# snap-research/MMVID

Hardware: AMD Instinct MI355X
Metric: video-tokens/sec training step, 8-frame 128px text-to-video (higher is better)
Workload: dtype bf16

## Files before the change

### include/mmvid_hip.h

```cpp
#ifndef MMVID_HIP_H
#define MMVID_HIP_H
#include <stdint.h>
#ifdef __cplusplus
extern "C" {
#endif

const char* mmvid_last_error(void);
int mmvid_abi_version(void);
int mmvid_device_count(void);

int mmvid_vq_sqnorm(const float* codebook, int n, int dim, float* ee, void* stream);
int mmvid_vq_argmin_l2(const float* z, const float* codebook, const float* ee, int64_t rows, int n, int dim,
                       int64_t* idx, float* dmin, void* stream);
int mmvid_gather_rows(const float* table, int64_t table_rows, const int64_t* idx, int64_t rows, int dim,
                      float* out_f32, void* out_bf16, void* stream);

int mmvid_gemm_bf16(int a_kmajor, int b_kmajor, int M, int N, int K, const void* A, int64_t lda, const void* B,
                    int64_t ldb, int batch, int64_t strideA, int64_t strideB, int64_t strideC, int splitk,
                    float alpha, const float* bias, const float* residual, int64_t ldr, const void* dact_pre,
                    void* save_pre, int64_t ldp, int act, int accumulate, float* out_f32, void* out_bf16,
                    int64_t ldc, float* out_colsum,
                    void* stream);

int mmvid_decode_trace(void* dev_buf);
int mmvid_decode_persistent_trace(void* dev_buf);

int mmvid_gemm_bf16_dw(int64_t M, int N, int K, const void* dY, int64_t ldy, const void* X, int64_t ldx, int splitk,
                       float* workspace, float* dW, int accumulate, void* stream);
int mmvid_gemm_dw_pick_splitk(int64_t M, int N, int K);
typedef struct {
    int N, K;
    const void* dY;
    int64_t ldy, strideY;
    const void* X;
    int64_t ldx, strideX;
    float* const* dW_list;
} mmvid_dw_kind_t;
int mmvid_gemm_bf16_dw_multi(int64_t M, int nkinds, const mmvid_dw_kind_t* kinds, int groups, int accumulate, void* stream);
int mmvid_gemm_bf16_dw_grouped(int64_t M, int N, int K, const void* dY, int64_t ldy, int64_t strideY, const void* X, int64_t ldx,
                               int64_t strideX, int groups, float* const* dW_list, int accumulate, void* stream);
double mmvid_gemm_dw_multi_fill(int nkinds, const mmvid_dw_kind_t* kinds, int groups);

int mmvid_layernorm_fwd(const float* x, int64_t ldx, int64_t rows, int E, const float* w, const float* b, float eps,
                        void* y_bf16, float* y_f32, int64_t ldy, float* mean, float* rstd, void* stream);
int mmvid_layernorm_bwd(const float* dy, int64_t lddy, const float* x, int64_t ldx, const float* mean,
                        const float* rstd, const float* w, int64_t rows, int E, float* dx, int64_t lddx,
                        int add_into_dx, void* dx_bf16, float* dw, float* db, float* dx_colsum, void* stream);
int mmvid_layernorm_bwd_ws(const float* dy, int64_t lddy, const float* x, int64_t ldx, const float* mean,
                           const float* rstd, const float* w, int64_t rows, int E, float* dx, int64_t lddx,
                           int add_into_dx, void* dx_bf16, float* dw, float* db, float* dx_colsum, float* workspace,
                           int64_t workspace_floats, void* stream);
int mmvid_layernorm_bwd_ex(const void* dy, int dy_is_bf16, int64_t lddy, const float* x, int64_t ldx, const float* mean,
                           const float* rstd, const float* w, int64_t rows, int E, float* dx, int64_t lddx, int add_into_dx,
                           void* dx_bf16, float* dw, float* db, float* dx_colsum, float* workspace, int64_t workspace_floats,
                           void* stream);
typedef struct {
    const float* partial;
    float *dw, *db, *dx_colsum;
} mmvid_ln_reduce_t;
int mmvid_layernorm_bwd_partial(const void* dy, int dy_is_bf16, int64_t lddy, const float* x, int64_t ldx, const float* mean,
                                const float* rstd, const float* w, int64_t rows, int E, float* dx, int64_t lddx, int add_into_dx,
                                void* dx_bf16, int want_dw, int want_db, int want_colsum, float* workspace,
                                int64_t workspace_floats, int* blocks_out, void* stream);
int mmvid_layernorm_bwd_reduce_multi(int n, const mmvid_ln_reduce_t* items, int blocks, int E, void* stream);
int mmvid_groupnorm_swish_nhwc(const void* x, int x_is_bf16, int N, int64_t hw, int C, const float* w,
                               const float* b, float eps, int swish, float* stats_scratch, int partial_blocks,
                               void* y_bf16, float* y_f32, void* stream);

int mmvid_attention_fwd(const void* qkv, int64_t ld, int B, int L, int H, int E, float scale, int mask_mode, int r0,
                        int c0, int r1, int c1, void* out, int64_t ldo, float* lse2, void* stream);
int mmvid_attention_bwd(const void* qkv, int64_t ld, const void* O, int64_t ldo, const void* dO, int64_t lddo,
                        const float* lse2, float* delta, int B, int L, int H, int E, float scale, int mask_mode,
                        int r0, int c0, int r1, int c1, void* dqkv, int64_t ldg, void* stream);
int mmvid_attention_bwd_bias(const void* qkv, int64_t ld, const void* O, int64_t ldo, const void* dO, int64_t lddo,
                             const float* lse2, float* delta, int B, int L, int H, int E, float scale, int mask_mode, int r0,
                             int c0, int r1, int c1, void* dqkv, int64_t ldg, float* dbias, void* stream);
int mmvid_assemble_sequence(const float* const* tables, const int64_t* table_rows, int ntables, const int64_t* ids,
                            const int32_t* seg, const float* pos, int64_t B, int L, int E, float* out, void* stream);
int mmvid_assemble_sequence_bwd(float* const* grad_tables, const int64_t* table_rows, int ntables,
                                const int64_t* ids, const int32_t* seg, const float* dx, int64_t B, int L, int E,
                                float* dpos, int accumulate_dpos, void* stream);
int mmvid_cross_entropy_fwd(const float* logits, int64_t ldl, const int64_t* target, const uint8_t* select,
                            int64_t rows, int V, float* lse, float* loss_sum, void* stream);
int mmvid_cross_entropy_bwd(const float* logits, int64_t ldl, const int64_t* target, const uint8_t* select,
                            const float* lse, const float* gscale, int64_t rows, int V, void* dlogits_bf16,
                            int64_t ldd, void* stream);
int mmvid_colsum_bf16(const void* dy, int64_t ld, int64_t M, int N, float* db, void* stream);
typedef struct {
    const float* w[3];
    float* gw[3];
    int32_t dst0, rows, naxes, src0;
    int32_t d[3];
    int32_t pad;
} mmvid_pos_segment_t;
int mmvid_pos_table_fwd(const mmvid_pos_segment_t* segs, int nseg, int L, int E, float* out, void* stream);
int mmvid_pos_table_bwd(const mmvid_pos_segment_t* segs, int nseg, int E, const float* g, void* stream);
int mmvid_lincomb3(const float* a, const float* b, const float* c, float wa, float wb, float wc, float* out, void* stream);
int mmvid_scale3(const float* g, float wa, float wb, float wc, float* ga, float* gb, float* gc, void* stream);
int mmvid_rows_pack(const float* W, int64_t V, int E, const int64_t* ids, int n, int64_t* uid, float* rows, void* stream);
int mmvid_rows_merge(float* W, int64_t V, int E, const int64_t* ids, const float* rows, int n, void* stream);

int mmvid_device_faults(int64_t* counts, int reset);

int mmvid_grad_sqnorm(const float* g, int64_t n, float* out_accum, void* stream);
int mmvid_adam_step(float* p, const float* g, float* m, float* v, void* shadow_bf16, int64_t n, float lr,
                    float beta1, float beta2, float eps, float weight_decay, int step, const float* step_dev,
                    float max_norm, const float* sqnorm, float grad_scale, void* stream);
int mmvid_grad_sqnorm_det(const float* g, int64_t n, float* partials, float* out_accum, void* stream);
int mmvid_adam_step_lr(float* p, const float* g, float* m, float* v, void* shadow_bf16, int64_t n, float lr,
                       const float* lr_dev, float beta1, float beta2, float eps, float weight_decay, int step,
                       const float* step_dev, float max_norm, const float* sqnorm, float grad_scale, void* stream);
int mmvid_grad_sqnorm_rows(const float* g, int64_t n, float* partials, float* out_accum, const uint8_t* row_flags,
                           int64_t table_lo, int64_t table_rows, int rowlen, void* stream);
int mmvid_adam_step_rows(float* p, const float* g, float* m, float* v, void* shadow_bf16, int64_t n, float lr,
                         const float* lr_dev, float beta1, float beta2, float eps, float weight_decay, int step,
                         const float* step_dev, float max_norm, const float* sqnorm, float grad_scale,
                         const uint8_t* row_flags, int64_t table_lo, int64_t table_rows, int rowlen, void* stream);
int mmvid_lr_schedule(const float* step_dev, int kind, float lr_min, float lr_max, int warmup_steps, int every,
                      float* lr_out, void* stream);
int mmvid_counter_add(float* counter, float value, void* stream);
int mmvid_cast_f32_to_bf16(const float* x, void* y, int64_t n, void* stream);

int mmvid_msm_masks(uint64_t seed, const float* step_dev, int B, int T, int f, const float* strategy_prob, float bern_lo,
                    float bern_hi, float pc_prob, uint8_t* mask1, float* not_fully_masked, int32_t* strategy_out,
                    void* stream);
int mmvid_msm_masks_inject(const int32_t* decisions, const uint8_t* bernoulli, int B, int T, int f, uint8_t* mask1,
                           float* not_fully_masked, void* stream);
int mmvid_warp_params_bytes(void);
int mmvid_vid_warp(uint64_t seed, const float* step_dev, const float* x, int B, int T, int C, int H, int W,
                   const float* strategy_prob, void* params_scratch, int draw_params, float* out, void* stream);
int mmvid_vid_warp_new_frames(uint64_t seed, const float* step_dev, const float* x, int B, int T, int C, int H, int W,
                              const float* strategy_prob, void* params_scratch, int draw_params, float* new_frames,
                              void* stream);
int mmvid_vid_warp_tokens(const int64_t* target_tok, const int64_t* new_frame_tok, const void* params, int B, int T, int n,
                          int64_t* out, void* stream);
int mmvid_frames_u8_to_f32(const uint8_t* frames_u8, int N, int H, int W, float* out, void* stream);
int mmvid_frames_to_u8(const float* img, int64_t N, int H, int W, uint8_t* out, void* stream);
int mmvid_vid_warp_new_frames_u8(uint64_t seed, const float* step_dev, const uint8_t* x_u8, int B, int T, int H, int W,
                                 const float* strategy_prob, void* params_scratch, int draw_params, float* new_frames,
                                 void* stream);
int mmvid_vid_warp_draw(uint64_t seed, const float* step_dev, int B, int T, const float* strategy_prob, void* params_scratch,
                        void* stream);
int mmvid_token_rows_gather(const uint16_t* table, int64_t table_rows, const int64_t* frame_index, int64_t rows, int n,
                            int64_t* out, void* stream);
int mmvid_erase_tokens_choice(uint64_t seed, const float* step_dev, int nchoice, const float* cumprob, const int32_t* modes,
                              const int32_t* boxes, int frame0_full, int B, int Tv, int f, int64_t value, int64_t* tok,
                              void* stream);
int mmvid_random_erase_tokens(uint64_t seed, const float* step_dev, int B, int Tv, int f, float p, float scale_lo,
                              float scale_hi, float ratio_lo, float ratio_hi, int erase_half, int64_t value, int64_t* tok,
                              void* stream);

int mmvid_visual_color_jitter(uint64_t seed, const float* step_dev, float* x, int B, int Tv, int C, int H, int W, float p,
                              int first_frame, float* params_out, void* stream);

typedef struct {
    const float *ln1_w, *ln1_b, *ln2_w, *ln2_b;
    const void* in_w;
    const float* in_b;
    const void* out_w;
    const float* out_b;
    const void* fc_w;
    const float* fc_b;
    const void* pj_w;
    const float* pj_b;
    float *g_ln1_w, *g_ln1_b, *g_ln2_w, *g_ln2_b, *g_in_w, *g_in_b, *g_out_w, *g_out_b, *g_fc_w, *g_fc_b, *g_pj_w,
        *g_pj_b;
} mmvid_tower_layer_t;

typedef struct {
    int B, L, E, H, F, layers;
    int mask_mode, r0, c0, r1, c1;
    float ln_eps;
} mmvid_tower_cfg_t;

int mmvid_tower_workspace(const mmvid_tower_cfg_t* cfg, int64_t* saved_bytes, int64_t* scratch_bytes);
int mmvid_tower_forward(const mmvid_tower_cfg_t* cfg, const mmvid_tower_layer_t* layers, const float* x_in,
                        float* x_out, void* saved, void* scratch, void* stream);
int mmvid_tower_backward(const mmvid_tower_cfg_t* cfg, const mmvid_tower_layer_t* layers, float* g,
                         void* saved, void* scratch, void* stream);


int mmvid_tower_prefill(const mmvid_tower_cfg_t* cfg, const mmvid_tower_layer_t* layers, const float* x_in,
                        float* x_out, void* kv_cache, int Lmax, void* scratch, void* stream);
int mmvid_tower_decode(const mmvid_tower_cfg_t* cfg, const mmvid_tower_layer_t* layers, const float* x_in, float* x_out,
                       void* kv_cache, int Lmax, const int32_t* pos_dev, int pos, void* scratch, void* stream);
int mmvid_tower_decode_fused(const mmvid_tower_cfg_t* cfg, const mmvid_tower_layer_t* layers, const float* x_in,
                             float* x_out, void* kv_cache, int Lmax, const int32_t* pos_dev, int pos, void* scratch,
                             void* stream);
int mmvid_tower_decode_fused_slice(const mmvid_tower_cfg_t* cfg, const mmvid_tower_layer_t* layers, const float* x_in,
                                   float* x_out, void* kv_cache, int Lmax, int cache_batch, int32_t* pos_dev, int pos,
                                   int advance_pos, void* scratch, void* stream);
int mmvid_tower_decode_persistent_supported(const mmvid_tower_cfg_t* cfg, int Lmax);
int64_t mmvid_tower_decode_persistent_workspace_bytes(int B);
int mmvid_tower_decode_persistent(const mmvid_tower_cfg_t* cfg, const mmvid_tower_layer_t* layers, const float* x_in, float* x_out,
                                  void* kv_cache, int Lmax, int32_t* pos_dev, int pos, int advance_pos, void* workspace, void* stream);
typedef struct {
    int64_t* tok;
    const float* table;
    int64_t table_rows;
    const float* pos_rows;
    int32_t pos_off;
    int32_t record_pos0;
    int64_t* record;
    int64_t record_ld;
    const float *lnf_w, *lnf_b;
    const void* head_w;
    const float* head_b;
    const float* E;
    int64_t e_step_stride;
    int64_t tok_offset;
    float* logits_out;
    int32_t V, e_pos0;
    float lnf_eps, temperature;
} mmvid_decode_token_t;
int mmvid_artv_token_step_persistent(const mmvid_tower_cfg_t* cfg, const mmvid_tower_layer_t* layers, const mmvid_decode_token_t* t,
                                     float* x_out, void* kv_cache, int Lmax, int32_t* pos_dev, void* workspace, void* stream);
int mmvid_gemv_rows(const float* x, int64_t ldx, int NB, int K, const float* ln_w, const float* ln_b, float eps, const void* W,
                    const float* bias, int N, int act, const float* residual, int64_t ldr, int round_in, int round_out,
                    float* out, int64_t ldo, void* stream);
int mmvid_decode_embed(const int64_t* tok, const float* table, int64_t table_rows, const float* pos_rows,
                       const int32_t* pos_dev, int pos_off, int B, int E, float* x, void* stream);
int mmvid_decode_embed_record(const int64_t* tok, const float* table, int64_t table_rows, const float* pos_rows,
                              const int32_t* pos_dev, int pos_off, int B, int E, float* x, int64_t* record, int64_t record_ld,
                              int record_pos0, void* stream);
int mmvid_kv_store(const void* qkv, int64_t ldq, int B, int L, int E, const int32_t* pos_dev, int pos0, int Lmax,
                   void* cache, void* stream);
int mmvid_attention_decode(const void* qkv, int64_t ldq, const void* cache, int B, int Lmax, int H, int E,
                           const int32_t* pos_dev, int pos0, float scale, void* out, int64_t ldo, void* stream);

int mmvid_conv2d_nhwc(int mode, const void* x, int N, int Hin, int Win, int Cin, const void* w, const float* bias,
                      int Cout, const void* residual_bf16, const float* residual_f32, int clamp01, void* out_bf16,
                      float* out_f32, float* gn_partial, void* stream);
int mmvid_conv2d_nhwc_splitk(int mode, const void* x, int N, int Hin, int Win, int Cin, const void* w, const float* bias,
                             int Cout, const void* residual_bf16, const float* residual_f32, int clamp01, void* out_bf16,
                             float* out_f32, float* gn_partial, int splitk, float* workspace, void* stream);
int mmvid_conv3x3_strip_supported(int H, int W, int Cin, int Cout);
int mmvid_conv3x3_strip_nhwc(const void* x, int N, int H, int W, int Cin, const void* w, const float* bias, int Cout,
                             const void* residual_bf16, const float* residual_f32, void* out_bf16, float* out_f32,
                             float* gn_partial64, void* stream);
int mmvid_image_to_nhwc8(const float* img, int N, int H, int W, void* out_bf16, void* stream);
int mmvid_nhwc_to_nchw_f32(const float* x, int N, int H, int W, int C, int Cuse, float* out, void* stream);
int mmvid_spatial_attention(const void* q, const void* k, const void* v, int N, int HW, int C, float scale,
                            float* scores_scratch, void* out_bf16, void* stream);
int mmvid_spatial_attention_ld(const void* q, const void* k, const void* v, int64_t ld, int N, int HW, int C, float scale,
                               float* scores_scratch, void* out_bf16, void* stream);

int mmvid_sample_race(const float* logits, int64_t ld, const float* E, const float* noise_u, float temperature,
                      float logit_div, int64_t R, int V, int64_t tok_offset, int64_t* tok, float* y, void* stream);
int mmvid_sample_race_at(const float* logits, int64_t ld, const float* E, const int32_t* step_dev, int step0, int64_t e_step_stride,
                         const float* noise_u, float temperature, float logit_div, int64_t R, int V, int64_t tok_offset, int64_t* tok,
                         float* y, void* stream);
int mmvid_mp_select_keep(const float* Y, const float* E, const uint8_t* preserve, int b, int Bm, int TS, int k,
                         uint8_t* mask1, void* stream);
int mmvid_mp_build_input(const float* control_emb, const float* image_emb, int64_t table_rows, const float* tpos,
                         const int64_t* I_tok, const uint8_t* mask1, int b, int Bm, int csl, int TS, int E, int64_t mask_id,
                         float* out, void* stream);
int mmvid_mp_update(const uint8_t* mask1, const float* Ynew, const int64_t* Inew, const float* rel_logit,
                    const float* vid_logit, int b, int Bm, int TS, int t, int dynamic, float* Y, int64_t* I_tok,
                    int64_t* Imax, float* Smax, int32_t* tmax, uint8_t* active, float* S_out, int32_t* jmax_out,
                    void* stream);
int mmvid_head_bce_fwd(const float* x, int64_t ldx, const int64_t* rows, int R, int E, const float* ln_w, const float* ln_b,
                       float eps, const float* w, const float* b, const float* label, const float* row_weight,
// ... 154 lines not shown
```

### mmvid_amd/_lib.py

```python
import ctypes
import os
from ctypes import POINTER, Structure, c_char_p, c_float, c_int, c_int32, c_int64, c_uint8, c_uint64, c_void_p

HERE = os.path.dirname(os.path.abspath(__file__))
LIB_PATH = os.environ.get('MMVID_LIB') or os.path.join(HERE, 'libmmvid_hip.so')

P = c_void_p
I, I64, F, U64 = c_int, c_int64, c_float, c_uint64


class TowerLayer(Structure):
    _fields_ = [(n, P) for n in (
        'ln1_w', 'ln1_b', 'ln2_w', 'ln2_b', 'in_w', 'in_b', 'out_w', 'out_b', 'fc_w', 'fc_b', 'pj_w', 'pj_b',
        'g_ln1_w', 'g_ln1_b', 'g_ln2_w', 'g_ln2_b', 'g_in_w', 'g_in_b', 'g_out_w', 'g_out_b', 'g_fc_w', 'g_fc_b',
        'g_pj_w', 'g_pj_b')]


class TowerCfg(Structure):
    _fields_ = [('B', I), ('L', I), ('E', I), ('H', I), ('F', I), ('layers', I), ('mask_mode', I), ('r0', I),
                ('c0', I), ('r1', I), ('c1', I), ('ln_eps', F)]


class DecodeToken(Structure):
    _fields_ = [('tok', c_void_p), ('table', c_void_p), ('table_rows', c_int64), ('pos_rows', c_void_p), ('pos_off', c_int32),
                ('record_pos0', c_int32), ('record', c_void_p), ('record_ld', c_int64), ('lnf_w', c_void_p), ('lnf_b', c_void_p),
                ('head_w', c_void_p), ('head_b', c_void_p), ('E', c_void_p), ('e_step_stride', c_int64), ('tok_offset', c_int64),
                ('logits_out', c_void_p), ('V', c_int32), ('e_pos0', c_int32), ('lnf_eps', c_float), ('temperature', c_float)]


class PostLnLayer(Structure):
    _fields_ = [(n, P) for n in ('qkv_w', 'qkv_b', 'out_w', 'out_b', 'ln1_w', 'ln1_b', 'fc_w', 'fc_b', 'pj_w', 'pj_b', 'ln2_w', 'ln2_b')]


class PostLnCfg(Structure):
    _fields_ = [('B', I), ('L', I), ('E', I), ('H', I), ('F', I), ('layers', I), ('ln_eps', F)]


class Conv3dCfg(Structure):
    _fields_ = [(n, I) for n in ('N', 'T', 'H', 'W', 'Cin', 'Cout', 'kt', 'kh', 'kw', 'st', 'sh', 'sw', 'pt0', 'pt1', 'ph0', 'ph1',
                                 'pw0', 'pw1', 'relu', 'nseg')] + [('seg_end', I * 3), ('ldo', I * 3), ('c_off', I * 3), ('out', P * 3)]


class VqganOp(Structure):
    _fields_ = [('op', c_int32), ('mode', c_int32), ('N', c_int32), ('H', c_int32), ('W', c_int32), ('C', c_int32),
                ('Cout', c_int32), ('flags', c_int32), ('in0', I64), ('in1', I64), ('in2', I64), ('out_bf16', I64),
                ('out_f32', I64), ('scratch', I64), ('w', P), ('b', P), ('ext_in', P), ('ext_out', P), ('eps', F),
                ('pad', c_int32)]


SIGNATURES = {
    'mmvid_vq_sqnorm': [P, I, I, P, P],
    'mmvid_vq_argmin_l2': [P, P, P, I64, I, I, P, P, P],
    'mmvid_gather_rows': [P, I64, P, I64, I, P, P, P],
    'mmvid_gemm_bf16': [I, I, I, I, I, P, I64, P, I64, I, I64, I64, I64, I, F, P, P, I64, P, P, I64, I, I, P, P, I64, P, P],
    'mmvid_gemm_bf16_dw': [I64, I, I, P, I64, P, I64, I, P, P, I, P],
    'mmvid_gemm_dw_pick_splitk': [I64, I, I],
    'mmvid_gemm_bf16_dw_grouped': [I64, I, I, P, I64, I64, P, I64, I64, I, P, I, P],
    'mmvid_gemm_bf16_dw_multi': [I64, I, P, I, I, P],
    'mmvid_layernorm_fwd': [P, I64, I64, I, P, P, F, P, P, I64, P, P, P],
    'mmvid_layernorm_bwd': [P, I64, P, I64, P, P, P, I64, I, P, I64, I, P, P, P, P, P],
    'mmvid_layernorm_bwd_ws': [P, I64, P, I64, P, P, P, I64, I, P, I64, I, P, P, P, P, P, I64, P],
    'mmvid_layernorm_bwd_partial': [P, I, I64, P, I64, P, P, P, I64, I, P, I64, I, P, I, I, I, P, I64, P, P],
    'mmvid_layernorm_bwd_reduce_multi': [I, P, I, I, P],
    'mmvid_layernorm_bwd_ex': [P, I, I64, P, I64, P, P, P, I64, I, P, I64, I, P, P, P, P, P, I64, P],
    'mmvid_groupnorm_swish_nhwc': [P, I, I, I64, I, P, P, F, I, P, I, P, P, P],
    'mmvid_attention_fwd': [P, I64, I, I, I, I, F, I, I, I, I, I, P, I64, P, P],
    'mmvid_attention_bwd': [P, I64, P, I64, P, I64, P, P, I, I, I, I, F, I, I, I, I, I, P, I64, P],
    'mmvid_attention_bwd_bias': [P, I64, P, I64, P, I64, P, P, I, I, I, I, F, I, I, I, I, I, P, I64, P, P],
    'mmvid_assemble_sequence': [POINTER(P), POINTER(I64), I, P, P, P, I64, I, I, P, P],
    'mmvid_assemble_sequence_bwd': [POINTER(P), POINTER(I64), I, P, P, P, I64, I, I, P, I, P],
    'mmvid_cross_entropy_fwd': [P, I64, P, P, I64, I, P, P, P],
    'mmvid_cross_entropy_bwd': [P, I64, P, P, P, P, I64, I, P, I64, P],
    'mmvid_colsum_bf16': [P, I64, I64, I, P, P],
    'mmvid_grad_sqnorm': [P, I64, P, P],
    'mmvid_adam_step': [P, P, P, P, P, I64, F, F, F, F, F, I, P, F, P, F, P],
    'mmvid_cast_f32_to_bf16': [P, P, I64, P],
    'mmvid_tower_workspace': [POINTER(TowerCfg), POINTER(I64), POINTER(I64)],
    'mmvid_tower_forward': [POINTER(TowerCfg), POINTER(TowerLayer), P, P, P, P, P],
    'mmvid_tower_backward': [POINTER(TowerCfg), POINTER(TowerLayer), P, P, P, P],
    'mmvid_tower_prefill': [POINTER(TowerCfg), POINTER(TowerLayer), P, P, P, I, P, P],
    'mmvid_tower_decode': [POINTER(TowerCfg), POINTER(TowerLayer), P, P, P, I, P, I, P, P],
    'mmvid_tower_decode_fused': [POINTER(TowerCfg), POINTER(TowerLayer), P, P, P, I, P, I, P, P],
    'mmvid_tower_decode_persistent': [POINTER(TowerCfg), POINTER(TowerLayer), P, P, P, I, P, I, I, P, P],
    'mmvid_artv_token_step_persistent': [POINTER(TowerCfg), POINTER(TowerLayer), POINTER(DecodeToken), P, P, I, P, P, P],
    'mmvid_tower_decode_fused_slice': [POINTER(TowerCfg), POINTER(TowerLayer), P, P, P, I, I, P, I, I, P, P],
    'mmvid_gemv_rows': [P, I64, I, I, P, P, F, P, P, I, I, P, I64, I, I, P, I64, P],
    'mmvid_decode_embed': [P, P, I64, P, P, I, I, I, P, P],
    'mmvid_decode_embed_record': [P, P, I64, P, P, I, I, I, P, P, I64, I, P],
    'mmvid_kv_store': [P, I64, I, I, I, P, I, I, P, P],
    'mmvid_attention_decode': [P, I64, P, I, I, I, I, P, I, F, P, I64, P],
    'mmvid_conv2d_nhwc': [I, P, I, I, I, I, P, P, I, P, P, I, P, P, P, P],
    'mmvid_conv2d_nhwc_splitk': [I, P, I, I, I, I, P, P, I, P, P, I, P, P, P, I, P, P],
    'mmvid_conv3x3_strip_supported': [I, I, I, I],
    'mmvid_conv3x3_strip_nhwc': [P, I, I, I, I, P, P, I, P, P, P, P, P, P],
    'mmvid_image_to_nhwc8': [P, I, I, I, P, P],
    'mmvid_nhwc_to_nchw_f32': [P, I, I, I, I, I, P, P],
    'mmvid_spatial_attention': [P, P, P, I, I, I, F, P, P, P],
    'mmvid_spatial_attention_ld': [P, P, P, I64, I, I, I, F, P, P, P],
    'mmvid_conv2d_nhwc_split3': [I, P, I, I, I, I, P, P, I, P, I, P, P, I, P, P],
    'mmvid_conv3x3_strip_nhwc_split3': [P, I, I, I, I, P, P, I, P, P, P, P, P],
    'mmvid_conv3x3_strip_nhwc_f16': [P, I, I, I, I, P, P, I, P, P, P, P, P],
    'mmvid_split_f32_bf16x2': [P, I64, P, P],
    'mmvid_image_to_nhwc8_split': [P, I, I, I, P, P],
    'mmvid_groupnorm_swish_nhwc_split': [P, I, I64, I, P, P, F, I, P, I, P, P],
    'mmvid_groupnorm_swish_nhwc_f16out': [P, I, I64, I, P, P, F, I, P, I, P, P],
    'mmvid_decode_trace': [P],
    'mmvid_decode_persistent_trace': [P],
    'mmvid_vqgan_run': [POINTER(VqganOp), I, P, P],
    'mmvid_sample_race': [P, I64, P, P, F, F, I64, I, I64, P, P, P],
    'mmvid_sample_race_at': [P, I64, P, P, I, I64, P, F, F, I64, I, I64, P, P, P],
    'mmvid_mp_select_keep': [P, P, P, I, I, I, I, P, P],
    'mmvid_mp_build_input': [P, P, I64, P, P, P, I, I, I, I, I, I64, P, P],
    'mmvid_mp_update': [P, P, P, P, P, I, I, I, I, I, P, P, P, P, P, P, P, P, P],
    'mmvid_head_bce_fwd': [P, I64, P, I, I, P, P, F, P, P, P, P, P, I, F, P, P, P, P, P],
    'mmvid_head_bce_bwd': [P, I64, P, I, I, P, P, P, P, P, P, P, P, P, I, F, P, P, I64, P, P, P, P, P],
    'mmvid_bert_build_ids': [P, P, P, P, P, P, I, I, I, I, I64, I64, I, I, P, P, P, P, P],
    'mmvid_grad_sqnorm_det': [P, I64, P, P, P],
    'mmvid_adam_step_lr': [P, P, P, P, P, I64, F, P, F, F, F, F, I, P, F, P, F, P],
    'mmvid_lr_schedule': [P, I, F, F, I, I, P, P],
    'mmvid_grad_sqnorm_rows': [P, I64, P, P, P, I64, I64, I, P],
    'mmvid_adam_step_rows': [P, P, P, P, P, I64, F, P, F, F, F, F, I, P, F, P, F, P, I64, I64, I, P],
    'mmvid_counter_add': [P, F, P],
    'mmvid_msm_masks': [U64, P, I, I, I, P, F, F, F, P, P, P, P],
    'mmvid_msm_masks_inject': [P, P, I, I, I, P, P, P],
    'mmvid_vid_warp': [U64, P, P, I, I, I, I, I, P, P, I, P, P],
    'mmvid_vid_warp_new_frames': [U64, P, P, I, I, I, I, I, P, P, I, P, P],
    'mmvid_vid_warp_tokens': [P, P, P, I, I, I, P, P],
    'mmvid_frames_u8_to_f32': [P, I, I, I, P, P],
    'mmvid_vid_warp_new_frames_u8': [U64, P, P, I, I, I, I, P, P, I, P, P],
    'mmvid_vid_warp_draw': [U64, P, I, I, P, P, P],
    'mmvid_token_rows_gather': [P, I64, P, I64, I, P, P],
    'mmvid_erase_tokens_choice': [U64, P, I, P, P, P, I, I, I, I, I64, P, P],
    'mmvid_random_erase_tokens': [U64, P, I, I, I, F, F, F, F, F, I, I64, P, P],
    'mmvid_visual_color_jitter': [U64, P, P, I, I, I, I, I, F, I, P, P],
    'mmvid_gemm_f32': [I, I, I, I, P, I64, P, I64, I, I64, I64, I64, F, P, P, P, I64, P],
    'mmvid_conv2d_nhwc_f32': [I, P, I, I, I, I, P, P, I, P, I, P, P],
    'mmvid_image_to_nhwc4_f32': [P, I, I, I, P, P],
    'mmvid_groupnorm_swish_nhwc_f32': [P, I, I64, I, P, P, F, I, P, P, P],
    'mmvid_spatial_attention_f32': [P, P, P, I, I, I, F, P, P, P],
    'mmvid_probe': [I, P, P, P],
    'mmvid_prof_begin': [I],
    'mmvid_prof_enable': [I],
    'mmvid_graph_stats': [P],
    'mmvid_set_option': [c_char_p, I],
    'mmvid_get_option': [c_char_p, POINTER(I)],
    'mmvid_colsum_bf16_det': [P, I64, I64, I, P, P, I64, P],
    'mmvid_cross_entropy_fwd_det': [P, I64, P, P, I64, I, P, P, P, I64, P],
    'mmvid_assemble_sequence_bwd_det': [POINTER(P), POINTER(I64), I, P, P, P, I64, I, I, P, I, P, I64, P],
    'mmvid_gemm_bf16_det': [I, I, I, I, I, P, I64, P, I64, I, I64, I64, I64, I, F, P, P, I64, P, P, I64, I, I, P, P, I64, P, P, I64, P],
    'mmvid_attention_bwd_bias_det': [P, I64, P, I64, P, I64, P, P, I, I, I, I, F, I, I, I, I, I, P, I64, P, P, I64, P],
    'mmvid_device_faults': [P, I],
    'mmvid_pos_table_fwd': [P, I, I, I, P, P],
    'mmvid_pos_table_bwd': [P, I, I, P, P],
    'mmvid_lincomb3': [P, P, P, F, F, F, P, P],
    'mmvid_scale3': [P, F, F, F, P, P, P, P],
    'mmvid_prof_end': [P, P, P, P, I],
    'mmvid_rows_pack': [P, I64, I, P, I, P, P, P],
    'mmvid_rows_merge': [P, I64, I, P, P, I, P],
    'mmvid_clip_patchify': [P, I, I, I, I, I, P, P],
    'mmvid_clip_image_assemble': [P, P, P, P, P, F, I, I, I, P, P],
    'mmvid_clip_text_embed': [P, I, I, P, I64, P, I, P, P, P],
    'mmvid_clip_pool_project': [P, I, I, I, P, P, P, F, P, I, I, P, P],
# ... 129 lines not shown
```

### mmvid_amd/clip_tower.py

```python
import ctypes
import os
import math

import torch
from torch import nn

from . import _lib, ops
from .functional import _note_params, _with_param_zeros

TOWER_SHAPES = {
    'openai_clip_visual': (768, 12, 12),
    'openai_clip_text': (512, 12, 8),
}
MATRIX_KEYS = ('attn.in_proj_weight', 'attn.out_proj.weight', 'mlp.c_fc.weight', 'mlp.c_proj.weight')


class _Holder(nn.Module):
    """Parameter container (no forward): gives parameters their reference names."""


def _linear_params(out_f, in_f, std):
    h = _Holder()
    h.weight = nn.Parameter(torch.randn(out_f, in_f) * std)
    h.bias = nn.Parameter(torch.zeros(out_f))
    return h


def _ln_params(e):
    h = _Holder()
    h.weight = nn.Parameter(torch.ones(e))
    h.bias = nn.Parameter(torch.zeros(e))
    return h


class ResidualAttentionBlockParams(_Holder):
    def __init__(self, width, layers):
        super().__init__()
        proj_std = (width**-0.5) * ((2 * layers)**-0.5)
        attn_std = width**-0.5
        fc_std = (2 * width)**-0.5
        self.attn = _Holder()
        self.attn.in_proj_weight = nn.Parameter(torch.randn(3 * width, width) * attn_std)
        self.attn.in_proj_bias = nn.Parameter(torch.zeros(3 * width))
        self.attn.out_proj = _linear_params(width, width, proj_std)
        self.ln_1 = _ln_params(width)
        self.mlp = _Holder()
        self.mlp.c_fc = _linear_params(4 * width, width, fc_std)
        self.mlp.c_proj = _linear_params(width, 4 * width, proj_std)
        self.ln_2 = _ln_params(width)


class _TowerParams(_Holder):
    def __init__(self, width, layers):
        super().__init__()
        self.resblocks = nn.ModuleList([ResidualAttentionBlockParams(width, layers) for _ in range(layers)])


class _TowerFn(torch.autograd.Function):
    @staticmethod
    def forward(ctx, x, tower, keep, *params):
        _note_params(ctx, (x, tower, keep) + params)
        ctx.tower = tower
        y, saved = tower._run_forward(x, keep=keep)
        ctx.saved_arena = saved
        ctx.shape = x.shape
        return y

    @staticmethod
    def backward(ctx, gy):
        g = gy.contiguous().clone()
        ctx.tower._run_backward(g, ctx.saved_arena, ctx.shape)
        ctx.saved_arena = None
        return _with_param_zeros(ctx, (g.view(ctx.shape), None, None) + (None, ) * (len(ctx.needs_input_grad) - 3))


class DecodeSession:

    def __init__(self, tower, kv_cache, first_pos, graph, fused=True):
        self.tower, self.cache, self.fused = tower, kv_cache, fused
        B, dev = kv_cache.shape[1], kv_cache.device
        self.cfg = tower._cfg(B, kv_cache.shape[2])
        self.layers, self._keep = tower._layer_structs(False)
        _, self.scratch = tower._workspace(self.cfg, dev, False)
        self.x = torch.zeros(B, tower.width, device=dev, dtype=torch.float32)
        self.y = torch.zeros_like(self.x)
        self.pos = torch.tensor([first_pos], dtype=torch.int32, device=dev)
        self.host_pos = int(first_pos)
        self.graph, self.want_graph, self.calls = None, graph, 0
        self._slice_cfgs = {}
        lib = _lib.load()
        self.persistent = bool(fused is True and os.environ.get('MMVID_DECODE_PERSISTENT', '1') != '0'
                               and lib.mmvid_tower_decode_persistent_supported(ctypes.byref(self.cfg), kv_cache.shape[2]))
        self.ws = torch.zeros(lib.mmvid_tower_decode_persistent_workspace_bytes(B) // 8, dtype=torch.int64, device=dev) if self.persistent else None

    def _enqueue(self):
        B, E = self.x.shape[0], self.x.shape[-1]
        if self.persistent:
            _lib.call('mmvid_tower_decode_persistent', ctypes.byref(self.cfg), self.layers, ops._p(self.x), ops._p(self.y),
                      ops._p(self.cache), self.cache.shape[2], ops._p(self.pos), 0, 1, ops._p(self.ws), ops._stream())
            return
        Lmax = self.cache.shape[2]
        if self.fused and E <= 768:
            per = 64 if E in (512, 768) else 16
            for b0 in range(0, B, per):
                nb = min(per, B - b0)
                cfg = self.cfg if nb == B else self._slice_cfgs.setdefault(nb, self.tower._cfg(nb, Lmax))
                _lib.call('mmvid_tower_decode_fused_slice', ctypes.byref(cfg), self.layers, self.x[b0:].data_ptr(), self.y[b0:].data_ptr(),
                          self.cache[0, b0].data_ptr(), Lmax, B, ops._p(self.pos), 0, int(b0 + per >= B), ops._p(self.scratch), ops._stream())
            return
        _lib.call('mmvid_tower_decode', ctypes.byref(self.cfg), self.layers, ops._p(self.x), ops._p(self.y),
                  ops._p(self.cache), Lmax, ops._p(self.pos), 0, ops._p(self.scratch), ops._stream())
        self.pos.add_(1)

    def token_step(self, tk):
        assert self.persistent
        _lib.call('mmvid_artv_token_step_persistent', ctypes.byref(self.cfg), self.layers, ctypes.byref(tk), ops._p(self.y), ops._p(self.cache),
                  self.cache.shape[2], ops._p(self.pos), ops._p(self.ws), ops._stream())
        self.host_pos += 1

    def failed(self):
        return bool(self.persistent and int(self.ws[1]) != 0)

    def fall_back(self, pos):
        self.persistent, self.graph = False, None
        self.fell_back = getattr(self, 'fell_back', 0) + 1
        self.pos.fill_(int(pos))
        self.host_pos = int(pos)

    def check(self):
        if self.failed():
            raise _lib.MMVIDError('persistent decode step: a poll timed out (the device was shared while it ran); results are invalid. '
                                  'Set MMVID_DECODE_PERSISTENT=0 to use the five-launch step.')

    @torch.no_grad()
    def step(self, x_new, verify=False):
        self.x.copy_(x_new)
        self.calls += 1
        if self.want_graph and self.graph is None and self.calls == 2:
            g = torch.cuda.CUDAGraph()
            side = torch.cuda.Stream()
            side.wait_stream(torch.cuda.current_stream())
            with torch.cuda.stream(side):
                with torch.cuda.graph(g, stream=side):
                    self._enqueue()
            torch.cuda.current_stream().wait_stream(side)
            self.graph = g
        if self.graph is not None:
            self.graph.replay()
        else:
            self._enqueue()
        if verify and self.persistent and self.failed():
            self.fall_back(self.host_pos)
            self._enqueue()
        self.host_pos += 1
        return self.y


class OpenAICLIPTransformer(nn.Module):
    def __init__(self, seq_len=0, which_model='openai_clip_text', model_path=None, causal=True, mask_type='causal',
                 mask_kwargs=None, layers=None, width=None, heads=None):
        super().__init__()
        if not which_model.startswith('openai_clip'):
            raise NotImplementedError(which_model)
        w, l, h = TOWER_SHAPES[which_model]
        self.width, self.layers, self.heads = width or w, layers or l, heads or h
        self.debug_keep_saved = False
        assert self.width == 64 * self.heads, 'head_dim must be 64 (CLIP towers)'
        self.context_length = seq_len
        self.causal = causal
        self.transformer = _TowerParams(self.width, self.layers)
        self.mask_spec = self.build_attention_mask(seq_len, mask_type, **(mask_kwargs or {})) if causal else None
        if model_path is not None:
            self.load_clip_checkpoint(model_path, which_model)
        self._shadow = None
        self._shadow_key = None
        self._scratch = None
        self._scratch_retired = []
        self.backward_chunk_layers = int(os.environ.get('MMVID_BWD_CHUNK', 0))
        self.on_layers_done = None

    @staticmethod
    def build_attention_mask(context_length, mask_type='causal', **kwargs):
        if mask_type == 'causal':
            return 'causal'
        if mask_type == 'mask_prev':
            idx = list(kwargs['index'])
            assert len(idx) <= 2, 'the kernels carry at most two restricted rows (BERT uses [ST1],[VID])'
            return ('rows', [(int(i), int(i)) for i in idx])
        raise NotImplementedError(mask_type)

    def dense_attention_mask(self, L=None):
        L = L or self.context_length
        if self.mask_spec is None:
            return None
        if self.mask_spec == 'causal':
            return torch.full((L, L), float('-inf')).triu_(1)
        m = torch.zeros(L, L)
        for r, c in self.mask_spec[1]:
            m[r, :c] = float('-inf')
        return m

    def load_clip_checkpoint(self, path, which_model):
        sd = torch.jit.load(path, map_location='cpu').state_dict()
        prefix = 'transformer.' if which_model == 'openai_clip_text' else 'visual.transformer.'
        own = {k[len(prefix):]: v.float() for k, v in sd.items() if k.startswith(prefix + 'resblocks.')}
        self.transformer.load_state_dict(own)

    def forward(self, x, **kwargs):
        assert x.dim() == 3 and x.shape[-1] == self.width
        keep = torch.is_grad_enabled() and (x.requires_grad or self._any_trainable())
        return _TowerFn.apply(x, self, keep, *self.parameters())

    def new_kv_cache(self, B, max_len, device):
        assert self.mask_spec == 'causal', 'incremental decoding needs the causal mask'
        return torch.empty(self.layers, B, max_len, 2 * self.width, device=device, dtype=torch.bfloat16)

    @torch.no_grad()
    def prefill(self, x, kv_cache):
        x = ops._chk(x.contiguous(), torch.float32, 'tower input')
        B, L, _ = x.shape
        cfg = self._cfg(B, L)
        layers, _keep = self._layer_structs(False)
        _, scratch = self._workspace(cfg, x.device, False)
        y = torch.empty_like(x)
        _lib.call('mmvid_tower_prefill', ctypes.byref(cfg), layers, ops._p(x), ops._p(y), ops._p(kv_cache),
                  kv_cache.shape[2], ops._p(scratch), ops._stream())
        return y

    @torch.no_grad()
    def decode_step(self, x_new, kv_cache, pos, pos_dev=None):
        x_new = ops._chk(x_new.contiguous(), torch.float32, 'tower input')
        B = x_new.shape[0]
        cfg = self._cfg(B, kv_cache.shape[2])
        layers, _keep = self._layer_structs(False)
        _, scratch = self._workspace(cfg, x_new.device, False)
        y = torch.empty_like(x_new)
        _lib.call('mmvid_tower_decode', ctypes.byref(cfg), layers, ops._p(x_new), ops._p(y), ops._p(kv_cache),
                  kv_cache.shape[2], ops._p(pos_dev), int(pos), ops._p(scratch), ops._stream())
        return y

    def decode_session(self, kv_cache, first_pos, graph=True, fused=True):
        return DecodeSession(self, kv_cache, first_pos, graph, fused)

    def _any_trainable(self):
        return any(p.requires_grad for p in self.parameters())

    def _matrix_params(self):
        for blk in self.transformer.resblocks:
            yield blk.attn.in_proj_weight
            yield blk.attn.out_proj.weight
            yield blk.mlp.c_fc.weight
            yield blk.mlp.c_proj.weight

    def attach_shadow(self, views):
        self._shadow = list(views)
        self.mark_shadow_fresh()

    def mark_shadow_fresh(self):
        self._shadow_key = tuple((p._version, p.data_ptr()) for p in self._matrix_params())

    def _sync_shadow(self):
        ps = list(self._matrix_params())
        key = tuple((p._version, p.data_ptr()) for p in ps)
        if self._shadow is None or self._shadow[0].device != ps[0].device:
            self._shadow = [torch.empty(p.shape, device=p.device, dtype=torch.bfloat16) for p in ps]
            self._shadow_key = None
        if key != self._shadow_key:
            for p, s in zip(ps, self._shadow):
                ops.cast_bf16(p.detach().contiguous(), s)
            self._shadow_key = key
        return self._shadow

    def _cfg(self, B, L):
        c = _lib.TowerCfg()
        c.B, c.L, c.E, c.H, c.F, c.layers = B, L, self.width, self.heads, 4 * self.width, self.layers
        c.mask_mode, c.r0, c.c0, c.r1, c.c1 = ops._mask_args(self.mask_spec)
        c.ln_eps = 1e-5
        return c

    def _layer_structs(self, with_grads):
        sh = self._sync_shadow()
        arr = (_lib.TowerLayer * self.layers)()
        keep = []

        def ptr(t):
            keep.append(t)
            return t.data_ptr()

        def gptr(p):
            if not with_grads or not p.requires_grad:
                return None
            if p.grad is None:
                p.grad = torch.zeros_like(p)
            return p.grad.data_ptr()

        for i, blk in enumerate(self.transformer.resblocks):
            a = arr[i]
            a.ln1_w, a.ln1_b = ptr(blk.ln_1.weight), ptr(blk.ln_1.bias)
            a.ln2_w, a.ln2_b = ptr(blk.ln_2.weight), ptr(blk.ln_2.bias)
            a.in_w, a.in_b = ptr(sh[4 * i]), ptr(blk.attn.in_proj_bias)
            a.out_w, a.out_b = ptr(sh[4 * i + 1]), ptr(blk.attn.out_proj.bias)
            a.fc_w, a.fc_b = ptr(sh[4 * i + 2]), ptr(blk.mlp.c_fc.bias)
            a.pj_w, a.pj_b = ptr(sh[4 * i + 3]), ptr(blk.mlp.c_proj.bias)
            a.g_ln1_w, a.g_ln1_b = gptr(blk.ln_1.weight), gptr(blk.ln_1.bias)
            a.g_ln2_w, a.g_ln2_b = gptr(blk.ln_2.weight), gptr(blk.ln_2.bias)
            a.g_in_w, a.g_in_b = gptr(blk.attn.in_proj_weight), gptr(blk.attn.in_proj_bias)
            a.g_out_w, a.g_out_b = gptr(blk.attn.out_proj.weight), gptr(blk.attn.out_proj.bias)
            a.g_fc_w, a.g_fc_b = gptr(blk.mlp.c_fc.weight), gptr(blk.mlp.c_fc.bias)
            a.g_pj_w, a.g_pj_b = gptr(blk.mlp.c_proj.weight), gptr(blk.mlp.c_proj.bias)
        return arr, keep

    def _workspace(self, cfg, device, keep):
        sb, cb = ctypes.c_int64(), ctypes.c_int64()
        _lib.call('mmvid_tower_workspace', ctypes.byref(cfg), ctypes.byref(sb), ctypes.byref(cb))
        if self._scratch is None or self._scratch.device != torch.device(device) or self._scratch.numel() < cb.value:
            if self._scratch is not None:
                self._scratch_retired.append(self._scratch)
            self._scratch = torch.empty(cb.value, device=device, dtype=torch.uint8)
        saved = torch.empty(sb.value, device=device, dtype=torch.uint8) if keep else None
        return saved, self._scratch

    def _run_forward(self, x, keep):
        x = ops._chk(x.contiguous(), torch.float32, 'tower input')
        B, L, _ = x.shape
        cfg = self._cfg(B, L)
        layers, _keep = self._layer_structs(False)
        saved, scratch = self._workspace(cfg, x.device, keep)
        y = torch.empty_like(x)
        _lib.call('mmvid_tower_forward', ctypes.byref(cfg), layers, ops._p(x), ops._p(y), ops._p(saved), ops._p(scratch),
                  ops._stream())
        if self.debug_keep_saved:
            self._last_saved = saved
        return y, saved

    def backward_chunks(self):
        if self.on_layers_done is None:
            return [(0, self.layers)]
        if self.backward_chunk_layers <= 0:
            return self._planned_chunks()
        step = self.backward_chunk_layers
        out, hi = [], self.layers
        while hi > 0:
            lo = max(0, hi - step)
            out.append((lo, hi))
            hi = lo
        return out

    def _planned_chunks(self):
        if getattr(self, '_chunk_plan', None) is None or self._chunk_plan[0] != self.layers:
            E = self.width
            F = 4 * E
            t = sum(-(-n // 256) * -(-k // 128) for n, k in ((3 * E, E), (E, E), (F, E), (E, F)))
            waste = lambda n: (-(-n * t // 256)) - n * t / 256.0
            best, plan = None, [(0, self.layers)]
            for a in range(3, self.layers - 2):
                w = waste(a) + waste(self.layers - a) + 0.02 * abs(a - 0.6 * self.layers)
                if best is None or w < best:
                    best, plan = w, [(self.layers - a, self.layers), (0, self.layers - a)]
            self._chunk_plan = (self.layers, plan)
        return self._chunk_plan[1]

    def _run_backward(self, g, saved, shape):
        if saved is None:
            raise _lib.MMVIDError('tower backward without saved activations (forward ran under no_grad)')
        B, L, _ = shape
        cfg = self._cfg(B, L)
        layers, _keep = self._layer_structs(True)
        _, scratch = self._workspace(cfg, g.device, False)
        sb = ctypes.c_int64()
        _lib.call('mmvid_tower_workspace', ctypes.byref(cfg), ctypes.byref(sb), None)
        if sb.value != saved.numel():
            raise _lib.MMVIDError(f'tower backward: the saved arena holds {saved.numel()} bytes, the current layout needs {sb.value} '
                                  '(the library changed between forward and backward)')
        per_layer = saved.numel() // self.layers
        for lo, hi in self.backward_chunks():
            sub = self._cfg(B, L)
            sub.layers = hi - lo
            lp = ctypes.cast(ctypes.byref(layers, lo * ctypes.sizeof(_lib.TowerLayer)), ctypes.POINTER(_lib.TowerLayer))
            _lib.call('mmvid_tower_backward', ctypes.byref(sub), lp, ops._p(g),
                      ctypes.c_void_p(saved.data_ptr() + lo * per_layer), ops._p(scratch), ops._stream())
            if self.on_layers_done is not None:
                self.on_layers_done(lo)
```

### mmvid_amd/csrc/attn.hip

```cpp
#include <type_traits>

#include "../../include/mmvid_hip.h"
#include "gemm_core.h"
#include "prof.h"

namespace {
using mmvid_core::blds16;
using mmvid_core::dma_publish_barrier;
using mmvid_core::make_rsrc;
using mmvid_core::rsrc_t;
using mmvid_core::bf16x4_t;
using mmvid_core::ds_read_tr16;
using mmvid_core::lds_addr;
using mmvid_core::lgkm_wait_tied;
using mmvid_core::xcd_remap;

struct MaskSpec {
    int mode;
    int r0, c0, r1, c1;
};

__device__ __forceinline__ bool is_masked(const MaskSpec& m, int q, int key, int L) {
    const bool pad = key >= L;
    const bool causal = (m.mode == 1) & (key > q);
// ... 441 lines not shown
            f32x16 dp = mfma32z(row_frag<SS, 0>(Vt, rl), dof[0]);
            s = mfma32(row_frag<SS, 1>(Kt, rl), qf[1], s), dp = mfma32(row_frag<SS, 1>(Vt, rl), dof[1], dp);
            s = mfma32(row_frag<SS, 2>(Kt, rl), qf[2], s), dp = mfma32(row_frag<SS, 2>(Vt, rl), dof[2], dp);
            s = mfma32(row_frag<SS, 3>(Kt, rl), qf[3], s), dp = mfma32(row_frag<SS, 3>(Vt, rl), dof[3], dp);
            if (SS == 0 && more) {
                __builtin_amdgcn_sched_barrier(0);
                sk.issue((t + 1) * 64, nxt, wave), sv.issue((t + 1) * 64, nxt + TILE, wave);
            }
            mfma_settle(s), mfma_settle(dp);
            bf16x8_t kt4[4];
            tr_frags4<SS, KOFF>(trk, kt4);
            if constexpr (!PLAIN) {
                if ((mask.mode == 1 && key0 + 31 > q_wave0) || key0 < row_kmax) {
#pragma unroll
                    for (int r = 0; r < 16; ++r) s[r] = is_masked(mask, q, key0 + acc_row(r, h), L) ? -INFINITY : s[r];
                }
                if (key0 + 32 > L) {
#pragma unroll
                    for (int r = 0; r < 16; ++r) s[r] = (key0 + acc_row(r, h) >= L) ? -INFINITY : s[r];
                }
            }
            (void)exp2_affine_sum(s, scale_log2, neg_lse);
#pragma unroll
            for (int r = 0; r < 16; ++r) s[r] *= dp[r] - my_delta;
            bf16x8_t dsf[2] = {pack_half(s, 0), pack_half(s, 1)};
            lgkm_wait_tied<0>(kt4[0], kt4[1], kt4[2], kt4[3], dsf[0], dsf[1]);
            dq[0] = mfma32(kt4[0], dsf[0], dq[0]);
            dq[1] = mfma32(kt4[1], dsf[0], dq[1]);
            dq[0] = mfma32(kt4[2], dsf[1], dq[0]);
            dq[1] = mfma32(kt4[3], dsf[1], dq[1]);
        };
        sub(ic<0>{});
        if (PLAIN || t * 64 + 32 < L) sub(ic<1>{});
    };
    if (!wave_active) {
        for (int t = t_begin; t < t_end; ++t) {
            dma_publish_barrier();
            char* nxt = smem[(t + 1 - t_begin) & 1];
            if (t + 1 < t_end) sk.issue((t + 1) * 64, nxt, wave), sv.issue((t + 1) * 64, nxt + TILE, wave);
        }
        return;
    }
#pragma unroll 1
    for (int ph = 0; ph < 2; ++ph) {
        const int a = ph == 0 ? t_begin : hi, z = ph == 0 ? lo : t_end;
#pragma unroll 1
        for (int t = a; t < z; ++t) {
            dma_publish_barrier();
            if ((t - t_begin) & 1)
                tile(ic<1>{}, ic<0>{}, t);
            else
                tile(ic<0>{}, ic<0>{}, t);
        }
        if (ph == 0) {
#pragma unroll 1
            for (int t = lo; t < hi; t += 2) {
                dma_publish_barrier();
                tile(ic<0>{}, ic<1>{}, t);
                dma_publish_barrier();
                tile(ic<1>{}, ic<1>{}, t + 1);
            }
        }
    }
    mfma_settle(dq[0]), mfma_settle(dq[1]);
    if (q < L) store_row64(dqkv + ((long)b * L + q) * ldg + hd * 64, dq, scale, h);
    if (dbias) colsum_rows64<DET>(dq, scale, q < L, (DET ? dbias_slab_row(dbias, b, qt, wave, L, E) : dbias) + hd * 64, lane);
}

constexpr int DKV_BUF = 2 * TILE + 512;

template <int SS>
__device__ __forceinline__ f32x16 row_consts(const float* st, int h) {
    f32x16 a;
#pragma unroll
    for (int g4 = 0; g4 < 4; ++g4) {
        const float4 v = *reinterpret_cast<const float4*>(st + 32 * SS + 8 * g4 + 4 * h);
        a[4 * g4] = v.x, a[4 * g4 + 1] = v.y, a[4 * g4 + 2] = v.z, a[4 * g4 + 3] = v.w;
    }
    return a;
}

template <bool DET>
__global__ __launch_bounds__(256, 3) void attn_bwd_dkv_kernel(const bf16_t* __restrict__ qkv, long ld, const bf16_t* __restrict__ dO, long lddo,
                                                               const float* __restrict__ lse2, const float* __restrict__ delta, int L, int H,
                                                               int E, FastDiv nrt_d, FastDiv h_d, float scale, float scale_log2,
                                                               float inv_scale_log2, MaskSpec mask, bf16_t* __restrict__ dqkv, long ldg,
                                                               float* __restrict__ dbias) {
    __shared__ __attribute__((aligned(16))) char dsm[2][DKV_BUF];
    const int tid = threadIdx.x, lane = tid & 63, wave = __builtin_amdgcn_readfirstlane(tid >> 6), l32 = lane & 31, h = lane >> 5;
    const BlockCoords bc = block_coords(nrt_d, h_d);
    const int kt = bc.rt, hd = bc.hd, b = bc.b;
    const bf16_t* Qbase = qkv + (long)b * L * ld + hd * 64;
    const bf16_t* dObase = dO + (long)b * L * lddo + hd * 64;
    const float* lse_b = lse2 + ((long)b * H + hd) * L;
    const float* del_b = delta + ((long)b * H + hd) * L;
    const int nq_tiles = (L + 63) >> 6;
    const RowLane rl = row_lane_offs(lane);
    const TrLane trq = tr_lane_at(tr_lane_offs(lane), lds_addr(dsm[0]));
    const int key_wave0 = kt * ROWS_PER_BLOCK + wave * 32;
    const int key = key_wave0 + l32;
    const bool wave_active = key_wave0 < L;
    bf16x8_t kf[4], vf[4];
    {
        const int keyc = key < L ? key : L - 1;
        const bf16_t* Kp = qkv + ((long)b * L + keyc) * ld + E + hd * 64;
        const bf16_t* Vp = Kp + E;
#pragma unroll
        for (int s = 0; s < 4; ++s) {
            kf[s] = *reinterpret_cast<const bf16x8_t*>(Kp + 16 * s + 8 * h);
            vf[s] = *reinterpret_cast<const bf16x8_t*>(Vp + 16 * s + 8 * h);
        }
    }
    auto load_stat = [&](int t) -> float {
        if (tid >= 128) return 0.f;
        const int qq = t * 64 + (tid & 63);
        if (tid < 64) return qq < L ? -lse_b[qq] * inv_scale_log2 : -INFINITY;
        return qq < L ? -del_b[qq] : 0.f;
    };
    const int t_begin = (mask.mode == 1) ? (kt * ROWS_PER_BLOCK) >> 6 : 0, t_end = nq_tiles;

    TileStage sq, sdo;
    sq.init(Qbase, ld, L, wave, lane), sdo.init(dObase, lddo, L, wave, lane);
    sq.issue(t_begin * 64, dsm[0], wave), sdo.issue(t_begin * 64, dsm[0] + TILE, wave);
    float stat = load_stat(t_begin);
    if (tid < 128) reinterpret_cast<float*>(dsm[0] + 2 * TILE)[tid] = stat;

    f32x16 dk[2] = {zero16(), zero16()}, dv[2] = {zero16(), zero16()};
    const bool rows_hit0 = mask.mode == 2 && key_wave0 < mask.c0, rows_hit1 = mask.mode == 2 && key_wave0 < mask.c1;

    auto tile = [&](auto st_c, int t) {
        constexpr int ST = decltype(st_c)::value;
        constexpr int OFF = ST * DKV_BUF;
        const char* Qt = dsm[ST];
        const char* dOt = Qt + TILE;
        const float* st_nlse = reinterpret_cast<const float*>(Qt + 2 * TILE);
        const float* st_ndel = st_nlse + 64;
        char* nx = dsm[ST ^ 1];
        const bool more = t + 1 < t_end;
        dma_publish_barrier();
        if (!wave_active) {
            if (more) {
                sq.issue((t + 1) * 64, nx, wave), sdo.issue((t + 1) * 64, nx + TILE, wave);
                stat = load_stat(t + 1);
                if (tid < 128) reinterpret_cast<float*>(nx + 2 * TILE)[tid] = stat;
            }
            return;
        }
        auto sub = [&](auto ss_c) {
            constexpr int SS = decltype(ss_c)::value;
            const int q0 = t * 64 + 32 * SS;
            f32x16 s = row_consts<SS>(st_nlse, h), dp = row_consts<SS>(st_ndel, h);
            s = mfma32(row_frag<SS, 0>(Qt, rl), kf[0], s), dp = mfma32(row_frag<SS, 0>(dOt, rl), vf[0], dp);
            s = mfma32(row_frag<SS, 1>(Qt, rl), kf[1], s), dp = mfma32(row_frag<SS, 1>(dOt, rl), vf[1], dp);
            s = mfma32(row_frag<SS, 2>(Qt, rl), kf[2], s), dp = mfma32(row_frag<SS, 2>(dOt, rl), vf[2], dp);
            s = mfma32(row_frag<SS, 3>(Qt, rl), kf[3], s), dp = mfma32(row_frag<SS, 3>(dOt, rl), vf[3], dp);
            if (SS == 0 && more) {
                __builtin_amdgcn_sched_barrier(0);
                sq.issue((t + 1) * 64, nx, wave), sdo.issue((t + 1) * 64, nx + TILE, wave);
                stat = load_stat(t + 1);
            }
            mfma_settle(s), mfma_settle(dp);
            bf16x8_t dot4[4];
            tr_frags4<SS, OFF + TILE>(trq, dot4);
            bool nm = mask.mode == 1 && key_wave0 + 31 > q0;
            nm = nm || (rows_hit0 && mask.r0 >= q0 && mask.r0 < q0 + 32) || (rows_hit1 && mask.r1 >= q0 && mask.r1 < q0 + 32);
            if (nm) {
#pragma unroll
                for (int r = 0; r < 16; ++r) s[r] = is_masked(mask, q0 + acc_row(r, h), key, L) ? -INFINITY : s[r];
            }
#pragma unroll
            for (int r = 0; r < 16; ++r) {
                float p, ds;
                asm("v_mul_f32 %0, %2, %3\n\tv_exp_f32 %0, %0\n\ts_nop 0\n\tv_mul_f32 %1, %0, %4"
                    : "=&v"(p), "=&v"(ds)
                    : "v"(s[r]), "v"(scale_log2), "v"(dp[r]));
                s[r] = p, dp[r] = ds;
            }
            bf16x8_t pf[2] = {pack_half(s, 0), pack_half(s, 1)};
            bf16x8_t dsf[2] = {pack_half(dp, 0), pack_half(dp, 1)};
            bf16x8_t qt4[4];
            tr_frags4<SS, OFF>(trq, qt4);
            lgkm_wait_tied<8>(dot4[0], dot4[1], dot4[2], dot4[3], pf[0], pf[1]);
            dv[0] = mfma32(dot4[0], pf[0], dv[0]);
            dv[1] = mfma32(dot4[1], pf[0], dv[1]);
            dv[0] = mfma32(dot4[2], pf[1], dv[0]);
            dv[1] = mfma32(dot4[3], pf[1], dv[1]);
            lgkm_wait_tied<0>(qt4[0], qt4[1], qt4[2], qt4[3], dsf[0], dsf[1]);
            dk[0] = mfma32(qt4[0], dsf[0], dk[0]);
            dk[1] = mfma32(qt4[1], dsf[0], dk[1]);
            dk[0] = mfma32(qt4[2], dsf[1], dk[0]);
            dk[1] = mfma32(qt4[3], dsf[1], dk[1]);
        };
        sub(ic<0>{});
        if (t * 64 + 32 < L) sub(ic<1>{});
        if (more && tid < 128) reinterpret_cast<float*>(nx + 2 * TILE)[tid] = stat;
    };
    for (int t = t_begin; t < t_end; t += 2) {
        tile(ic<0>{}, t);
        if (t + 1 >= t_end) break;
        tile(ic<1>{}, t + 1);
    }
    if (!wave_active) return;
    mfma_settle(dk[0]), mfma_settle(dk[1]), mfma_settle(dv[0]), mfma_settle(dv[1]);
    const int lane_e = (int)__lane_id(), key_e = key_wave0 + (lane_e & 31), h_e = lane_e >> 5;
    if (key_e < L) {
        bf16_t* kp = dqkv + ((long)b * L + key_e) * ldg + E + hd * 64;
        store_row64(kp, dk, scale, h_e);
        store_row64(kp + E, dv, 1.0f, h_e);
    }
    if (dbias) {
        float* db = DET ? dbias_slab_row(dbias, b, kt, wave, L, E) : dbias;
        colsum_rows64<DET>(dk, scale, key_e < L, db + E + hd * 64, lane_e);
        colsum_rows64<DET>(dv, 1.0f, key_e < L, db + 2 * E + hd * 64, lane_e);
    }
}

static MaskSpec make_mask(int mode, int r0, int c0, int r1, int c1) {
    MaskSpec m;
    m.mode = mode, m.r0 = r0, m.c0 = c0, m.r1 = r1, m.c1 = c1;
    return m;
}

}

#define ATTN_COMMON_CHECKS(name)                                                                            \
    MMVID_REQUIRE(B > 0 && L > 0 && H > 0 && E == H * 64, name ": need E == H*64 (head_dim 64), got E=%d H=%d", E, H); \
    MMVID_REQUIRE(mask_mode >= 0 && mask_mode <= 2, name ": mask_mode %d", mask_mode);                             \
    MMVID_REQUIRE((int64_t)cdiv(L, ROWS_PER_BLOCK) * H * B * (H > 64 ? H : 64) < (1ll << 31), name ": too many (batch, head, row block) units")

extern "C" int mmvid_attention_fwd(const void* qkv, int64_t ld, int B, int L, int H, int E, float scale, int mask_mode,
                                   int r0, int c0, int r1, int c1, void* out, int64_t ldo, float* lse2, void* stream) {
    MMVID_REQUIRE(qkv && out && lse2, "attention_fwd: null pointer");
    ATTN_COMMON_CHECKS("attention_fwd");
    MMVID_REQUIRE(ld % 8 == 0 && ldo % 8 == 0 && ((uintptr_t)out & 15) == 0, "attention_fwd: leading dims must be multiples of 8, out 16-byte aligned");
    MMVID_REQUIRE((int64_t)L * ld * 2 < (1ll << 31), "attention_fwd: one batch entry of qkv must be smaller than 2 GiB");
    hipStream_t s = (hipStream_t)stream;
    MmvidProfScope prof(PROF_ATTN_FWD, 4.0 * B * H * (double)L * L * 64, s);
    const int nrt = cdiv(L, ROWS_PER_BLOCK), nblocks = nrt * H * B;
    const FastDiv nrt_d = make_fastdiv(nrt), h_d = make_fastdiv(H);
    const MaskSpec m = make_mask(mask_mode, r0, c0, r1, c1);
    hipLaunchKernelGGL(attn_fwd_kernel<false>, dim3(nblocks), dim3(256), 0, s, (const bf16_t*)qkv, (long)ld, L, H, E, nrt_d, h_d,
                       scale * 1.4426950408889634f, m, (bf16_t*)out, (long)ldo, lse2, (const int32_t*)nullptr);
    MMVID_LAUNCH_CHECK("attention_fwd");
    return MMVID_OK;
}

extern "C" int mmvid_attention_fwd_keylen(const void* qkv, int64_t ld, int B, int L, int H, int E, float scale, const int32_t* key_len,
                                          void* out, int64_t ldo, float* lse2, void* stream) {
    MMVID_REQUIRE(qkv && out && key_len, "attention_fwd_keylen: null pointer");
    const int mask_mode = 0;
    ATTN_COMMON_CHECKS("attention_fwd_keylen");
    MMVID_REQUIRE(ld % 8 == 0 && ldo % 8 == 0 && ((uintptr_t)out & 15) == 0,
                  "attention_fwd_keylen: leading dims must be multiples of 8, out 16-byte aligned");
    MMVID_REQUIRE((int64_t)L * ld * 2 < (1ll << 31), "attention_fwd_keylen: one batch entry of qkv must be smaller than 2 GiB");
    hipStream_t s = (hipStream_t)stream;
    MmvidProfScope prof(PROF_ATTN_FWD, 4.0 * B * H * (double)L * L * 64, s);
    const int nrt = cdiv(L, ROWS_PER_BLOCK), nblocks = nrt * H * B;
    const FastDiv nrt_d = make_fastdiv(nrt), h_d = make_fastdiv(H);
    hipLaunchKernelGGL(attn_fwd_kernel<true>, dim3(nblocks), dim3(256), 0, s, (const bf16_t*)qkv, (long)ld, L, H, E, nrt_d, h_d,
                       scale * 1.4426950408889634f, make_mask(0, -1, 0, -1, 0), (bf16_t*)out, (long)ldo, lse2, key_len);
    MMVID_LAUNCH_CHECK("attention_fwd_keylen");
    return MMVID_OK;
}

extern "C" int mmvid_attention_bwd(const void* qkv, int64_t ld, const void* O, int64_t ldo, const void* dO, int64_t lddo,
                                   const float* lse2, float* delta, int B, int L, int H, int E, float scale,
                                   int mask_mode, int r0, int c0, int r1, int c1, void* dqkv, int64_t ldg,
                                   void* stream) {
    return mmvid_attention_bwd_bias(qkv, ld, O, ldo, dO, lddo, lse2, delta, B, L, H, E, scale, mask_mode, r0, c0, r1, c1, dqkv, ldg,
                                    nullptr, stream);
}

static int attention_bwd_impl(const void* qkv, int64_t ld, const void* O, int64_t ldo, const void* dO, int64_t lddo,
                                        const float* lse2, float* delta, int B, int L, int H, int E, float scale,
                                        int mask_mode, int r0, int c0, int r1, int c1, void* dqkv, int64_t ldg,
                                        float* dbias, float* det_slab, void* stream) {
    MMVID_REQUIRE(qkv && O && dO && lse2 && delta && dqkv, "attention_bwd: null pointer");
    ATTN_COMMON_CHECKS("attention_bwd");
    MMVID_REQUIRE(ld % 8 == 0 && ldo % 8 == 0 && lddo % 8 == 0 && ldg % 8 == 0 && ((uintptr_t)dqkv & 15) == 0,
                  "attention_bwd: leading dims must be multiples of 8, dqkv 16-byte aligned");
    MMVID_REQUIRE((int64_t)L * ld * 2 < (1ll << 31) && (int64_t)L * lddo * 2 < (1ll << 31),
                  "attention_bwd: one batch entry of qkv / dO must be smaller than 2 GiB");
    hipStream_t s = (hipStream_t)stream;
    const MaskSpec m = make_mask(mask_mode, r0, c0, r1, c1);
    const float sl2 = scale * 1.4426950408889634f;
    MmvidProfScope prof(PROF_ATTN_BWD, 10.0 * B * H * (double)L * L * 64, s);
    const int nrt = cdiv(L, ROWS_PER_BLOCK), nblocks = nrt * H * B;
    const FastDiv nrt_d = make_fastdiv(nrt), h_d = make_fastdiv(H);
    if (dbias && det_slab) {
        const int nslab = B * nrt * 4;
        if (hipMemsetAsync(det_slab, 0, (size_t)nslab * 3 * E * 4, s) != hipSuccess) {
            mmvid_set_error("attention_bwd_bias_det: memset failed");
            return MMVID_ERR_HIP;
        }
        hipLaunchKernelGGL(attn_bwd_dq_kernel<true>, dim3(nblocks), dim3(256), 0, s, (const bf16_t*)qkv, (long)ld, (const bf16_t*)O, (long)ldo,
                           (const bf16_t*)dO, (long)lddo, lse2, delta, L, H, E, nrt_d, h_d, scale, sl2, m, (bf16_t*)dqkv, (long)ldg, det_slab);
        hipLaunchKernelGGL(attn_bwd_dkv_kernel<true>, dim3(nblocks), dim3(256), 0, s, (const bf16_t*)qkv, (long)ld, (const bf16_t*)dO, (long)lddo,
                           lse2, delta, L, H, E, nrt_d, h_d, scale, sl2, 1.0f / sl2, m, (bf16_t*)dqkv, (long)ldg, det_slab);
        mmvid_slab_reduce(det_slab, nslab, 3 * E, dbias, s);
        MMVID_LAUNCH_CHECK("attention_bwd_bias_det");
        return MMVID_OK;
    }
    hipLaunchKernelGGL(attn_bwd_dq_kernel<false>, dim3(nblocks), dim3(256), 0, s, (const bf16_t*)qkv, (long)ld, (const bf16_t*)O, (long)ldo,
                       (const bf16_t*)dO, (long)lddo, lse2, delta, L, H, E, nrt_d, h_d, scale, sl2, m, (bf16_t*)dqkv, (long)ldg, dbias);
    hipLaunchKernelGGL(attn_bwd_dkv_kernel<false>, dim3(nblocks), dim3(256), 0, s, (const bf16_t*)qkv, (long)ld, (const bf16_t*)dO, (long)lddo, lse2,
                       delta, L, H, E, nrt_d, h_d, scale, sl2, 1.0f / sl2, m, (bf16_t*)dqkv, (long)ldg, dbias);
    MMVID_LAUNCH_CHECK("attention_bwd");
    return MMVID_OK;
}

extern "C" int mmvid_attention_bwd_bias(const void* qkv, int64_t ld, const void* O, int64_t ldo, const void* dO, int64_t lddo,
                                        const float* lse2, float* delta, int B, int L, int H, int E, float scale,
                                        int mask_mode, int r0, int c0, int r1, int c1, void* dqkv, int64_t ldg,
                                        float* dbias, void* stream) {
    return attention_bwd_impl(qkv, ld, O, ldo, dO, lddo, lse2, delta, B, L, H, E, scale, mask_mode, r0, c0, r1, c1, dqkv, ldg, dbias,
                              nullptr, stream);
}

extern "C" int64_t mmvid_attention_bwd_bias_det_workspace_bytes(int B, int L, int E) {
    return (int64_t)B * cdiv(L > 0 ? L : 1, ROWS_PER_BLOCK) * 4 * 3 * E * 4;
}

extern "C" int mmvid_attention_bwd_bias_det(const void* qkv, int64_t ld, const void* O, int64_t ldo, const void* dO, int64_t lddo,
                                            const float* lse2, float* delta, int B, int L, int H, int E, float scale,
                                            int mask_mode, int r0, int c0, int r1, int c1, void* dqkv, int64_t ldg,
                                            float* dbias, void* workspace, int64_t workspace_bytes, void* stream) {
    if (dbias)
        MMVID_REQUIRE(workspace && B > 0 && L > 0 && workspace_bytes >= mmvid_attention_bwd_bias_det_workspace_bytes(B, L, E),
                      "attention_bwd_bias_det: workspace of %lld bytes needed (mmvid_attention_bwd_bias_det_workspace_bytes)",
                      (long long)mmvid_attention_bwd_bias_det_workspace_bytes(B, L, E));
    return attention_bwd_impl(qkv, ld, O, ldo, dO, lddo, lse2, delta, B, L, H, E, scale, mask_mode, r0, c0, r1, c1, dqkv, ldg, dbias,
                              (float*)workspace, stream);
}
```

### mmvid_amd/csrc/gemm.hip

```cpp
#include "../../include/mmvid_hip.h"
#include "gemm_core.h"
#include "prof.h"

namespace {
using namespace mmvid_core;


constexpr int GROUP_MAX = 48;
constexpr int KIND_MAX = 4;
struct GroupKind {
    const unsigned short* A;
    const unsigned short* B;
    long strideA, strideB, lda, ldb;
    int M, N, tiles_n, tiles_m;
    int first;
    int out0;
    int colmajor;
};

struct GemmParams {
    const bf16_t* A;
    const bf16_t* B;
    int M, N, K;
    long lda, ldb;
    long strideA, strideB, strideC;
    int splitk;
    const float* bias;
    const float* residual;
    long ldr;
    const bf16_t* dact_pre;
    bf16_t* save_pre;
    long ldp;
    int act;
    int accumulate;
    float alpha;
    float* out_f32;
    bf16_t* out_bf16;
    long ldc;
    float* partial;
    float* colsum;
    int colsum_det;
    int tiles_n, tiles_m;
    int group_n;
};
struct GroupTable {
    int n_kinds;
    GroupKind kinds[KIND_MAX];
    float* out_list[GROUP_MAX];
};
__device__ __forceinline__ float sigmoid1702(float x) {
    return __builtin_amdgcn_rcpf(1.0f + __builtin_amdgcn_exp2f(-1.702f * 1.4426950408889634f * x));
}
__device__ __forceinline__ float quick_gelu(float x) { return x * sigmoid1702(x); }
__device__ __forceinline__ float gelu_erf(float x) { return 0.5f * x * (1.0f + erff(x * 0.70710678118654752f)); }
__device__ __forceinline__ float quick_gelu_grad(float x) {
    float s = sigmoid1702(x);
    return s * (1.0f + 1.702f * x * (1.0f - s));
}

__device__ __forceinline__ void slab_write_row(const f32x16 (&acc_i)[2], float* slab, int wm, int wn, int lane) {
    const int frow = lane & 31, fh = lane >> 5;
#pragma unroll
    for (int j = 0; j < 2; ++j)
#pragma unroll
        for (int q = 0; q < 4; ++q)
            *reinterpret_cast<float4*>(slab + (wm * 32 + frow) * SLAB_PITCH + wn * 64 + j * 32 + 8 * q + 4 * fh) =
                make_float4(acc_i[j][4 * q], acc_i[j][4 * q + 1], acc_i[j][4 * q + 2], acc_i[j][4 * q + 3]);
}
template <int NT, int WAVE_ROWS>
__device__ __forceinline__ void slab_piece_wr(int tid, int k, int i, int& r, int& m_local, int& c) {
    const int idx = tid + NT * k;
    r = idx >> 5;
    c = (idx & 31) * 4;
    m_local = (r >> 5) * WAVE_ROWS + i * 32 + (r & 31);
}
template <int THREADS, int WAVE_ROWS, int NI>
__device__ __forceinline__ void gemm_epilogue(const GemmParams& p, char* smem, f32x16 (&acc)[NI][2], int bm0, int bn0, int batch,
                                              int ks, int tid, int wm, int wn, int lane) {
#pragma unroll
    for (int i = 0; i < NI; ++i) mfma_settle(acc[i][0]), mfma_settle(acc[i][1]);
    float* slab = reinterpret_cast<float*>(smem);
    const long cb = (long)batch * p.strideC;
    const int n = bn0 + 4 * (tid & 31);
    const bool n_ok = n < p.N;
    const bool use_bias = p.bias && (p.splitk == 1 || ks == 0);
    const float4 bias4 = (use_bias && n_ok) ? *reinterpret_cast<const float4*>(p.bias + n) : make_float4(0.f, 0.f, 0.f, 0.f);
    const float* addbase = p.residual ? p.residual + cb
                                      : ((p.accumulate && !p.partial && p.splitk == 1) ? p.out_f32 + cb : nullptr);
    const long ldadd = p.residual ? p.ldr : p.ldc;
    float cs[4] = {0.f, 0.f, 0.f, 0.f};
#pragma unroll
    for (int i = 0; i < NI; ++i) {
        __syncthreads();
        slab_write_row(acc[i], slab, wm, wn, lane);
        __syncthreads();
        float4 v4[8], add4[8];
        uint2 pre2[8];
        int mrow[8];
#pragma unroll
        for (int k = 0; k < 8; ++k) {
            int r, ml, c;
            slab_piece_wr<THREADS, WAVE_ROWS>(tid, k, i, r, ml, c);
            mrow[k] = bm0 + ml;
            const bool ok = n_ok && mrow[k] < p.M;
            v4[k] = *reinterpret_cast<const float4*>(slab + r * SLAB_PITCH + c);
            add4[k] = (addbase && ok) ? *reinterpret_cast<const float4*>(addbase + (long)mrow[k] * ldadd + n)
                                      : make_float4(0.f, 0.f, 0.f, 0.f);
            pre2[k] = (p.dact_pre && ok) ? *reinterpret_cast<const uint2*>(p.dact_pre + cb + (long)mrow[k] * p.ldp + n)
                                         : make_uint2(0u, 0u);
        }
#pragma unroll
        for (int k = 0; k < 8; ++k) {
            const int m = mrow[k];
            if (!n_ok || m >= p.M) continue;
            float v[4] = {v4[k].x * p.alpha + bias4.x, v4[k].y * p.alpha + bias4.y, v4[k].z * p.alpha + bias4.z,
                          v4[k].w * p.alpha + bias4.w};
            if (p.partial) {
                *reinterpret_cast<float4*>(p.partial + ((long)ks * p.M + m) * p.N + n) = make_float4(v[0], v[1], v[2], v[3]);
                continue;
            }
            if (p.splitk > 1) {
                float* o = p.out_f32 + cb + (long)m * p.ldc + n;
#pragma unroll
                for (int e = 0; e < 4; ++e) unsafeAtomicAdd(o + e, v[e]);
                continue;
            }
            if (p.save_pre)
                *reinterpret_cast<uint2*>(p.save_pre + cb + (long)m * p.ldp + n) = make_uint2(pack_bf2(v[0], v[1]), pack_bf2(v[2], v[3]));
            if (p.act == 1) {
#pragma unroll
                for (int e = 0; e < 4; ++e) v[e] = quick_gelu(v[e]);
// ... 295 lines not shown
    extern __shared__ __attribute__((aligned(16))) char smem[];
    const int tid = threadIdx.x;
    const int lane = tid & 63, wave = __builtin_amdgcn_readfirstlane(tid >> 6);
    const int wm = wave >> 1, wn = wave & 1;
    const int ntiles = p.tiles_n > 0 ? p.tiles_n * p.tiles_m : 1;
    const int tile_step = p.tiles_n > 0 ? (int)gridDim.x : 1;
    const int batch = blockIdx.z / p.splitk, ks = blockIdx.z % p.splitk;
  for (int tile = p.tiles_n > 0 ? (int)blockIdx.x : 0; tile < ntiles; tile += tile_step) {
    const int gx = p.tiles_n > 0 ? p.tiles_n : (int)gridDim.x;
    const int wg = p.tiles_n > 0 ? xcd_remap(tile, ntiles) : xcd_remap(blockIdx.x + gridDim.x * blockIdx.y, gridDim.x * gridDim.y);
    const int bn0 = (wg % gx) * BN, bm0 = (wg / gx) * S::ROWS;
    const bf16_t* A = p.A + (long)batch * p.strideA;
    const bf16_t* B = p.B + (long)batch * p.strideB;

    const int ktiles_total = (p.K + BK - 1) / BK;
    const int per = (ktiles_total + p.splitk - 1) / p.splitk;
    const int kt0 = ks * per;
    int kt1 = kt0 + per;
    if (kt1 > ktiles_total) kt1 = ktiles_total;
    const int nt = kt1 - kt0;

    f32x16 acc[2][2];
#pragma unroll
    for (int i = 0; i < 2; ++i)
#pragma unroll
        for (int j = 0; j < 2; ++j)
#pragma unroll
            for (int r = 0; r < 16; ++r) acc[i][j][r] = 0.0f;

    OperandStage<AKM, S::NSUB, S::PPW> sa;
    OperandStage<BKM, 1, S::PPW> sb;
    sa.init(A, p.lda, p.M, p.K, bm0, wave, lane);
    sb.init(B, p.ldb, p.N, p.K, bn0, wave, lane);
    if constexpr (S::NSTAGE == 2) {
        auto stage_tile = [&](int t, char* buf) {
            const int k0 = (kt0 + t) * BK;
            sa.issue(k0, p.K, buf, wave, lane);
            sb.issue(k0, p.K, buf + S::NSUB * TILE_BYTES, wave, lane);
        };
        if (nt > 0) stage_tile(0, smem);
        for (int t = 0; t < nt; ++t) {
            char* cur = smem + (t & 1) * S::STAGE_BYTES;
            char* nxt = smem + ((t + 1) & 1) * S::STAGE_BYTES;
            dma_publish_barrier();
            if (t + 1 < nt) stage_tile(t + 1, nxt);
            mma_tile<AKM, BKM>(cur + (wm >> 1) * TILE_BYTES, cur + S::NSUB * TILE_BYTES, acc, wm & 1, wn, lane);
        }
    } else {
        k_loop_pingpong<AKM, BKM>(
            smem, nt, wave, lane, wm, wn, acc, [&](int t, char* buf) { sa.issue((kt0 + t) * BK, p.K, buf, wave, lane); },
            [&](int t, char* buf) { sb.issue((kt0 + t) * BK, p.K, buf + S::NSUB * TILE_BYTES, wave, lane); });
    }

    gemm_epilogue<S::THREADS, 64, 2>(p, smem, acc, bm0, bn0, batch, ks, tid, wm, wn, lane);
    if (tile + tile_step < ntiles) __syncthreads();
  }
}

template <bool AKM, bool BKM, int EPI, bool GROUPED>
__device__ __forceinline__ void gemm_lw_body(GemmParams p, const GroupTable* gt) {
    using S = BlockShape<4>;
    constexpr int NMW = 8, NL = NLOAD;
    int multi_bm0 = 0, multi_bn0 = 0;
    if constexpr (GROUPED) {
        const int wg = xcd_remap(blockIdx.x, gridDim.x);
        GroupKind kd = gt->kinds[0];
#pragma unroll
        for (int i = 1; i < KIND_MAX; ++i)
            if (wg >= gt->kinds[i].first) kd = gt->kinds[i];
        const int rem = wg - kd.first, per = kd.tiles_n * kd.tiles_m;
        const int g = rem / per, t = rem - g * per;
        float* const out = gt->out_list[kd.out0 + g];
        if (out == nullptr) return;
        int tm, tn;
        if (kd.colmajor)
            tn = t / kd.tiles_m, tm = t - tn * kd.tiles_m;
        else
            tm = t / kd.tiles_n, tn = t - tm * kd.tiles_n;
        multi_bm0 = tm * S::ROWS, multi_bn0 = tn * BN;
        p.A = kd.A + (long)g * kd.strideA, p.B = kd.B + (long)g * kd.strideB;
        p.strideA = p.strideB = p.strideC = 0;
        p.M = kd.M, p.N = kd.N, p.lda = kd.lda, p.ldb = kd.ldb, p.ldc = kd.N;
        p.out_f32 = out;
    }
    extern __shared__ __attribute__((aligned(16))) char smem[];
    const int tid = threadIdx.x;
    const int lane = tid & 63, wave = __builtin_amdgcn_readfirstlane(tid >> 6);
    const int wm = (wave & 7) >> 1, wn = wave & 1;
    const int ntiles = p.tiles_n > 0 ? p.tiles_n * p.tiles_m : 1;
    const int tile_step = p.tiles_n > 0 ? (int)gridDim.x : 1;
    const int ks = p.splitk > 1 ? (int)blockIdx.z : 0;
    const int batch = blockIdx.z;
    const int gx = p.tiles_n > 0 ? p.tiles_n : (int)gridDim.x;
    const bf16_t* A = p.A + (long)batch * p.strideA;
    const bf16_t* B = p.B + (long)batch * p.strideB;
    const int ktiles_total = (p.K + BK - 1) / BK;
    const int per = (ktiles_total + p.splitk - 1) / p.splitk;
    const int kt0 = ks * per;
    const int nt = kt0 + per > ktiles_total ? (ktiles_total - kt0 > 0 ? ktiles_total - kt0 : 0) : per;
    float* bias_lds = nullptr;
    if (p.bias) {
        bias_lds = reinterpret_cast<float*>(smem + S::LDS_BYTES);
        for (int e = tid; e < p.N; e += 64 * NMW + 64 * NL) bias_lds[e] = p.bias[e];
        __syncthreads();
    }
    auto tile_origin = [&](int tile, int& bm0, int& bn0) {
        if constexpr (GROUPED) {
            bm0 = multi_bm0, bn0 = multi_bn0;
            return;
        }
        const int wg = p.tiles_n > 0 ? xcd_remap(tile, ntiles) : xcd_remap(blockIdx.x + gridDim.x * blockIdx.y, gridDim.x * gridDim.y);
        int tn = wg % gx, tm = wg / gx;
        if (p.tiles_n > 0 && p.group_n > 0) {
            const int per_group = p.tiles_m * p.group_n;
            const int g = wg / per_group, rem = wg - g * per_group;
            const int c0 = g * p.group_n;
            const int width = p.tiles_n - c0 < p.group_n ? p.tiles_n - c0 : p.group_n;
            tm = rem / width, tn = c0 + rem - tm * width;
        }
        bn0 = tn * BN, bm0 = tm * S::ROWS;
    };
    const int first = p.tiles_n > 0 ? (int)blockIdx.x : 0;
    if (wave >= NMW) {
        const int w = wave - NMW;
        LoaderStage<AKM, NL> sa;
        LoaderStage<BKM, NL> sb;
        bool have = false;
        for (int tile = first; tile < ntiles; tile += tile_step) {
            int bm0, bn0;
            if (!have) {
                tile_origin(tile, bm0, bn0);
                sa.init(A, p.lda, p.M, p.K, bm0), sb.init(B, p.ldb, p.N, p.K, bn0), sa.init_offsets(2, w, lane), sb.init_offsets(1, w, lane);
                loader_prologue<AKM, BKM, NL>(sa, sb, smem, kt0, nt, p.K, w, lane);
            }
            k_loop_loader<AKM, BKM, NL>(sa, sb, smem, kt0, nt, p.K, w, lane);
            have = false;
            if (tile + tile_step < ntiles) {
                tile_origin(tile + tile_step, bm0, bn0);
                sa.init(A, p.lda, p.M, p.K, bm0), sb.init(B, p.ldb, p.N, p.K, bn0), sa.init_offsets(2, w, lane), sb.init_offsets(1, w, lane);
                loader_prologue<AKM, BKM, NL>(sa, sb, smem, kt0, nt, p.K, w, lane);
                have = true;
            }
        }
        return;
    }
    DirectEpi de;
    de.init(p, batch);
    constexpr int NOUT = EPI == 3 ? 2 : 1;
    [[maybe_unused]] Pending<NOUT> pend;
    for (int tile = first; tile < ntiles; tile += tile_step) {
        int bm0, bn0;
        tile_origin(tile, bm0, bn0);
        f32x16 acc[2][2];
#pragma unroll
        for (int i = 0; i < 2; ++i)
#pragma unroll
            for (int j = 0; j < 2; ++j)
#pragma unroll
                for (int r = 0; r < 16; ++r) acc[i][j][r] = 0.0f;
        [[maybe_unused]] PreRegs pre_in;
        if constexpr (EPI == 4) pre_load(p, de, bm0, bn0, wm, wn, lane, pre_in);
        k_loop_consumer<AKM, BKM>(smem, nt, wave, lane, wm, wn, acc);
        if constexpr (EPI == 4) {
            pending_fill_dact(p, pre_in, acc, pend, bm0, bn0, wm, wn, lane);
            pending_flush<1>(de, pend);
        } else if constexpr (EPI >= 2) {
// ... 169 lines not shown
    else if (!a_kmajor && b_kmajor)
        launch<false, true>(p, batch, s);
    else
        launch<true, true>(p, batch, s);
    if (det_ws && out_colsum) mmvid_slab_reduce(det_ws, nslab, N, out_colsum, s);
    if (det_ws && splitk > 1) {
        const long mn = (long)M * N;
        hipLaunchKernelGGL(splitk_reduce_kernel, dim3(cdiv(mn / 4, 256)), dim3(256), 0, s, det_ws, splitk, mn, out_f32, 1);
    }
    MMVID_LAUNCH_CHECK("gemm_bf16");
    return MMVID_OK;
}

extern "C" int mmvid_gemm_bf16(int a_kmajor, int b_kmajor, int M, int N, int K, const void* A, int64_t lda,
                               const void* B, int64_t ldb, int batch, int64_t strideA, int64_t strideB,
                               int64_t strideC, int splitk, float alpha, const float* bias, const float* residual,
                               int64_t ldr, const void* dact_pre, void* save_pre, int64_t ldp, int act,
                               int accumulate, float* out_f32, void* out_bf16, int64_t ldc, float* out_colsum,
                               void* stream) {
    return gemm_bf16_impl(a_kmajor, b_kmajor, M, N, K, A, lda, B, ldb, batch, strideA, strideB, strideC, splitk, alpha, bias, residual,
                          ldr, dact_pre, save_pre, ldp, act, accumulate, out_f32, out_bf16, ldc, out_colsum, nullptr, stream);
}

extern "C" int64_t mmvid_gemm_bf16_det_workspace_bytes(int M, int N, int splitk, int with_colsum) {
    if (splitk > 1) return (int64_t)splitk * M * N * 4;
    return with_colsum ? (int64_t)cdiv(M, 64) * N * 4 : 0;
}

extern "C" int mmvid_gemm_bf16_det(int a_kmajor, int b_kmajor, int M, int N, int K, const void* A, int64_t lda,
                                   const void* B, int64_t ldb, int batch, int64_t strideA, int64_t strideB,
                                   int64_t strideC, int splitk, float alpha, const float* bias, const float* residual,
                                   int64_t ldr, const void* dact_pre, void* save_pre, int64_t ldp, int act,
                                   int accumulate, float* out_f32, void* out_bf16, int64_t ldc, float* out_colsum,
                                   void* workspace, int64_t workspace_bytes, void* stream) {
    float* ws = nullptr;
    if (M > 0 && N > 0 && (splitk > 1 || out_colsum)) {
        const int64_t need = mmvid_gemm_bf16_det_workspace_bytes(M, N, splitk, out_colsum != nullptr);
        MMVID_REQUIRE(workspace && workspace_bytes >= need && ((uintptr_t)workspace & 15) == 0,
                      "gemm_bf16_det: a 16-byte aligned workspace of %lld bytes is needed (mmvid_gemm_bf16_det_workspace_bytes)",
                      (long long)need);
        ws = (float*)workspace;
    }
    return gemm_bf16_impl(a_kmajor, b_kmajor, M, N, K, A, lda, B, ldb, batch, strideA, strideB, strideC, splitk, alpha, bias, residual,
                          ldr, dact_pre, save_pre, ldp, act, accumulate, out_f32, out_bf16, ldc, out_colsum, ws, stream);
}

extern "C" int mmvid_gemm_dw_pick_splitk(int64_t M, int N, int K) {
    const long tiles = (long)cdiv(N, 256) * cdiv(K, BN);
    const long ktiles = cdiv(M, BK);
    long sk = tiles > 0 ? 256 / tiles : 1;
    if (sk > ktiles / 6) sk = ktiles / 6;
    if (sk > 16) sk = 16;
    if (sk < 1) sk = 1;
    return (int)sk;
}

extern "C" int mmvid_gemm_bf16_dw(int64_t M, int N, int K, const void* dY, int64_t ldy, const void* X, int64_t ldx,
                                  int splitk, float* workspace, float* dW, int accumulate, void* stream) {
    MMVID_REQUIRE(dY && X && dW && M > 0 && N > 0 && K > 0, "gemm_bf16_dw: bad arguments");
    MMVID_REQUIRE(N % 8 == 0 && K % 8 == 0 && ldy % 8 == 0 && ldx % 8 == 0, "gemm_bf16_dw: N, K, ldy, ldx must be multiples of 8");
    MMVID_REQUIRE(splitk >= 1 && (splitk == 1 || workspace), "gemm_bf16_dw: split-K needs a workspace");
    MMVID_REQUIRE(M * ldy * 2 < (1ll << 31) && M * ldx * 2 < (1ll << 31), "gemm_bf16_dw: an operand of 2 GiB or more");
    GemmParams p;
    p.A = (const bf16_t*)dY, p.B = (const bf16_t*)X;
    p.M = N, p.N = K, p.K = (int)M, p.lda = ldy, p.ldb = ldx;
    p.strideA = p.strideB = p.strideC = 0, p.splitk = splitk;
    p.bias = nullptr, p.residual = nullptr, p.ldr = 0, p.dact_pre = nullptr, p.save_pre = nullptr, p.ldp = 0;
    p.act = 0, p.accumulate = accumulate, p.alpha = 1.0f;
    p.out_f32 = dW, p.out_bf16 = nullptr, p.ldc = K;
    p.partial = splitk > 1 ? workspace : nullptr;
    p.colsum = nullptr, p.colsum_det = 0;
    p.tiles_n = p.tiles_m = 0, p.group_n = 0;
    hipStream_t s = (hipStream_t)stream;
    launch<true, true>(p, 1, s);
    if (splitk > 1) {
        const long mn = (long)N * K;
        hipLaunchKernelGGL(splitk_reduce_kernel, dim3(cdiv(mn / 4, 256)), dim3(256), 0, s, workspace, splitk, mn, dW, accumulate);
    }
    MMVID_LAUNCH_CHECK("gemm_bf16_dw");
    return MMVID_OK;
}

extern "C" int mmvid_gemm_bf16_dw_multi(int64_t M, int nkinds, const mmvid_dw_kind_t* kinds, int groups, int accumulate, void* stream) {
    MMVID_REQUIRE(kinds && M > 0 && nkinds > 0 && nkinds <= KIND_MAX && groups > 0, "gemm_bf16_dw_multi: bad arguments");
    using S = BlockShape<4>;
    static bool attr = false;
    if (!attr) {
        (void)hipFuncSetAttribute((const void*)gemm_bf16_lw_grouped_kernel, hipFuncAttributeMaxDynamicSharedMemorySize,
                                  (int)(S::LDS_BYTES + BIAS_LDS_BYTES));
        attr = true;
    }
    for (int k = 0; k < nkinds; ++k) {
        const mmvid_dw_kind_t& kd = kinds[k];
        MMVID_REQUIRE(kd.dY && kd.X && kd.dW_list && kd.N > 0 && kd.K > 0, "gemm_bf16_dw_multi: kind %d: null pointer / bad size", k);
        MMVID_REQUIRE(kd.N % 8 == 0 && kd.K % 8 == 0 && kd.ldy % 8 == 0 && kd.ldx % 8 == 0 && kd.strideY % 8 == 0 && kd.strideX % 8 == 0,
                      "gemm_bf16_dw_multi: kind %d: N, K, ldy, ldx and the group strides must be multiples of 8", k);
        MMVID_REQUIRE(M * kd.ldy * 2 < (1ll << 31) && M * kd.ldx * 2 < (1ll << 31), "gemm_bf16_dw_multi: an operand of 2 GiB or more per group");
        MMVID_REQUIRE((int64_t)kd.N * kd.K < (1ll << 29), "gemm_bf16_dw_multi: an output of 2 GiB or more");
    }
    const int per_launch = GROUP_MAX / nkinds;
    for (int g0 = 0; g0 < groups; g0 += per_launch) {
        const int n = groups - g0 < per_launch ? groups - g0 : per_launch;
        GroupTable gt;
        gt.n_kinds = nkinds;
        int tiles = 0;
        bool any = false;
        double flops = 0;
        for (int g = 0; g < GROUP_MAX; ++g) gt.out_list[g] = nullptr;
        for (int k = 0; k < KIND_MAX; ++k) {
            GroupKind& o = gt.kinds[k];
            if (k >= nkinds) {
                o = gt.kinds[0];
                o.first = 0x7fffffff;
                continue;
            }
            const mmvid_dw_kind_t& kd = kinds[k];
            o.A = (const unsigned short*)kd.dY + (int64_t)g0 * kd.strideY, o.B = (const unsigned short*)kd.X + (int64_t)g0 * kd.strideX;
            o.strideA = kd.strideY, o.strideB = kd.strideX, o.lda = kd.ldy, o.ldb = kd.ldx;
            o.M = kd.N, o.N = kd.K, o.tiles_n = cdiv(kd.K, BN), o.tiles_m = cdiv(kd.N, S::ROWS);
            o.first = tiles, o.out0 = k * n;
            o.colmajor = kd.K > kd.N ? 1 : 0;
            tiles += o.tiles_n * o.tiles_m * n;
            for (int g = 0; g < n; ++g) {
                gt.out_list[o.out0 + g] = kd.dW_list[g0 + g];
                if (kd.dW_list[g0 + g]) any = true, flops += 2.0 * M * kd.N * (double)kd.K;
            }
        }
        if (!any) continue;
        GemmParams p;
        p.A = gt.kinds[0].A, p.B = gt.kinds[0].B;
        p.M = gt.kinds[0].M, p.N = gt.kinds[0].N, p.K = (int)M, p.lda = gt.kinds[0].lda, p.ldb = gt.kinds[0].ldb;
        p.strideA = p.strideB = p.strideC = 0, p.splitk = 1;
        p.bias = nullptr, p.residual = nullptr, p.ldr = 0, p.dact_pre = nullptr, p.save_pre = nullptr, p.ldp = 0;
        p.act = 0, p.accumulate = accumulate, p.alpha = 1.0f;
        p.out_f32 = nullptr, p.out_bf16 = nullptr, p.ldc = gt.kinds[0].N;
        p.partial = nullptr, p.colsum = nullptr, p.colsum_det = 0;
        p.tiles_n = p.tiles_m = 0, p.group_n = 0;
        MmvidProfScope prof(PROF_GEMM_TN, flops, (hipStream_t)stream);
        hipLaunchKernelGGL(gemm_bf16_lw_grouped_kernel, dim3(tiles), dim3(512 + 64 * NLOAD), S::LDS_BYTES + BIAS_LDS_BYTES, (hipStream_t)stream, p, gt);
    }
    MMVID_LAUNCH_CHECK("gemm_bf16_dw_multi");
    return MMVID_OK;
}

extern "C" int mmvid_gemm_bf16_dw_grouped(int64_t M, int N, int K, const void* dY, int64_t ldy, int64_t strideY, const void* X,
                                          int64_t ldx, int64_t strideX, int groups, float* const* dW_list, int accumulate,
                                          void* stream) {
    mmvid_dw_kind_t kd;
    kd.N = N, kd.K = K, kd.dY = dY, kd.ldy = ldy, kd.strideY = strideY, kd.X = X, kd.ldx = ldx, kd.strideX = strideX, kd.dW_list = dW_list;
    return mmvid_gemm_bf16_dw_multi(M, 1, &kd, groups, accumulate, stream);
}

extern "C" double mmvid_gemm_dw_multi_fill(int nkinds, const mmvid_dw_kind_t* kinds, int groups) {
    long tiles = 0;
    for (int k = 0; k < nkinds; ++k) {
        long live = 0;
        for (int g = 0; g < groups; ++g) live += kinds[k].dW_list == nullptr || kinds[k].dW_list[g] != nullptr;
        tiles += (long)cdiv(kinds[k].N, 256) * cdiv(kinds[k].K, BN) * live;
    }
    const long rounds = cdiv(tiles, 256);
    return tiles > 0 ? (double)tiles / (double)(rounds * 256) : 0.0;
}
```

### mmvid_amd/csrc/tower.hip

```cpp
#include "../../include/mmvid_hip.h"
#include "common.h"
#include <vector>

#include "graphs.h"

namespace {

inline int64_t align256(int64_t x) { return (x + 255) & ~(int64_t)255; }
constexpr int kMaxSplitK = 16;
constexpr int kLnBwdBlocks = 512;

struct Dims {
    int B, L, E, H, F, layers;
    int64_t M;
};
Dims dims_of(const mmvid_tower_cfg_t& c) {
    Dims d;
    d.B = c.B, d.L = c.L, d.E = c.E, d.H = c.H, d.F = c.F, d.layers = c.layers;
    d.M = (int64_t)c.B * c.L;
    return d;
}

struct SavedLayer {
    int64_t x_in, x_mid, mean1, rstd1, mean2, rstd2, h1, qkv, o, lse2, h2, pre, act, k_gpj, k_dpre, k_gout, k_dqkv, k_ln1, k_ln2, total;
// ... 7 lines not shown
        return o;
    };
    s.x_in = take(d.M * d.E * 4);
    s.x_mid = take(d.M * d.E * 4);
    s.mean1 = take(d.M * 4), s.rstd1 = take(d.M * 4), s.mean2 = take(d.M * 4), s.rstd2 = take(d.M * 4);
    s.h1 = take(d.M * d.E * 2);
    s.qkv = take(d.M * 3 * d.E * 2);
    s.o = take(d.M * d.E * 2);
    s.lse2 = take((int64_t)d.B * d.H * d.L * 4);
    s.h2 = take(d.M * d.E * 2);
    s.pre = take(d.M * d.F * 2);
    s.act = take(d.M * d.F * 2);
    const int64_t keep = 1;
    s.k_gpj = take(keep * d.M * d.E * 2), s.k_dpre = take(keep * d.M * d.F * 2);
    s.k_gout = take(keep * d.M * d.E * 2), s.k_dqkv = take(keep * d.M * 3 * d.E * 2);
    s.k_ln1 = take(keep * (int64_t)kLnBwdBlocks * 3 * d.E * 4), s.k_ln2 = take(keep * (int64_t)kLnBwdBlocks * 3 * d.E * 4);
    s.total = off;
    return s;
}

struct Scratch {
    int64_t delta, d_h, d_o, splitk_ws, infer, total;
};
Scratch scratch_layout(const Dims& d) {
    Scratch s;
    int64_t off = 0;
    auto take = [&](int64_t bytes) {
        int64_t o = off;
        off += align256(bytes);
        return o;
    };
    s.delta = take((int64_t)d.B * d.H * d.L * 4);
    s.d_h = take(d.M * d.E * 2);
    s.d_o = take(d.M * d.E * 2);
    s.splitk_ws = take((int64_t)kMaxSplitK * d.F * d.E * 4);
    s.infer = take(saved_layout(d).total);
    s.total = off;
    return s;
}

int64_t det_slab_bytes(const Dims& d) {
    const int64_t a = mmvid_gemm_bf16_det_workspace_bytes((int)d.M, d.F, 1, 1);
    const int64_t b = mmvid_attention_bwd_bias_det_workspace_bytes(d.B, d.L, d.E);
    const int64_t c = mmvid_colsum_bf16_det_workspace_bytes(d.M, d.E);
    return a > b ? (a > c ? a : c) : (b > c ? b : c);
}

#define TRY(call)                   \
    do {                            \
        int rc__ = (call);          \
        if (rc__ != 0) return rc__; \
    } while (0)

int check_cfg(const mmvid_tower_cfg_t* c) {
    MMVID_REQUIRE(c, "tower: null config");
    MMVID_REQUIRE(c->B > 0 && c->L > 0 && c->layers > 0, "tower: bad B/L/layers");
    MMVID_REQUIRE(c->E == c->H * 64 && c->E % 8 == 0 && c->F % 8 == 0 && c->E <= 1024,
                  "tower: need E == 64*H <= 1024 and F %% 8 == 0 (E=%d H=%d F=%d)", c->E, c->H, c->F);
    return 0;
}

int linear_fwd(int64_t M, int N, int K, const void* X, const void* W, const float* bias, const float* residual,
               void* save_pre, int act, float* out_f32, void* out_bf16, void* st) {
    return mmvid_gemm_bf16(0, 0, (int)M, N, K, X, K, W, K, 1, 0, 0, 0, 1, 1.0f, bias, residual, N, nullptr, save_pre, N,
                           act, 0, out_f32, out_bf16, N, nullptr, st);
}
int linear_dx(int64_t M, int N, int K, const void* dY, const void* W, const void* dact_pre, float* out_f32,
              void* out_bf16, void* st, float* out_colsum = nullptr, void* det_ws = nullptr, int64_t det_bytes = 0) {
    if (out_colsum && det_ws)
        return mmvid_gemm_bf16_det(0, 1, (int)M, K, N, dY, N, W, K, 1, 0, 0, 0, 1, 1.0f, nullptr, nullptr, 0, dact_pre, nullptr, K,
                                   0, 0, out_f32, out_bf16, K, out_colsum, det_ws, det_bytes, st);
    return mmvid_gemm_bf16(0, 1, (int)M, K, N, dY, N, W, K, 1, 0, 0, 0, 1, 1.0f, nullptr, nullptr, 0, dact_pre, nullptr, K,
                           0, 0, out_f32, out_bf16, K, out_colsum, st);
}
int linear_dw(int64_t M, int N, int K, const void* dY, const void* X, float* dW, float* db, float* ws, void* st) {
    if (dW) {
        const int sk = mmvid_gemm_dw_pick_splitk(M, N, K);
        TRY(mmvid_gemm_bf16_dw(M, N, K, dY, N, X, K, sk, ws, dW, 1, st));
    }
    if (db) TRY(mmvid_colsum_bf16(dY, N, M, N, db, st));
    return 0;
}

}

extern "C" int mmvid_tower_workspace(const mmvid_tower_cfg_t* cfg, int64_t* saved_bytes, int64_t* scratch_bytes) {
    TRY(check_cfg(cfg));
    const Dims d = dims_of(*cfg);
    if (saved_bytes) *saved_bytes = saved_layout(d).total * d.layers;
    if (scratch_bytes) *scratch_bytes = scratch_layout(d).total;
    return MMVID_OK;
}

static int tower_forward_enqueue(const mmvid_tower_cfg_t* cfg, const mmvid_tower_layer_t* layers, const float* x_in,
                                 float* x_out, void* saved, void* scratch, void* stream, void* kv_cache = nullptr,
                                 int kv_lmax = 0);
static int tower_backward_enqueue(const mmvid_tower_cfg_t* cfg, const mmvid_tower_layer_t* layers, float* g,
                                  void* saved, void* scratch, void* stream);

static uint64_t tower_key(uint64_t seed, const mmvid_tower_cfg_t* cfg, const mmvid_tower_layer_t* layers, const void* a,
                          const void* b, const void* c, const void* d, const void* stream) {
    uint64_t k = mmvid_hash_bytes(cfg, sizeof(*cfg), 0xcbf29ce484222325ull ^ seed);
    k = mmvid_hash_bytes(layers, sizeof(mmvid_tower_layer_t) * (size_t)cfg->layers, k);
    return mmvid_hash_ptr(stream, mmvid_hash_ptr(d, mmvid_hash_ptr(c, mmvid_hash_ptr(b, mmvid_hash_ptr(a, k)))));
}

extern "C" int mmvid_tower_forward(const mmvid_tower_cfg_t* cfg, const mmvid_tower_layer_t* layers,
                                   const float* x_in, float* x_out, void* saved, void* scratch, void* stream) {
    TRY(check_cfg(cfg));
    MMVID_REQUIRE(layers && x_in && x_out && scratch, "tower_forward: null pointer");
    const uint64_t key = tower_key(2, cfg, layers, x_in, x_out, saved, scratch, stream);
    return mmvid_run_cached(key, (hipStream_t)stream, [=](hipStream_t s) {
        return tower_forward_enqueue(cfg, layers, x_in, x_out, saved, scratch, (void*)s);
    });
}

static int tower_forward_enqueue(const mmvid_tower_cfg_t* cfg, const mmvid_tower_layer_t* layers, const float* x_in,
                                 float* x_out, void* saved, void* scratch, void* stream, void* kv_cache, int kv_lmax) {
    const Dims d = dims_of(*cfg);
    const SavedLayer sl = saved_layout(d);
    const Scratch sc = scratch_layout(d);
    char* scr = (char*)scratch;
    const float scale = 0.125f;
    const float* x = x_in;
    for (int i = 0; i < d.layers; ++i) {
        const mmvid_tower_layer_t& ly = layers[i];
        char* sv = saved ? (char*)saved + (int64_t)i * sl.total : scr + sc.infer;
        float* xin_s = (float*)(sv + sl.x_in);
        float* xmid = (float*)(sv + sl.x_mid);
        if (saved && i == 0) {
            if (hipMemcpyAsync(xin_s, x_in, d.M * d.E * 4, hipMemcpyDeviceToDevice, (hipStream_t)stream) != hipSuccess) {
                mmvid_set_error("tower_forward: memcpy failed");
                return MMVID_ERR_HIP;
            }
            x = xin_s;
        }
        float* xnext;
        if (i == d.layers - 1)
            xnext = x_out;
        else if (saved)
            xnext = (float*)((char*)saved + (int64_t)(i + 1) * sl.total + sl.x_in);
        else
            xnext = x_out;
        TRY(mmvid_layernorm_fwd(x, d.E, d.M, d.E, ly.ln1_w, ly.ln1_b, cfg->ln_eps, sv + sl.h1, nullptr, d.E,
                                (float*)(sv + sl.mean1), (float*)(sv + sl.rstd1), stream));
        TRY(linear_fwd(d.M, 3 * d.E, d.E, sv + sl.h1, ly.in_w, ly.in_b, nullptr, nullptr, 0, nullptr, sv + sl.qkv, stream));
        if (kv_cache)
            TRY(mmvid_kv_store(sv + sl.qkv, 3 * d.E, d.B, d.L, d.E, nullptr, 0, kv_lmax,
                               (char*)kv_cache + (int64_t)i * d.B * kv_lmax * 2 * d.E * 2, stream));
        TRY(mmvid_attention_fwd(sv + sl.qkv, 3 * d.E, d.B, d.L, d.H, d.E, scale, cfg->mask_mode, cfg->r0, cfg->c0, cfg->r1,
                                cfg->c1, sv + sl.o, d.E, (float*)(sv + sl.lse2), stream));
        TRY(linear_fwd(d.M, d.E, d.E, sv + sl.o, ly.out_w, ly.out_b, x, nullptr, 0, xmid, nullptr, stream));
        TRY(mmvid_layernorm_fwd(xmid, d.E, d.M, d.E, ly.ln2_w, ly.ln2_b, cfg->ln_eps, sv + sl.h2, nullptr, d.E,
                                (float*)(sv + sl.mean2), (float*)(sv + sl.rstd2), stream));
        TRY(linear_fwd(d.M, d.F, d.E, sv + sl.h2, ly.fc_w, ly.fc_b, nullptr, saved ? sv + sl.pre : nullptr, 1, nullptr,
                       sv + sl.act, stream));
        TRY(linear_fwd(d.M, d.E, d.F, sv + sl.act, ly.pj_w, ly.pj_b, xmid, nullptr, 0, xnext, nullptr, stream));
        x = xnext;
    }
    return MMVID_OK;
}

extern "C" int mmvid_tower_backward(const mmvid_tower_cfg_t* cfg, const mmvid_tower_layer_t* layers, float* g,
                                    void* saved, void* scratch, void* stream) {
    TRY(check_cfg(cfg));
    MMVID_REQUIRE(layers && g && saved && scratch, "tower_backward: null pointer");
    const uint64_t key = tower_key(mmvid_option(MMVID_OPT_DETERMINISTIC) ? 5 : 3, cfg, layers, g, saved, scratch, nullptr, stream);
    return mmvid_run_cached(key, (hipStream_t)stream, [=](hipStream_t s) {
        return tower_backward_enqueue(cfg, layers, g, saved, scratch, (void*)s);
    });
}

static int tower_backward_enqueue(const mmvid_tower_cfg_t* cfg, const mmvid_tower_layer_t* layers, float* g, void* saved,
                                  void* scratch, void* stream) {
    const Dims d = dims_of(*cfg);
    const SavedLayer sl = saved_layout(d);
    const Scratch sc = scratch_layout(d);
    char* scr = (char*)scratch;
    char* keep = (char*)saved;
    struct { int64_t g_pj, d_pre, g_out, dqkv, total; } kl = {sl.k_gpj, sl.k_dpre, sl.k_gout, sl.k_dqkv, sl.total};
    const float scale = 0.125f;
    void* d_h = scr + sc.d_h;
    float* ws = (float*)(scr + sc.splitk_ws);
    void* det_ws = nullptr;
    const int64_t det_bytes = det_slab_bytes(d);
    if (mmvid_option(MMVID_OPT_DETERMINISTIC)) {
        MMVID_REQUIRE(det_bytes <= sc.total - sc.infer, "tower_backward: the deterministic slabs do not fit the scratch arena");
        det_ws = scr + sc.infer;
    }
    const int64_t ln_ws_floats = (int64_t)kLnBwdBlocks * 3 * d.E;
    std::vector<mmvid_ln_reduce_t> ln_items;
    int ln_blocks = 0;
    for (int i = d.layers - 1; i >= 0; --i) {
        const mmvid_tower_layer_t& ly = layers[i];
        const char* sv = (const char*)saved + (int64_t)i * sl.total;
        char* kp = keep + (int64_t)i * kl.total;
        void* g_pj = kp + kl.g_pj;
        if (i == d.layers - 1) {
            TRY(mmvid_cast_f32_to_bf16(g, g_pj, d.M * d.E, stream));
            if (ly.g_pj_b && det_ws) TRY(mmvid_colsum_bf16_det(g_pj, d.E, d.M, d.E, ly.g_pj_b, det_ws, det_bytes, stream));
            if (ly.g_pj_b && !det_ws) TRY(mmvid_colsum_bf16(g_pj, d.E, d.M, d.E, ly.g_pj_b, stream));
        }
        TRY(linear_dx(d.M, d.E, d.F, g_pj, ly.pj_w, sv + sl.pre, nullptr, kp + kl.d_pre, stream, ly.g_fc_b, det_ws, det_bytes));
        TRY(linear_dx(d.M, d.F, d.E, kp + kl.d_pre, ly.fc_w, nullptr, nullptr, d_h, stream));
        {
            mmvid_ln_reduce_t r = {(const float*)(kp + sl.k_ln2), ly.g_ln2_w, ly.g_ln2_b, ly.g_out_b};
            int nb = 0;
            TRY(mmvid_layernorm_bwd_partial(d_h, 1, d.E, (const float*)(sv + sl.x_mid), d.E, (const float*)(sv + sl.mean2),
                                            (const float*)(sv + sl.rstd2), ly.ln2_w, d.M, d.E, g, d.E, 1, kp + kl.g_out, r.dw != nullptr,
                                            r.db != nullptr, r.dx_colsum != nullptr, (float*)(kp + sl.k_ln2), ln_ws_floats, &nb, stream));
            if (r.dw || r.db || r.dx_colsum) ln_items.push_back(r), ln_blocks = nb;
        }
        TRY(linear_dx(d.M, d.E, d.E, kp + kl.g_out, ly.out_w, nullptr, nullptr, scr + sc.d_o, stream));
        if (det_ws)
            TRY(mmvid_attention_bwd_bias_det(sv + sl.qkv, 3 * d.E, sv + sl.o, d.E, scr + sc.d_o, d.E, (const float*)(sv + sl.lse2),
                                             (float*)(scr + sc.delta), d.B, d.L, d.H, d.E, scale, cfg->mask_mode, cfg->r0, cfg->c0,
                                             cfg->r1, cfg->c1, kp + kl.dqkv, 3 * d.E, ly.g_in_b, det_ws, det_bytes, stream));
        else
            TRY(mmvid_attention_bwd_bias(sv + sl.qkv, 3 * d.E, sv + sl.o, d.E, scr + sc.d_o, d.E, (const float*)(sv + sl.lse2),
                                         (float*)(scr + sc.delta), d.B, d.L, d.H, d.E, scale, cfg->mask_mode, cfg->r0, cfg->c0,
                                         cfg->r1, cfg->c1, kp + kl.dqkv, 3 * d.E, ly.g_in_b, stream));
        TRY(linear_dx(d.M, 3 * d.E, d.E, kp + kl.dqkv, ly.in_w, nullptr, nullptr, d_h, stream));
        {
            mmvid_ln_reduce_t r = {(const float*)(kp + sl.k_ln1), ly.g_ln1_w, ly.g_ln1_b, i > 0 ? layers[i - 1].g_pj_b : nullptr};
            int nb = 0;
            TRY(mmvid_layernorm_bwd_partial(d_h, 1, d.E, (const float*)(sv + sl.x_in), d.E, (const float*)(sv + sl.mean1),
                                            (const float*)(sv + sl.rstd1), ly.ln1_w, d.M, d.E, g, d.E, 1,
                                            i > 0 ? (void*)(keep + (int64_t)(i - 1) * kl.total + kl.g_pj) : nullptr, r.dw != nullptr,
                                            r.db != nullptr, r.dx_colsum != nullptr, (float*)(kp + sl.k_ln1), ln_ws_floats, &nb, stream));
            if (r.dw || r.db || r.dx_colsum) ln_items.push_back(r), ln_blocks = nb;
        }
    }
    if (!ln_items.empty()) TRY(mmvid_layernorm_bwd_reduce_multi((int)ln_items.size(), ln_items.data(), ln_blocks, d.E, stream));
    struct Kind {
        int N, K;
        int64_t dy_off, x_off;
        float* mmvid_tower_layer_t::*gw;
    };
    const Kind kinds[4] = {{d.E, d.F, kl.g_pj, sl.act, &mmvid_tower_layer_t::g_pj_w},
                           {d.F, d.E, kl.d_pre, sl.h2, &mmvid_tower_layer_t::g_fc_w},
                           {d.E, d.E, kl.g_out, sl.o, &mmvid_tower_layer_t::g_out_w},
                           {3 * d.E, d.E, kl.dqkv, sl.h1, &mmvid_tower_layer_t::g_in_w}};
    std::vector<float*> outs((size_t)d.layers * 4);
    mmvid_dw_kind_t kd[4];
    int nk = 0;
    for (const Kind& k : kinds) {
        float** o = outs.data() + (size_t)nk * d.layers;
        bool any = false;
        for (int i = 0; i < d.layers; ++i) o[i] = layers[i].*(k.gw), any = any || o[i];
        if (!any) continue;
        kd[nk].N = k.N, kd[nk].K = k.K;
        kd[nk].dY = keep + k.dy_off, kd[nk].ldy = k.N, kd[nk].strideY = kl.total / 2;
        kd[nk].X = (const char*)saved + k.x_off, kd[nk].ldx = k.K, kd[nk].strideX = sl.total / 2;
        kd[nk].dW_list = o;
        ++nk;
    }
    if (nk == 0) return MMVID_OK;
    if (mmvid_gemm_dw_multi_fill(nk, kd, d.layers) >= 0.7) return mmvid_gemm_bf16_dw_multi(d.M, nk, kd, d.layers, 1, stream);
    for (int k = 0; k < nk; ++k)
        for (int i = d.layers - 1; i >= 0; --i)
            TRY(linear_dw(d.M, kd[k].N, kd[k].K, (const char*)kd[k].dY + (int64_t)i * kl.total, (const char*)kd[k].X + (int64_t)i * sl.total,
                          kd[k].dW_list[i], nullptr, ws, stream));
    return MMVID_OK;
}

extern "C" int mmvid_tower_prefill(const mmvid_tower_cfg_t* cfg, const mmvid_tower_layer_t* layers, const float* x_in,
                                   float* x_out, void* kv_cache, int Lmax, void* scratch, void* stream) {
    TRY(check_cfg(cfg));
    MMVID_REQUIRE(layers && x_in && x_out && kv_cache && scratch, "tower_prefill: null pointer");
    MMVID_REQUIRE(cfg->mask_mode == 1 && cfg->L <= Lmax, "tower_prefill: needs the causal mask and L (%d) <= Lmax (%d)", cfg->L,
                  Lmax);
    return tower_forward_enqueue(cfg, layers, x_in, x_out, nullptr, scratch, stream, kv_cache, Lmax);
}

extern "C" int mmvid_tower_decode(const mmvid_tower_cfg_t* cfg, const mmvid_tower_layer_t* layers, const float* x_in,
                                  float* x_out, void* kv_cache, int Lmax, const int32_t* pos_dev, int pos, void* scratch,
                                  void* stream) {
    TRY(check_cfg(cfg));
    MMVID_REQUIRE(layers && x_in && x_out && kv_cache && scratch, "tower_decode: null pointer");
    MMVID_REQUIRE(cfg->mask_mode == 1, "tower_decode: incremental decoding needs the causal mask");
    const int B = cfg->B, E = cfg->E, F = cfg->F, H = cfg->H;
    char* p = (char*)scratch;
    auto take = [&](int64_t bytes) {
        char* o = p;
        p += align256(bytes);
        return o;
    };
    void* h = take((int64_t)B * E * 2);
    void* qkv = take((int64_t)B * 3 * E * 2);
    void* o = take((int64_t)B * E * 2);
    float* xmid = (float*)take((int64_t)B * E * 4);
    void* act = take((int64_t)B * F * 2);
    float* xa = (float*)take((int64_t)B * E * 4);
    float* xb = (float*)take((int64_t)B * E * 4);
    const float* x = x_in;
    for (int i = 0; i < cfg->layers; ++i) {
        const mmvid_tower_layer_t& ly = layers[i];
        void* cache = (char*)kv_cache + (int64_t)i * B * Lmax * 2 * E * 2;
        float* xnext = (i == cfg->layers - 1) ? x_out : ((i & 1) ? xb : xa);
        TRY(mmvid_layernorm_fwd(x, E, B, E, ly.ln1_w, ly.ln1_b, cfg->ln_eps, h, nullptr, E, nullptr, nullptr, stream));
        TRY(linear_fwd(B, 3 * E, E, h, ly.in_w, ly.in_b, nullptr, nullptr, 0, nullptr, qkv, stream));
        TRY(mmvid_kv_store(qkv, 3 * E, B, 1, E, pos_dev, pos, Lmax, cache, stream));
        TRY(mmvid_attention_decode(qkv, 3 * E, cache, B, Lmax, H, E, pos_dev, pos, 0.125f, o, E, stream));
        TRY(linear_fwd(B, E, E, o, ly.out_w, ly.out_b, x, nullptr, 0, xmid, nullptr, stream));
        TRY(mmvid_layernorm_fwd(xmid, E, B, E, ly.ln2_w, ly.ln2_b, cfg->ln_eps, h, nullptr, E, nullptr, nullptr, stream));
        TRY(linear_fwd(B, F, E, h, ly.fc_w, ly.fc_b, nullptr, nullptr, 1, nullptr, act, stream));
        TRY(linear_fwd(B, E, F, act, ly.pj_w, ly.pj_b, xmid, nullptr, 0, xnext, nullptr, stream));
        x = xnext;
    }
    return MMVID_OK;
}
```

### mmvid_amd/dalle_bert.py

```python
import torch
import torch.nn.functional as F
from torch import nn

from . import ops, sampling
from .clip_tower import OpenAICLIPTransformer
from .frontend import Frontend, face_choices
from .functional import PosTable, AssembleSequence, BertHeads, LNLinear, Linear, LayerNormRows
from .modules import AxialPositionalEmbedding, AxialPositionalEmbeddingList


def exists(val):
    return val is not None


def set_requires_grad(model, value):
    if model is not None:
        for p in model.parameters():
            p.requires_grad = value


def eval_decorator(fn):
    def inner(model, *args, **kwargs):
        was_training = model.training
        model.eval()
        out = fn(model, *args, **kwargs)
        model.train(was_training)
        return out

    return inner


class DivideMax(nn.Module):
    def __init__(self, dim):
        super().__init__()
        self.dim = dim

    def forward(self, x):
        return x / x.amax(dim=self.dim, keepdim=True)


class BERT(nn.Module):
    TEXT_ID_LOG_MAX = 16

    def __init__(self, *, dim, vae, cvae=None, num_text_tokens=10000, text_seq_len=256, stable=False,
                 text_feature_dim=0, fixed_language_model=None, which_transformer='none', num_visuals=1,
                 num_targets=1, use_separate_visual_emb=False, insert_sep=False, text_emb_bottleneck=False,
                 **kwargs):
        super().__init__()
        image_size = vae.image_size
        num_image_tokens = vae.num_tokens
        image_fmap_size = vae.image_size // (2**vae.num_layers)
        image_seq_len = image_fmap_size**2
        self.dim, self.num_visuals, self.num_targets = dim, num_visuals, num_targets
        self.random_erasing = dict(p=1.0, scale=(0.2, 0.8), ratio=(0.5, 2.0))
        self.visual_eraser = dict(p=0.95, scale=(0.55, 0.85), ratio=(0.5, 2.0))

        if fixed_language_model is None:
            num_text_tokens = num_text_tokens + text_seq_len
            self.text_emb = nn.Embedding(num_text_tokens, dim)
            self.text_pos_emb = nn.Embedding(text_seq_len, dim)
            self.text_feature_mapping = None
        else:
            assert text_feature_dim > 0
            text_seq_len, num_text_tokens = 1, 1
            self.text_emb = self.text_pos_emb = None
            if text_emb_bottleneck is not None:
                nf = int(text_emb_bottleneck)
                if nf <= 0 or nf % 8 or text_feature_dim % 8 or max(nf, text_feature_dim, dim) > 1024:
                    raise ValueError(f'text_emb_bottleneck={text_emb_bottleneck!r}, text_feature_dim={text_feature_dim}: the mapping '
                                     'kernels take widths that are multiples of 8, at most 1024 (pass text_emb_bottleneck=None '
                                     'for the single Linear)')
                self.text_feature_mapping = nn.Sequential(nn.LayerNorm(text_feature_dim), nn.Linear(text_feature_dim, nf),
                                                          nn.LayerNorm(nf), nn.Linear(nf, dim), nn.LayerNorm(dim))
            else:
                if text_feature_dim % 8:
                    raise ValueError(f'text_feature_dim={text_feature_dim} must be a multiple of 8')
                self.text_feature_mapping = nn.Linear(text_feature_dim, dim)
            self.register_buffer('_no_text_row', torch.zeros(1, dim), persistent=False)
        self.text_feature_dim = text_feature_dim
        self.image_emb = nn.Embedding(num_image_tokens + 2, dim)
        self.target_pos_emb = AxialPositionalEmbedding(dim, axial_shape=(num_targets, image_fmap_size, image_fmap_size))
        if cvae is not None:
# ... 59 lines not shown
    def _w16(self, lin):
        w = lin.weight
        c = self._w16_cache.get(id(lin))
        if c is not None and c[0] == 'attached':
            if c[2] == w.data_ptr():
                if c[3] != w._version:
                    ops.cast_bf16(w.detach().contiguous(), c[1])
                    self._w16_cache[id(lin)] = ('attached', c[1], c[2], w._version)
                return c[1]
            c = None
        key = (w._version, w.data_ptr())
        if c is None or c[0] != key:
            c = (key, ops.cast_bf16(w.detach().contiguous()))
            self._w16_cache[id(lin)] = c
        return c[1]

    def attach_head_shadow(self, lin, view):
        self._w16_cache[id(lin)] = ('attached', view, lin.weight.data_ptr(), lin.weight._version)

    def head_shadow_targets(self):
        m = self.text_feature_mapping
        extra = [] if m is None else ([m] if isinstance(m, nn.Linear) else [m[1], m[3]])
        return [self.to_logits[1]] + extra

    def _tables(self):
        vis = self.visual_emb.weight if (self.num_visuals > 0 and self.visual_emb is not None) else self.image_emb.weight
        text = self.text_emb.weight if self.text_emb is not None else self._no_text_row
        return (self.special_emb.weight, text, vis, self.image_emb.weight)

    def sparse_grad_rows(self):
        if self.text_emb is None:
            return {}
        log = self._text_id_log
        if not log or self._text_id_overflow:
            return {'text_emb.weight': None}
        return {'text_emb.weight': log[0] if len(log) == 1 else torch.cat(log)}

    def _note_table_backward(self, _g):
        self.table_grad_pending = True

    table_grad_pending = False

    def reset_sparse_grad_rows(self):
        self._text_id_log, self._text_id_overflow = [], False

    def _log_text_ids(self, ids):
        if not torch.is_grad_enabled() or self.text_emb is None:
            return
        if len(self._text_id_log) >= self.TEXT_ID_LOG_MAX:
            self._text_id_overflow = True
            return
        self._text_id_log.append(ids[:, 1:1 + self.text_seq_len].reshape(-1))

    def _pos_layout(self):
        sp, f = self.special_pos_emb.weight, self.image_fmap_size
        text_pos = self.text_pos_emb.weight if self.text_pos_emb is not None else self._no_text_row
        lay = [(0, 1, 0, (sp, ), ()), (1, self.text_seq_len, 0, (text_pos, ), ())]
        at = 1 + self.text_seq_len
        if self.num_visuals > 0:
            for m in self.visual_pos_emb.module_list:
                lay.append((at, f * f, 0, (m.weights_0, m.weights_1), (f, f)))
                at += f * f + (1 if self.insert_sep else 0)
        lay.append((at, 2, 1, (sp, ), ()))
        at += 2
        tp, T = self.target_pos_emb, self.num_targets
        lay.append((at, T * f * f, 0, (tp.weights_0, tp.weights_1, tp.weights_2), (T, f, f)))
        return lay, at + T * f * f

    def _pos_table(self):
        sp = self.special_pos_emb.weight
        if sp.is_cuda:
            lay, L = self._pos_layout()
            params = [w for seg in lay for w in seg[3]]
            return PosTable.apply(lay, L, *params)
        parts = [sp[0:1], (self.text_pos_emb.weight if self.text_pos_emb is not None else self._no_text_row)[:self.text_seq_len]]
        if self.num_visuals > 0:
            parts.append(self.visual_pos_emb.table(insert_sep=bool(self.insert_sep)))
        parts += [sp[1:3], self.target_pos_emb.table()]
        return torch.cat(parts, 0)

    def get_special_token(self, tok_list, batch_size=1, device='cuda'):
        return torch.tensor(tok_list, dtype=torch.long, device=device).repeat(batch_size, 1)

    def transformer_forward(self, tokens):
        out = self.transformer(tokens)
        if self.stable:
            out = self.norm_by_max(out)
        return out

    def to_logits_rows(self, x):
        shp = x.shape
        lin = self.to_logits[1]
        y = LNLinear.apply(x.reshape(-1, shp[-1]), self.to_logits[0].weight, self.to_logits[0].bias, lin.weight,
                           lin.bias, self._w16(lin))
        return y.view(*shp[:-1], -1)

    def get_image_tokens(self, image, reshape=True, insert_sep=False, which_vae='vae'):
        vae = self.cvae if (which_vae == 'cvae' and self.cvae is not None) else self.vae
        if isinstance(image, list):
            assert len(image[0].shape) == 4, 'image should be list of 4d image tensors'
            image = torch.stack(image, dim=1)
        if len(image.shape) == 4:
            image = image.unsqueeze(1)
        if len(image.shape) == 5:
            b, t, c, h, w = image.shape
            s = vae.image_size
            assert (c, h, w) == (3, s, s), f'invalid image of dimensions {image.shape} passed in during training'
            image = vae.get_codebook_indices(image.reshape(b * t, c, h, w))
            if reshape:
                if insert_sep:
                    image = image.view(b, t, -1)
                    sep = torch.full((b, t, 1), self.image_token_lut['[SEP]'], device=image.device, dtype=torch.long)
                    image = torch.cat((image, sep), dim=2).reshape(b, -1)
                else:
                    image = image.view(b, -1)
        return image

    @torch.no_grad()
    def recon_images(self, images, which_vae='vae'):
        vae = self.cvae if (which_vae == 'cvae' and self.cvae is not None) else self.vae
        return vae.decode(self.get_image_tokens(images, reshape=False, which_vae=which_vae))

    @torch.no_grad()
    def get_codebook_emb(self, images, which_vae='vae'):
        b, t = images.shape[:2]
        img_seq = self.get_image_tokens(images, reshape=False, which_vae=which_vae)
        img_code = img_seq.view(b, t, -1)
        return img_code, ops.gather_rows(self.image_emb.weight.detach(), img_code.contiguous())

    def swap_one_frame_along_batch(self, tokens, t=1):
        b, n, c = tokens.shape
        out = tokens.detach().clone().reshape(b, t, n // t, c)
        rows = torch.arange(b, device=tokens.device)
        idx = torch.randint(0, t, (b, ), device=tokens.device)
        picked = out[rows, idx]
        h = (b + 1) // 2
        out[rows, idx] = torch.cat((picked[h:], picked[:h]), 0)
        return out.reshape(b, n, c)

    def decode_images(self, img_seq):
        return self.vae.decode(img_seq.reshape(-1, self.image_seq_len))

    def decode_masks(self, mask):
        f = self.image_fmap_size
        patch = self.image_size // f
        up = mask.reshape(-1, 1, f, f).repeat_interleave(patch, 2).repeat_interleave(patch, 3)
        return F.pad(up, (0, 0, 0, 0, 0, 2))

    def random_erase_codebook(self, image, eraser, erase_half=False):
        f = self.image_fmap_size
        image = image.contiguous()
        tv = image.shape[1] // (f * f)
        return self.frontend.random_erase(image, tv, f, self.image_token_lut['[MASK]'], eraser['p'], eraser['scale'],
                                          eraser['ratio'], erase_half)

    def erase_codebook_face(self, image, vc_mode, face_mode=None):
        f = self.image_fmap_size
        image = image.contiguous()
        tv = image.shape[1] // (f * f)
        choices, frame0 = face_choices(vc_mode, face_mode)
        return self.frontend.erase_choice(image, tv, f, self.image_token_lut['[MASK]'], choices, frame0)

    def _visual_tokens(self, visual, erase_visual, erase_visual_half, vc_mode, face_mode, visual_aug_mode):
        if self.num_visuals == 0 or not (exists(visual) and len(visual)):
            return None
        if visual_aug_mode == 'motion_color' and torch.is_tensor(visual) and visual.dim() == 5:
            visual = self.frontend.visual_color_jitter(visual, 0.9, 1)
        tok = self.get_image_tokens(visual, insert_sep=self.insert_sep, which_vae='cvae')
# ... 65 lines not shown
        B = text.shape[0]
        text_rows = None
        if self.fixed_language_model is None:
            assert text.shape[-1] == self.text_seq_len, \
                f'the length {text.shape[-1]} of the text tokens you passed in does not have the correct length ({self.text_seq_len})'
            text = ops._chk(text.contiguous(), torch.int64, 'text')
        else:
            if negvc:
                raise NotImplementedError('negvc with a fixed language model: the reference indexes a text table it does not '
                                          'have in this mode (dalle_bert.py:930-932)')
            assert text.dim() == 2 and text.shape[-1] == self.text_feature_dim, \
                f'expected text features of shape [B, {self.text_feature_dim}], got {tuple(text.shape)}'
            text_rows = self._map_text_feature(ops._chk(text.contiguous().float(), torch.float32, 'text'))
            text = torch.zeros(B, 1, dtype=torch.int64, device=device)
        MASK = self.image_token_lut['[MASK]']
        pad_base = self.num_text_tokens - self.text_seq_len
        vis_tok = self._visual_tokens(visual, erase_visual, erase_visual_half, vc_mode, face_mode, visual_aug_mode)
        if not return_loss:
            empty = torch.empty(B, 0, dtype=torch.long, device=device)
            ids = ops.bert_build_ids(text, vis_tok, self.visual_seq_len, empty, None, torch.empty(B, 0, dtype=torch.uint8, device=device),
                                     pad_base, MASK, False, False)[0]
            self.frontend.advance(device)
            self._log_text_ids(ids)
            return self._assemble(ids, self.control_seq_len, text_rows)

        T, f = self.num_targets, self.image_fmap_size
        do_vid = vid and T > 1
        if _mask1 is None:
            mask1, not_fully_masked = self.frontend.msm_masks(B, T, f, device, msm_strategy_prob, msm_bernoulli_prob, pc_prob)
        else:
            mask1 = _mask1.to(device=device, dtype=torch.uint8).contiguous()
            not_fully_masked = kwargs.get('_not_fully_masked', torch.ones(B, device=device))
        target_warp = None
        if do_vid and torch.is_tensor(target) and target.dim() == 5 and _target_warp is None:
            frames = ops._chk(target.contiguous().float(), torch.float32, 'target')
            _, _, C, H, W = frames.shape
            both = torch.empty(B * T + B, C, H, W, device=device, dtype=torch.float32)
            both[:B * T].copy_(frames.view(B * T, C, H, W))
            self.frontend.vid_warp_new_frames(frames, vid_strategy_prob, both[B * T:])
            toks = self.vae.get_codebook_indices(both)
            target = toks[:B * T].reshape(B, -1).contiguous()
            target_warp = self.frontend.vid_warp_tokens(target, toks[B * T:], T)
        elif do_vid and torch.is_tensor(target) and target.dim() == 5:
            both = torch.empty((2 * B, ) + tuple(target.shape[1:]), device=device, dtype=torch.float32)
            both[:B].copy_(target)
            both[B:].copy_(_target_warp)
            toks = self.get_image_tokens(both)
            target, target_warp = toks[:B].contiguous(), toks[B:].contiguous()
        else:
            token_target = torch.is_tensor(target) and target.dim() == 2 and not target.is_floating_point()
            target = self.get_image_tokens(target).contiguous()
            if do_vid and _target_warp is None and token_target:
                target_warp = self._token_target_negative(target, target_frames, vid_strategy_prob)
            elif do_vid:
                tw = _target_warp if _target_warp is not None else target
                target_warp = self.get_image_tokens(tw.to(device)).contiguous()
        self.frontend.advance(device)

        if rel:
            assert B >= 2 and B % 2 == 0
        text_neg_ids = None
        if rel and negvc:
            text_neg_ids = ops._chk(text_neg.contiguous(), torch.int64, 'text_neg')
        ids, sel, tfull, cnt = ops.bert_build_ids(text, vis_tok, self.visual_seq_len, target, target_warp, mask1, pad_base, MASK,
                                                  bool(rel), bool(do_vid), text_neg=text_neg_ids)
        self._log_text_ids(ids)
        if text_rows is not None and (rel or do_vid):
            half = B // 2
            per_pass = [text_rows] + ([torch.cat((text_rows[half:], text_rows[:half]))] if rel else []) + \
                ([text_rows] if do_vid else [])
            text_rows = torch.cat(per_pass)
        x_seq = self._assemble(ids, self.total_seq_len, text_rows)
        if text_neg_ids is not None and self.num_visuals > 0 and self.visual_seq_len > 0:
            L = self.total_seq_len
            v0 = 1 + self.text_seq_len
            keep = torch.cat((torch.arange(0, v0, device=device), torch.arange(v0 + self.visual_seq_len, L, device=device)))
            x_neg = x_seq[B:2 * B].index_select(1, keep).contiguous()
            x_main = torch.cat((x_seq[:B], x_seq[2 * B:])) if do_vid else x_seq[:B]
            y_main = self.transformer_forward(x_main.contiguous())
            y_neg = self.transformer_forward(x_neg)
            y_rel = torch.zeros(B, L, y_neg.shape[-1], device=device, dtype=y_neg.dtype).index_copy(1, keep, y_neg)
            y = torch.cat((y_main[:B], y_rel, y_main[B:])) if do_vid else torch.cat((y_main, y_rel))
        else:
            y = self.transformer_forward(x_seq)
        if self._debug_keep is not None:
            self._debug_keep.update(mask1=mask1, nfm=not_fully_masked, target=target, target_warp=target_warp, ids=ids, sel=sel,
                                    tfull=tfull, cnt=cnt, x_seq=x_seq, y=y)
        nseq = 1 + int(bool(rel)) + int(bool(do_vid))
        rows, labels = self._head_rows(B, nseq, device)
        lin = self.to_logits[1]
        loss_msm, loss_rel, loss_vid, logits = BertHeads.apply(
            y, tfull, sel, cnt, not_fully_masked, labels, rows['rel'][1] if rel else None,
            rows['vid'][nseq - 1] if do_vid else None, bool(rel_no_fully_masked), B, self._w16(lin),
            self.to_logits[0].weight, self.to_logits[0].bias, lin.weight, lin.bias,
            self.to_logits_rel[0].weight, self.to_logits_rel[0].bias, self.to_logits_rel[1].weight, self.to_logits_rel[1].bias,
            self.to_logits_vid[0].weight, self.to_logits_vid[0].bias, self.to_logits_vid[1].weight, self.to_logits_vid[1].bias)
        self._last_logits_msm = logits.view(B, self.total_seq_len, -1)[:, self.control_seq_len:]
        return loss_msm, loss_rel, loss_vid

    @torch.no_grad()
    @eval_decorator
    def generate_images(self, text, *, visual=None, mask=None, img=None, argmax=False, dynamic=True, debug=False,
                        erase_visual=False, mask_predict_steps=10, preserve=None, t_overlap=1, pc_mode=None,
                        vc_mode=None, face_mode=None, mp_config=None, long_mode='long', **kwargs):
        control_emb = self(text, visual=visual, erase_visual=erase_visual, erase_visual_half=True, vc_mode=vc_mode,
                           face_mode=face_mode, return_loss=False)
        img_seq, pnag_samples = self.mask_predict(control_emb, argmax=argmax, dynamic=dynamic, debug=debug,
                                                  steps=mask_predict_steps, preserve=preserve, t_overlap=t_overlap,
                                                  pc_mode=pc_mode, mp_config=mp_config, long_mode=long_mode, **kwargs)
        img_seq = img_seq.reshape(-1, self.image_seq_len)
        images = self.vae.decode(img_seq)
        return images.view(-1, self.num_targets, *images.shape[1:]), pnag_samples, img_seq

    @torch.no_grad()
    def mask_predict(self, control_emb, dynamic=True, debug=False, steps=10, preserve=None, t_overlap=1,
                     mp_config=None, long_mode='long', _race=None, _trace=None, **kwargs):
        return sampling.mask_predict(self, control_emb, dynamic=dynamic, debug=debug, steps=steps, preserve=preserve,
                                     t_overlap=t_overlap, mp_config=mp_config, long_mode=long_mode, race=_race, trace=_trace)
```

### mmvid_amd/ops.py

```python
import ctypes

import torch

from . import _lib
from ._lib import call

bf16, f32, i64 = torch.bfloat16, torch.float32, torch.int64


def _stream():
    return ctypes.c_void_p(torch.cuda.current_stream().cuda_stream)


def _p(t):
    if t is None:
        return None
    return ctypes.c_void_p(t.data_ptr())


_DET_WS = {}


def _det_ws(op, device, nbytes):
    key = (op, str(device), int(nbytes))
# ... 73 lines not shown
    _chk(table, torch.uint16, 'table'), _chk(frame_index, i64, 'frame_index')
    n = table.shape[1]
    out = torch.empty(*frame_index.shape[:-1], frame_index.shape[-1] * n, device=table.device, dtype=i64)
    call('mmvid_token_rows_gather', _p(table), table.shape[0], _p(frame_index), frame_index.numel(), n, _p(out), _stream())
    return out


def gemm(A, B, *, a_kmajor=False, b_kmajor=False, bias=None, residual=None, dact_pre=None, save_pre=None, act=0,
         out_dtype=bf16, out=None, accumulate=False, splitk=1, alpha=1.0, colsum=None):
    _chk(A, bf16, 'A'), _chk(B, bf16, 'B')
    batch = 1
    sA = sB = 0
    if A.dim() == 3:
        batch = A.shape[0]
        sA, sB = A.stride(0), B.stride(0)
        A2, B2 = A[0], B[0]
    else:
        A2, B2 = A, B
    K, M = (A2.shape if a_kmajor else A2.shape[::-1])
    Kb, N = (B2.shape if b_kmajor else B2.shape[::-1])
    assert K == Kb, (A.shape, B.shape)
    if out is None:
        shape = (batch, M, N) if A.dim() == 3 else (M, N)
        out = torch.empty(shape, device=A.device, dtype=out_dtype)
    sC = M * N if batch > 1 else 0
    is32 = out.dtype == f32
    for t, n in ((bias, 'bias'), (residual, 'residual')):
        if t is not None:
            _chk(t, f32, n)
    if _lib.is_deterministic() and (colsum is not None or splitk > 1):
        nb = _lib.load().mmvid_gemm_bf16_det_workspace_bytes(M, N, splitk, int(colsum is not None))
        ws = _det_ws('gemm_bf16', A.device, nb)
        call('mmvid_gemm_bf16_det', int(a_kmajor), int(b_kmajor), M, N, K, _p(A), A2.stride(0), _p(B), B2.stride(0), batch,
             sA, sB, sC, splitk, float(alpha), _p(bias), _p(residual), N, _p(dact_pre), _p(save_pre), N, act,
             int(accumulate), _p(out) if is32 else None, None if is32 else _p(out), N, _p(colsum), _p(ws), ws.numel(), _stream())
        return out
    call('mmvid_gemm_bf16', int(a_kmajor), int(b_kmajor), M, N, K, _p(A), A2.stride(0), _p(B), B2.stride(0), batch,
         sA, sB, sC, splitk, float(alpha), _p(bias), _p(residual), N, _p(dact_pre), _p(save_pre), N, act,
         int(accumulate), _p(out) if is32 else None, None if is32 else _p(out), N, _p(colsum), _stream())
    return out


def gemm_dw(dY, X, dW, accumulate=True, splitk=None):
    _chk(dY, bf16, 'dY'), _chk(X, bf16, 'X'), _chk(dW, f32, 'dW')
    M, N = dY.shape
    K = X.shape[1]
    if splitk is None:
        splitk = _lib.load().mmvid_gemm_dw_pick_splitk(M, N, K)
    ws = torch.empty(splitk * N * K, device=dY.device, dtype=f32) if splitk > 1 else None
    call('mmvid_gemm_bf16_dw', M, N, K, _p(dY), N, _p(X), K, splitk, _p(ws), _p(dW), int(accumulate), _stream())
    return dW


def gemm_dw_grouped(dY, X, dWs, accumulate=True):
    _chk(dY, bf16, 'dY'), _chk(X, bf16, 'X')
    G, M, N = dY.shape
    K = X.shape[2]
    assert X.shape[:2] == (G, M) and len(dWs) == G
    ptrs = (ctypes.c_void_p * G)(*[(_chk(w, f32, 'dW').data_ptr() if w is not None else None) for w in dWs])
    call('mmvid_gemm_bf16_dw_grouped', M, N, K, _p(dY), dY.stride(1), dY.stride(0), _p(X), X.stride(1), X.stride(0), G, ptrs,
         int(accumulate), _stream())
    return dWs


def _dw_kinds(kinds):
    arr = (_lib.DwKind * len(kinds))()
    keep = []
    G, M = kinds[0][0].shape[:2]
    for a, (dY, X, dWs) in zip(arr, kinds):
        _chk(dY, bf16, 'dY'), _chk(X, bf16, 'X')
        assert dY.shape[:2] == (G, M) and X.shape[:2] == (G, M) and len(dWs) == G
        ptrs = (ctypes.c_void_p * G)(*[(_chk(w, f32, 'dW').data_ptr() if w is not None else None) for w in dWs])
        keep.append(ptrs)
        a.N, a.K, a.dY, a.ldy, a.strideY = dY.shape[2], X.shape[2], dY.data_ptr(), dY.stride(1), dY.stride(0)
        a.X, a.ldx, a.strideX, a.dW_list = X.data_ptr(), X.stride(1), X.stride(0), ctypes.cast(ptrs, ctypes.c_void_p)
    return arr, keep, M, G


def gemm_dw_multi(kinds, accumulate=True):
    arr, keep, M, G = _dw_kinds(kinds)
    call('mmvid_gemm_bf16_dw_multi', M, len(kinds), arr, G, int(accumulate), _stream())


def gemm_dw_multi_fill(shapes, groups):
    arr = (_lib.DwKind * len(shapes))()
    for a, (N, K) in zip(arr, shapes):
        a.N, a.K, a.dW_list = N, K, None
    return _lib.load().mmvid_gemm_dw_multi_fill(len(shapes), arr, groups)


def gemm_f32(A, B, *, b_kmajor=False, bias=None, residual=None, alpha=1.0):
    _chk(A, f32, 'A'), _chk(B, f32, 'B')
    M, K = A.shape
    N = B.shape[1] if b_kmajor else B.shape[0]
    out = torch.empty(M, N, device=A.device, dtype=f32)
    call('mmvid_gemm_f32', int(b_kmajor), M, N, K, _p(A), K, _p(B), B.shape[1], 1, 0, 0, 0, float(alpha), _p(bias),
         _p(residual), _p(out), N, _stream())
    return out


def layernorm_fwd(x, w, b, eps=1e-5, out_dtype=bf16, save_stats=True):
    _chk(x, f32, 'x')
    rows, E = x.numel() // x.shape[-1], x.shape[-1]
    y = torch.empty(x.shape, device=x.device, dtype=out_dtype)
    mean = torch.empty(rows, device=x.device, dtype=f32) if save_stats else None
    rstd = torch.empty(rows, device=x.device, dtype=f32) if save_stats else None
    call('mmvid_layernorm_fwd', _p(x), E, rows, E, _p(w), _p(b), float(eps), _p(y) if out_dtype == bf16 else None,
         _p(y) if out_dtype == f32 else None, E, _p(mean), _p(rstd), _stream())
    return y, mean, rstd


def layernorm_bwd(dy, x, mean, rstd, w, dx=None, add=False, dw=None, db=None, dx_colsum=None, workspace=None):
    _chk(dy, f32, 'dy'), _chk(x, f32, 'x')
    rows, E = x.numel() // x.shape[-1], x.shape[-1]
    if dx is None:
        dx = torch.empty_like(x)
        add = False
    if workspace is None and _lib.is_deterministic() and (dw is not None or db is not None or dx_colsum is not None):
        workspace = _det_ws('layernorm_bwd', x.device, 512 * 3 * E * 4).view(f32)
    call('mmvid_layernorm_bwd_ws', _p(dy), E, _p(x), E, _p(mean), _p(rstd), _p(w), rows, E, _p(dx), E, int(add), None,
         _p(dw), _p(db), _p(dx_colsum), _p(workspace), workspace.numel() if workspace is not None else 0, _stream())
    return dx


def layernorm_bwd_partial(dy, x, mean, rstd, w, workspace, dx=None, add=False, dx_bf16=None, want=(True, True, True)):
    _chk(x, f32, 'x'), _chk(workspace, f32, 'workspace')
    rows, E = x.numel() // x.shape[-1], x.shape[-1]
    if dx is None:
        dx, add = torch.empty_like(x), False
    nb = ctypes.c_int()
    call('mmvid_layernorm_bwd_partial', _p(dy), int(dy.dtype == bf16), E, _p(x), E, _p(mean), _p(rstd), _p(w), rows, E, _p(dx), E, int(add),
         _p(dx_bf16), int(want[0]), int(want[1]), int(want[2]), _p(workspace), workspace.numel(), ctypes.byref(nb), _stream())
    return dx, nb.value


def layernorm_bwd_reduce_multi(items, blocks, E):
    arr = (_lib.LnReduce * len(items))()
    for a, (ws, dw, db, cs) in zip(arr, items):
        a.partial, a.dw, a.db, a.dx_colsum = ws.data_ptr(), _p(dw), _p(db), _p(cs)
    call('mmvid_layernorm_bwd_reduce_multi', len(items), arr, blocks, E, _stream())


def gn_stats_buffer(N, hw, C, device):
    return torch.empty(N * (2 * C + 64 * ((hw + 63) // 64)), device=device, dtype=f32)


def conv3x3_strip(x, w, bias, residual=None, out_dtype=bf16, also_bf16=False, gn_stats=None):
    _chk(x, bf16, 'x'), _chk(w, bf16, 'w')
    N, H, W, Cin = x.shape
    Cout = w.shape[0]
    out = torch.empty(N, H, W, Cout, device=x.device, dtype=out_dtype)
    o16 = torch.empty(N, H, W, Cout, device=x.device, dtype=bf16) if (also_bf16 and out_dtype == f32) else None
    rb = residual if (residual is not None and residual.dtype == bf16) else None
    rf = residual if (residual is not None and residual.dtype == f32) else None
    gp = ctypes.c_void_p(gn_stats.data_ptr() + N * Cout * 2 * 4) if gn_stats is not None else None
    call('mmvid_conv3x3_strip_nhwc', _p(x), N, H, W, Cin, _p(w), _p(bias), Cout, _p(rb), _p(rf),
         _p(out) if out_dtype == bf16 else _p(o16), _p(out) if out_dtype == f32 else None, gp, _stream())
    return (out, o16) if o16 is not None else out


def groupnorm_swish(x, w, b, eps=1e-6, swish=True, out_dtype=bf16, stats=None, stats_block=128):
    N, H, W, C = x.shape
    assert x.is_contiguous() and x.dtype in (bf16, f32)
    blocks = 0
    if stats is None:
        stats = gn_stats_buffer(N, H * W, C, x.device)
# ... 367 lines not shown
```

Baseline: 213,200.

## Prune last tower layer to prefix rows for auxiliary rel/vid sequences

For the auxiliary relevance and video-discriminator sequences only a prefix of token rows feeds the heads, so the final transformer layer now computes attention queries, MLP and weight gradients only for those prefix rows, while full sequences keep the whole work. New row-limited attention forward and backward entry points, a row-masked dW multi-GEMM, and top-layer forward/backward paths with row copies are added. This adds complexity, extra copies and memsets, and is enabled by default through an environment variable when the model is not in stable mode.

```diff
diff --git a/include/mmvid_hip.h b/include/mmvid_hip.h
--- a/include/mmvid_hip.h
+++ b/include/mmvid_hip.h
@@ -40,6 +40,8 @@
 int mmvid_gemm_bf16_dw_grouped(int64_t M, int N, int K, const void* dY, int64_t ldy, int64_t strideY, const void* X, int64_t ldx,
                                int64_t strideX, int groups, float* const* dW_list, int accumulate, void* stream);
 double mmvid_gemm_dw_multi_fill(int nkinds, const mmvid_dw_kind_t* kinds, int groups);
+int mmvid_gemm_bf16_dw_multi_rows(int64_t M, int nkinds, const mmvid_dw_kind_t* kinds, int groups, const int32_t* rows, int accumulate,
+                                  void* stream);
 
 int mmvid_layernorm_fwd(const float* x, int64_t ldx, int64_t rows, int E, const float* w, const float* b, float eps,
                         void* y_bf16, float* y_f32, int64_t ldy, float* mean, float* rstd, void* stream);
@@ -75,6 +77,11 @@
 int mmvid_attention_bwd_bias(const void* qkv, int64_t ld, const void* O, int64_t ldo, const void* dO, int64_t lddo,
                              const float* lse2, float* delta, int B, int L, int H, int E, float scale, int mask_mode, int r0,
                              int c0, int r1, int c1, void* dqkv, int64_t ldg, float* dbias, void* stream);
+int mmvid_attention_fwd_rows(const void* qkv, int64_t ld, int B, int L, int H, int E, float scale, int mask_mode, int r0, int c0,
+                             int r1, int c1, int q_rows, void* out, int64_t ldo, float* lse2, void* stream);
+int mmvid_attention_bwd_bias_rows(const void* qkv, int64_t ld, const void* O, int64_t ldo, const void* dO, int64_t lddo,
+                                  const float* lse2, float* delta, int B, int L, int H, int E, float scale, int mask_mode, int r0,
+                                  int c0, int r1, int c1, int q_rows, void* dqkv, int64_t ldg, float* dbias, void* stream);
 int mmvid_assemble_sequence(const float* const* tables, const int64_t* table_rows, int ntables, const int64_t* ids,
                             const int32_t* seg, const float* pos, int64_t B, int L, int E, float* out, void* stream);
 int mmvid_assemble_sequence_bwd(float* const* grad_tables, const int64_t* table_rows, int ntables,
@@ -178,6 +185,10 @@
                         float* x_out, void* saved, void* scratch, void* stream);
 int mmvid_tower_backward(const mmvid_tower_cfg_t* cfg, const mmvid_tower_layer_t* layers, float* g,
                          void* saved, void* scratch, void* stream);
+int mmvid_tower_forward_top(const mmvid_tower_cfg_t* cfg, const mmvid_tower_layer_t* layers, const float* x_in, float* x_out,
+                            void* saved, void* scratch, int full_seqs, int prefix_rows, void* stream);
+int mmvid_tower_backward_top(const mmvid_tower_cfg_t* cfg, const mmvid_tower_layer_t* layers, float* g, void* saved, void* scratch,
+                             int full_seqs, int prefix_rows, void* stream);
 
 
 int mmvid_tower_prefill(const mmvid_tower_cfg_t* cfg, const mmvid_tower_layer_t* layers, const float* x_in,
diff --git a/mmvid_amd/_lib.py b/mmvid_amd/_lib.py
--- a/mmvid_amd/_lib.py
+++ b/mmvid_amd/_lib.py
@@ -57,6 +57,7 @@
     'mmvid_gemm_dw_pick_splitk': [I64, I, I],
     'mmvid_gemm_bf16_dw_grouped': [I64, I, I, P, I64, I64, P, I64, I64, I, P, I, P],
     'mmvid_gemm_bf16_dw_multi': [I64, I, P, I, I, P],
+    'mmvid_gemm_bf16_dw_multi_rows': [I64, I, P, I, P, I, P],
     'mmvid_layernorm_fwd': [P, I64, I64, I, P, P, F, P, P, I64, P, P, P],
     'mmvid_layernorm_bwd': [P, I64, P, I64, P, P, P, I64, I, P, I64, I, P, P, P, P, P],
     'mmvid_layernorm_bwd_ws': [P, I64, P, I64, P, P, P, I64, I, P, I64, I, P, P, P, P, P, I64, P],
@@ -67,6 +68,8 @@
     'mmvid_attention_fwd': [P, I64, I, I, I, I, F, I, I, I, I, I, P, I64, P, P],
     'mmvid_attention_bwd': [P, I64, P, I64, P, I64, P, P, I, I, I, I, F, I, I, I, I, I, P, I64, P],
     'mmvid_attention_bwd_bias': [P, I64, P, I64, P, I64, P, P, I, I, I, I, F, I, I, I, I, I, P, I64, P, P],
+    'mmvid_attention_bwd_bias_rows': [P, I64, P, I64, P, I64, P, P, I, I, I, I, F, I, I, I, I, I, I, P, I64, P, P],
+    'mmvid_attention_fwd_rows': [P, I64, I, I, I, I, F, I, I, I, I, I, I, P, I64, P, P],
     'mmvid_assemble_sequence': [POINTER(P), POINTER(I64), I, P, P, P, I64, I, I, P, P],
     'mmvid_assemble_sequence_bwd': [POINTER(P), POINTER(I64), I, P, P, P, I64, I, I, P, I, P],
     'mmvid_cross_entropy_fwd': [P, I64, P, P, I64, I, P, P, P],
@@ -78,6 +81,8 @@
     'mmvid_tower_workspace': [POINTER(TowerCfg), POINTER(I64), POINTER(I64)],
     'mmvid_tower_forward': [POINTER(TowerCfg), POINTER(TowerLayer), P, P, P, P, P],
     'mmvid_tower_backward': [POINTER(TowerCfg), POINTER(TowerLayer), P, P, P, P],
+    'mmvid_tower_forward_top': [POINTER(TowerCfg), POINTER(TowerLayer), P, P, P, P, I, I, P],
+    'mmvid_tower_backward_top': [POINTER(TowerCfg), POINTER(TowerLayer), P, P, P, I, I, P],
     'mmvid_tower_prefill': [POINTER(TowerCfg), POINTER(TowerLayer), P, P, P, I, P, P],
     'mmvid_tower_decode': [POINTER(TowerCfg), POINTER(TowerLayer), P, P, P, I, P, I, P, P],
     'mmvid_tower_decode_fused': [POINTER(TowerCfg), POINTER(TowerLayer), P, P, P, I, P, I, P, P],
diff --git a/mmvid_amd/clip_tower.py b/mmvid_amd/clip_tower.py
--- a/mmvid_amd/clip_tower.py
+++ b/mmvid_amd/clip_tower.py
@@ -58,10 +58,11 @@
 
 class _TowerFn(torch.autograd.Function):
     @staticmethod
-    def forward(ctx, x, tower, keep, *params):
-        _note_params(ctx, (x, tower, keep) + params)
+    def forward(ctx, x, tower, keep, top_rows, *params):
+        _note_params(ctx, (x, tower, keep, top_rows) + params)
         ctx.tower = tower
-        y, saved = tower._run_forward(x, keep=keep)
+        ctx.top_rows = top_rows
+        y, saved = tower._run_forward(x, keep=keep, top_rows=top_rows)
         ctx.saved_arena = saved
         ctx.shape = x.shape
         return y
@@ -69,9 +70,9 @@
     @staticmethod
     def backward(ctx, gy):
         g = gy.contiguous().clone()
-        ctx.tower._run_backward(g, ctx.saved_arena, ctx.shape)
+        ctx.tower._run_backward(g, ctx.saved_arena, ctx.shape, top_rows=ctx.top_rows)
         ctx.saved_arena = None
-        return _with_param_zeros(ctx, (g.view(ctx.shape), None, None) + (None, ) * (len(ctx.needs_input_grad) - 3))
+        return _with_param_zeros(ctx, (g.view(ctx.shape), None, None, None) + (None, ) * (len(ctx.needs_input_grad) - 4))
 
 
 class DecodeSession:
@@ -206,10 +207,12 @@
         own = {k[len(prefix):]: v.float() for k, v in sd.items() if k.startswith(prefix + 'resblocks.')}
         self.transformer.load_state_dict(own)
 
-    def forward(self, x, **kwargs):
+    def forward(self, x, top_rows=None, **kwargs):
         assert x.dim() == 3 and x.shape[-1] == self.width
         keep = torch.is_grad_enabled() and (x.requires_grad or self._any_trainable())
-        return _TowerFn.apply(x, self, keep, *self.parameters())
+        if top_rows is not None:
+            top_rows = (int(top_rows[0]), int(top_rows[1]))
+        return _TowerFn.apply(x, self, keep, top_rows, *self.parameters())
 
     def new_kv_cache(self, B, max_len, device):
         assert self.mask_spec == 'causal', 'incremental decoding needs the causal mask'
@@ -320,15 +323,19 @@
         saved = torch.empty(sb.value, device=device, dtype=torch.uint8) if keep else None
         return saved, self._scratch
 
-    def _run_forward(self, x, keep):
+    def _run_forward(self, x, keep, top_rows=None):
         x = ops._chk(x.contiguous(), torch.float32, 'tower input')
         B, L, _ = x.shape
         cfg = self._cfg(B, L)
         layers, _keep = self._layer_structs(False)
         saved, scratch = self._workspace(cfg, x.device, keep)
         y = torch.empty_like(x)
-        _lib.call('mmvid_tower_forward', ctypes.byref(cfg), layers, ops._p(x), ops._p(y), ops._p(saved), ops._p(scratch),
-                  ops._stream())
+        if top_rows is None:
+            _lib.call('mmvid_tower_forward', ctypes.byref(cfg), layers, ops._p(x), ops._p(y), ops._p(saved), ops._p(scratch),
+                      ops._stream())
+        else:
+            _lib.call('mmvid_tower_forward_top', ctypes.byref(cfg), layers, ops._p(x), ops._p(y), ops._p(saved), ops._p(scratch),
+                      top_rows[0], top_rows[1], ops._stream())
         if self.debug_keep_saved:
             self._last_saved = saved
         return y, saved
@@ -360,7 +367,7 @@
             self._chunk_plan = (self.layers, plan)
         return self._chunk_plan[1]
 
-    def _run_backward(self, g, saved, shape):
+    def _run_backward(self, g, saved, shape, top_rows=None):
         if saved is None:
             raise _lib.MMVIDError('tower backward without saved activations (forward ran under no_grad)')
         B, L, _ = shape
@@ -377,7 +384,11 @@
             sub = self._cfg(B, L)
             sub.layers = hi - lo
             lp = ctypes.cast(ctypes.byref(layers, lo * ctypes.sizeof(_lib.TowerLayer)), ctypes.POINTER(_lib.TowerLayer))
-            _lib.call('mmvid_tower_backward', ctypes.byref(sub), lp, ops._p(g),
-                      ctypes.c_void_p(saved.data_ptr() + lo * per_layer), ops._p(scratch), ops._stream())
+            if top_rows is not None and hi == self.layers:
+                _lib.call('mmvid_tower_backward_top', ctypes.byref(sub), lp, ops._p(g),
+                          ctypes.c_void_p(saved.data_ptr() + lo * per_layer), ops._p(scratch), top_rows[0], top_rows[1], ops._stream())
+            else:
+                _lib.call('mmvid_tower_backward', ctypes.byref(sub), lp, ops._p(g),
+                          ctypes.c_void_p(saved.data_ptr() + lo * per_layer), ops._p(scratch), ops._stream())
             if self.on_layers_done is not None:
                 self.on_layers_done(lo)
diff --git a/mmvid_amd/csrc/attn.hip b/mmvid_amd/csrc/attn.hip
--- a/mmvid_amd/csrc/attn.hip
+++ b/mmvid_amd/csrc/attn.hip
@@ -547,8 +547,8 @@
 
 template <bool DET>
 __global__ __launch_bounds__(256, 3) void attn_bwd_dkv_kernel(const bf16_t* __restrict__ qkv, long ld, const bf16_t* __restrict__ dO, long lddo,
-                                                               const float* __restrict__ lse2, const float* __restrict__ delta, int L, int H,
-                                                               int E, FastDiv nrt_d, FastDiv h_d, float scale, float scale_log2,
+                                                               const float* __restrict__ lse2, const float* __restrict__ delta, int L, int q_rows,
+                                                               int H, int E, FastDiv nrt_d, FastDiv h_d, float scale, float scale_log2,
                                                                float inv_scale_log2, MaskSpec mask, bf16_t* __restrict__ dqkv, long ldg,
                                                                float* __restrict__ dbias) {
     __shared__ __attribute__((aligned(16))) char dsm[2][DKV_BUF];
@@ -559,7 +559,7 @@
     const bf16_t* dObase = dO + (long)b * L * lddo + hd * 64;
     const float* lse_b = lse2 + ((long)b * H + hd) * L;
     const float* del_b = delta + ((long)b * H + hd) * L;
-    const int nq_tiles = (L + 63) >> 6;
+    const int nq_tiles = (q_rows + 63) >> 6;
     const RowLane rl = row_lane_offs(lane);
     const TrLane trq = tr_lane_at(tr_lane_offs(lane), lds_addr(dsm[0]));
     const int key_wave0 = kt * ROWS_PER_BLOCK + wave * 32;
@@ -695,13 +695,19 @@
 
 extern "C" int mmvid_attention_fwd(const void* qkv, int64_t ld, int B, int L, int H, int E, float scale, int mask_mode,
                                    int r0, int c0, int r1, int c1, void* out, int64_t ldo, float* lse2, void* stream) {
+    return mmvid_attention_fwd_rows(qkv, ld, B, L, H, E, scale, mask_mode, r0, c0, r1, c1, L, out, ldo, lse2, stream);
+}
+
+extern "C" int mmvid_attention_fwd_rows(const void* qkv, int64_t ld, int B, int L, int H, int E, float scale, int mask_mode, int r0,
+                                        int c0, int r1, int c1, int q_rows, void* out, int64_t ldo, float* lse2, void* stream) {
     MMVID_REQUIRE(qkv && out && lse2, "attention_fwd: null pointer");
+    MMVID_REQUIRE(q_rows >= 1 && q_rows <= L, "attention_fwd_rows: q_rows %d outside [1, L]", q_rows);
     ATTN_COMMON_CHECKS("attention_fwd");
     MMVID_REQUIRE(ld % 8 == 0 && ldo % 8 == 0 && ((uintptr_t)out & 15) == 0, "attention_fwd: leading dims must be multiples of 8, out 16-byte aligned");
     MMVID_REQUIRE((int64_t)L * ld * 2 < (1ll << 31), "attention_fwd: one batch entry of qkv must be smaller than 2 GiB");
     hipStream_t s = (hipStream_t)stream;
-    MmvidProfScope prof(PROF_ATTN_FWD, 4.0 * B * H * (double)L * L * 64, s);
-    const int nrt = cdiv(L, ROWS_PER_BLOCK), nblocks = nrt * H * B;
+    MmvidProfScope prof(PROF_ATTN_FWD, 4.0 * B * H * (double)q_rows * L * 64, s);
+    const int nrt = cdiv(q_rows, ROWS_PER_BLOCK), nblocks = nrt * H * B;
     const FastDiv nrt_d = make_fastdiv(nrt), h_d = make_fastdiv(H);
     const MaskSpec m = make_mask(mask_mode, r0, c0, r1, c1);
     hipLaunchKernelGGL(attn_fwd_kernel<false>, dim3(nblocks), dim3(256), 0, s, (const bf16_t*)qkv, (long)ld, L, H, E, nrt_d, h_d,
@@ -738,9 +744,11 @@
 
 static int attention_bwd_impl(const void* qkv, int64_t ld, const void* O, int64_t ldo, const void* dO, int64_t lddo,
                                         const float* lse2, float* delta, int B, int L, int H, int E, float scale,
-                                        int mask_mode, int r0, int c0, int r1, int c1, void* dqkv, int64_t ldg,
+                                        int mask_mode, int r0, int c0, int r1, int c1, int q_rows, void* dqkv, int64_t ldg,
                                         float* dbias, float* det_slab, void* stream) {
     MMVID_REQUIRE(qkv && O && dO && lse2 && delta && dqkv, "attention_bwd: null pointer");
+    MMVID_REQUIRE(q_rows >= 1 && q_rows <= L && (q_rows == L || mask_mode != 1),
+                  "attention_bwd_bias_rows: q_rows %d outside [1, L], or below L with the causal mask", q_rows);
     ATTN_COMMON_CHECKS("attention_bwd");
     MMVID_REQUIRE(ld % 8 == 0 && ldo % 8 == 0 && lddo % 8 == 0 && ldg % 8 == 0 && ((uintptr_t)dqkv & 15) == 0,
                   "attention_bwd: leading dims must be multiples of 8, dqkv 16-byte aligned");
@@ -749,27 +757,29 @@
     hipStream_t s = (hipStream_t)stream;
     const MaskSpec m = make_mask(mask_mode, r0, c0, r1, c1);
     const float sl2 = scale * 1.4426950408889634f;
-    MmvidProfScope prof(PROF_ATTN_BWD, 10.0 * B * H * (double)L * L * 64, s);
+    MmvidProfScope prof(PROF_ATTN_BWD, 10.0 * B * H * (double)q_rows * L * 64, s);
     const int nrt = cdiv(L, ROWS_PER_BLOCK), nblocks = nrt * H * B;
     const FastDiv nrt_d = make_fastdiv(nrt), h_d = make_fastdiv(H);
+    const int nrt_q = cdiv(q_rows, ROWS_PER_BLOCK), nblocks_q = nrt_q * H * B;
+    const FastDiv nrt_q_d = make_fastdiv(nrt_q);
     if (dbias && det_slab) {
         const int nslab = B * nrt * 4;
         if (hipMemsetAsync(det_slab, 0, (size_t)nslab * 3 * E * 4, s) != hipSuccess) {
             mmvid_set_error("attention_bwd_bias_det: memset failed");
             return MMVID_ERR_HIP;
         }
-        hipLaunchKernelGGL(attn_bwd_dq_kernel<true>, dim3(nblocks), dim3(256), 0, s, (const bf16_t*)qkv, (long)ld, (const bf16_t*)O, (long)ldo,
-                           (const bf16_t*)dO, (long)lddo, lse2, delta, L, H, E, nrt_d, h_d, scale, sl2, m, (bf16_t*)dqkv, (long)ldg, det_slab);
+        hipLaunchKernelGGL(attn_bwd_dq_kernel<true>, dim3(nblocks_q), dim3(256), 0, s, (const bf16_t*)qkv, (long)ld, (const bf16_t*)O, (long)ldo,
+                           (const bf16_t*)dO, (long)lddo, lse2, delta, L, H, E, nrt_q_d, h_d, scale, sl2, m, (bf16_t*)dqkv, (long)ldg, det_slab);
         hipLaunchKernelGGL(attn_bwd_dkv_kernel<true>, dim3(nblocks), dim3(256), 0, s, (const bf16_t*)qkv, (long)ld, (const bf16_t*)dO, (long)lddo,
-                           lse2, delta, L, H, E, nrt_d, h_d, scale, sl2, 1.0f / sl2, m, (bf16_t*)dqkv, (long)ldg, det_slab);
+                           lse2, delta, L, q_rows, H, E, nrt_d, h_d, scale, sl2, 1.0f / sl2, m, (bf16_t*)dqkv, (long)ldg, det_slab);
         mmvid_slab_reduce(det_slab, nslab, 3 * E, dbias, s);
         MMVID_LAUNCH_CHECK("attention_bwd_bias_det");
         return MMVID_OK;
     }
-    hipLaunchKernelGGL(attn_bwd_dq_kernel<false>, dim3(nblocks), dim3(256), 0, s, (const bf16_t*)qkv, (long)ld, (const bf16_t*)O, (long)ldo,
-                       (const bf16_t*)dO, (long)lddo, lse2, delta, L, H, E, nrt_d, h_d, scale, sl2, m, (bf16_t*)dqkv, (long)ldg, dbias);
+    hipLaunchKernelGGL(attn_bwd_dq_kernel<false>, dim3(nblocks_q), dim3(256), 0, s, (const bf16_t*)qkv, (long)ld, (const bf16_t*)O, (long)ldo,
+                       (const bf16_t*)dO, (long)lddo, lse2, delta, L, H, E, nrt_q_d, h_d, scale, sl2, m, (bf16_t*)dqkv, (long)ldg, dbias);
     hipLaunchKernelGGL(attn_bwd_dkv_kernel<false>, dim3(nblocks), dim3(256), 0, s, (const bf16_t*)qkv, (long)ld, (const bf16_t*)dO, (long)lddo, lse2,
-                       delta, L, H, E, nrt_d, h_d, scale, sl2, 1.0f / sl2, m, (bf16_t*)dqkv, (long)ldg, dbias);
+                       delta, L, q_rows, H, E, nrt_d, h_d, scale, sl2, 1.0f / sl2, m, (bf16_t*)dqkv, (long)ldg, dbias);
     MMVID_LAUNCH_CHECK("attention_bwd");
     return MMVID_OK;
 }
@@ -778,8 +788,16 @@
                                         const float* lse2, float* delta, int B, int L, int H, int E, float scale,
                                         int mask_mode, int r0, int c0, int r1, int c1, void* dqkv, int64_t ldg,
                                         float* dbias, void* stream) {
-    return attention_bwd_impl(qkv, ld, O, ldo, dO, lddo, lse2, delta, B, L, H, E, scale, mask_mode, r0, c0, r1, c1, dqkv, ldg, dbias,
+    return attention_bwd_impl(qkv, ld, O, ldo, dO, lddo, lse2, delta, B, L, H, E, scale, mask_mode, r0, c0, r1, c1, L, dqkv, ldg, dbias,
                               nullptr, stream);
+}
+
+extern "C" int mmvid_attention_bwd_bias_rows(const void* qkv, int64_t ld, const void* O, int64_t ldo, const void* dO, int64_t lddo,
+                                             const float* lse2, float* delta, int B, int L, int H, int E, float scale, int mask_mode,
+                                             int r0, int c0, int r1, int c1, int q_rows, void* dqkv, int64_t ldg, float* dbias,
+                                             void* stream) {
+    return attention_bwd_impl(qkv, ld, O, ldo, dO, lddo, lse2, delta, B, L, H, E, scale, mask_mode, r0, c0, r1, c1, q_rows, dqkv, ldg,
+                              dbias, nullptr, stream);
 }
 
 extern "C" int64_t mmvid_attention_bwd_bias_det_workspace_bytes(int B, int L, int E) {
@@ -794,6 +812,6 @@
         MMVID_REQUIRE(workspace && B > 0 && L > 0 && workspace_bytes >= mmvid_attention_bwd_bias_det_workspace_bytes(B, L, E),
                       "attention_bwd_bias_det: workspace of %lld bytes needed (mmvid_attention_bwd_bias_det_workspace_bytes)",
                       (long long)mmvid_attention_bwd_bias_det_workspace_bytes(B, L, E));
-    return attention_bwd_impl(qkv, ld, O, ldo, dO, lddo, lse2, delta, B, L, H, E, scale, mask_mode, r0, c0, r1, c1, dqkv, ldg, dbias,
+    return attention_bwd_impl(qkv, ld, O, ldo, dO, lddo, lse2, delta, B, L, H, E, scale, mask_mode, r0, c0, r1, c1, L, dqkv, ldg, dbias,
                               (float*)workspace, stream);
 }
diff --git a/mmvid_amd/csrc/gemm.hip b/mmvid_amd/csrc/gemm.hip
--- a/mmvid_amd/csrc/gemm.hip
+++ b/mmvid_amd/csrc/gemm.hip
@@ -47,6 +47,7 @@
     int n_kinds;
     GroupKind kinds[KIND_MAX];
     float* out_list[GROUP_MAX];
+    int rows[GROUP_MAX];
 };
 __device__ __forceinline__ float sigmoid1702(float x) {
     return __builtin_amdgcn_rcpf(1.0f + __builtin_amdgcn_exp2f(-1.702f * 1.4426950408889634f * x));
@@ -508,6 +509,8 @@
         p.strideA = p.strideB = p.strideC = 0;
         p.M = kd.M, p.N = kd.N, p.lda = kd.lda, p.ldb = kd.ldb, p.ldc = kd.N;
         p.out_f32 = out;
+        const int rows = gt->rows[kd.out0 + g];
+        if (rows > 0) p.K = rows;
     }
     extern __shared__ __attribute__((aligned(16))) char smem[];
     const int tid = threadIdx.x;
@@ -843,7 +846,15 @@
 }
 
 extern "C" int mmvid_gemm_bf16_dw_multi(int64_t M, int nkinds, const mmvid_dw_kind_t* kinds, int groups, int accumulate, void* stream) {
+    return mmvid_gemm_bf16_dw_multi_rows(M, nkinds, kinds, groups, nullptr, accumulate, stream);
+}
+
+extern "C" int mmvid_gemm_bf16_dw_multi_rows(int64_t M, int nkinds, const mmvid_dw_kind_t* kinds, int groups, const int32_t* rows,
+                                             int accumulate, void* stream) {
     MMVID_REQUIRE(kinds && M > 0 && nkinds > 0 && nkinds <= KIND_MAX && groups > 0, "gemm_bf16_dw_multi: bad arguments");
+    if (rows)
+        for (int i = 0; i < nkinds * groups; ++i)
+            MMVID_REQUIRE(rows[i] >= 0 && rows[i] <= M, "gemm_bf16_dw_multi_rows: rows[%d] = %d outside [0, M]", i, (int)rows[i]);
     using S = BlockShape<4>;
     static bool attr = false;
     if (!attr) {
@@ -867,7 +878,7 @@
         int tiles = 0;
         bool any = false;
         double flops = 0;
-        for (int g = 0; g < GROUP_MAX; ++g) gt.out_list[g] = nullptr;
+        for (int g = 0; g < GROUP_MAX; ++g) gt.out_list[g] = nullptr, gt.rows[g] = 0;
         for (int k = 0; k < KIND_MAX; ++k) {
             GroupKind& o = gt.kinds[k];
             if (k >= nkinds) {
@@ -884,7 +895,9 @@
             tiles += o.tiles_n * o.tiles_m * n;
             for (int g = 0; g < n; ++g) {
                 gt.out_list[o.out0 + g] = kd.dW_list[g0 + g];
-                if (kd.dW_list[g0 + g]) any = true, flops += 2.0 * M * kd.N * (double)kd.K;
+                const int r = rows ? rows[k * groups + g0 + g] : 0;
+                gt.rows[o.out0 + g] = r;
+                if (kd.dW_list[g0 + g]) any = true, flops += 2.0 * (r > 0 ? r : M) * kd.N * (double)kd.K;
             }
         }
         if (!any) continue;
diff --git a/mmvid_amd/csrc/tower.hip b/mmvid_amd/csrc/tower.hip
--- a/mmvid_amd/csrc/tower.hip
+++ b/mmvid_amd/csrc/tower.hip
@@ -113,6 +113,56 @@
     return 0;
 }
 
+struct TopRows {
+    int fs = 0, P = 0;
+    bool on() const { return P > 0; }
+};
+struct TopDims {
+    int64_t Mf, Mp, R;
+    int nP, T;
+};
+TopDims top_dims(const Dims& d, const TopRows& t) {
+    TopDims o;
+    o.nP = d.B - t.fs;
+    o.Mf = (int64_t)t.fs * d.L, o.Mp = (int64_t)o.nP * t.P, o.R = o.Mf + o.Mp;
+    o.T = (t.P + 127) / 128 * 128 < d.L ? (t.P + 127) / 128 * 128 : d.L;
+    return o;
+}
+int check_top(const mmvid_tower_cfg_t* c, int full_seqs, int prefix_rows) {
+    MMVID_REQUIRE(full_seqs >= 0 && full_seqs <= c->B && prefix_rows >= 1 && prefix_rows <= c->L,
+                  "tower (top rows): need 0 <= full_seqs (%d) <= B (%d) and 1 <= prefix_rows (%d) <= L (%d)", full_seqs, c->B, prefix_rows, c->L);
+    return 0;
+}
+bool top_wanted(const mmvid_tower_cfg_t* c, const void* saved, int full_seqs, int prefix_rows) {
+    return saved && full_seqs < c->B && prefix_rows < c->L && c->mask_mode != 1 && !mmvid_option(MMVID_OPT_DETERMINISTIC);
+}
+
+__global__ __launch_bounds__(256) void copy_rows_kernel(uint4* __restrict__ dst, long dst_stride, const uint4* __restrict__ src,
+                                                        long src_stride, long copy, long total, long n) {
+    const long idx = (long)blockIdx.x * 256 + threadIdx.x;
+    if (idx >= n * total) return;
+    const long i = idx / total, c = idx - i * total;
+    dst[i * dst_stride + c] = (src && c < copy) ? src[i * src_stride + c] : make_uint4(0u, 0u, 0u, 0u);
+}
+int copy_rows(void* dst, int64_t dst_stride, const void* src, int64_t src_stride, int64_t copy, int64_t total, int64_t n, void* stream) {
+    MMVID_REQUIRE(((dst_stride | src_stride | copy | total) & 15) == 0 && (((uintptr_t)dst | (uintptr_t)src) & 15) == 0 && copy <= total,
+                  "tower (top rows): row copies need 16-byte multiples");
+    if (n <= 0 || total <= 0) return MMVID_OK;
+    const int64_t units = n * (total / 16);
+    MMVID_REQUIRE((units + 255) / 256 < (1ll << 31), "tower (top rows): row copy too large");
+    hipLaunchKernelGGL(copy_rows_kernel, dim3((unsigned)((units + 255) / 256)), dim3(256), 0, (hipStream_t)stream, (uint4*)dst, (long)(dst_stride / 16),
+                       (const uint4*)src, (long)(src_stride / 16), (long)(copy / 16), (long)(total / 16), (long)n);
+    MMVID_LAUNCH_CHECK("tower copy_rows");
+    return MMVID_OK;
+}
+int copy_d2d(void* dst, const void* src, int64_t bytes, void* stream) {
+    if (bytes > 0 && hipMemcpyAsync(dst, src, (size_t)bytes, hipMemcpyDeviceToDevice, (hipStream_t)stream) != hipSuccess) {
+        mmvid_set_error("tower (top rows): memcpy failed");
+        return MMVID_ERR_HIP;
+    }
+    return MMVID_OK;
+}
+
 }
 
 extern "C" int mmvid_tower_workspace(const mmvid_tower_cfg_t* cfg, int64_t* saved_bytes, int64_t* scratch_bytes) {
@@ -125,9 +175,9 @@
 
 static int tower_forward_enqueue(const mmvid_tower_cfg_t* cfg, const mmvid_tower_layer_t* layers, const float* x_in,
                                  float* x_out, void* saved, void* scratch, void* stream, void* kv_cache = nullptr,
-                                 int kv_lmax = 0);
+                                 int kv_lmax = 0, TopRows top = TopRows());
 static int tower_backward_enqueue(const mmvid_tower_cfg_t* cfg, const mmvid_tower_layer_t* layers, float* g,
-                                  void* saved, void* scratch, void* stream);
+                                  void* saved, void* scratch, void* stream, TopRows top = TopRows());
 
 static uint64_t tower_key(uint64_t seed, const mmvid_tower_cfg_t* cfg, const mmvid_tower_layer_t* layers, const void* a,
                           const void* b, const void* c, const void* d, const void* stream) {
@@ -146,8 +196,22 @@
     });
 }
 
+extern "C" int mmvid_tower_forward_top(const mmvid_tower_cfg_t* cfg, const mmvid_tower_layer_t* layers, const float* x_in,
+                                       float* x_out, void* saved, void* scratch, int full_seqs, int prefix_rows, void* stream) {
+    TRY(check_cfg(cfg));
+    TRY(check_top(cfg, full_seqs, prefix_rows));
+    if (!top_wanted(cfg, saved, full_seqs, prefix_rows)) return mmvid_tower_forward(cfg, layers, x_in, x_out, saved, scratch, stream);
+    MMVID_REQUIRE(layers && x_in && x_out && scratch, "tower_forward_top: null pointer");
+    TopRows top;
+    top.fs = full_seqs, top.P = prefix_rows;
+    const uint64_t key = mmvid_hash_bytes(&top, sizeof(top), tower_key(6, cfg, layers, x_in, x_out, saved, scratch, stream));
+    return mmvid_run_cached(key, (hipStream_t)stream, [=](hipStream_t s) {
+        return tower_forward_enqueue(cfg, layers, x_in, x_out, saved, scratch, (void*)s, nullptr, 0, top);
+    });
+}
+
 static int tower_forward_enqueue(const mmvid_tower_cfg_t* cfg, const mmvid_tower_layer_t* layers, const float* x_in,
-                                 float* x_out, void* saved, void* scratch, void* stream, void* kv_cache, int kv_lmax) {
+                                 float* x_out, void* saved, void* scratch, void* stream, void* kv_cache, int kv_lmax, TopRows top) {
     const Dims d = dims_of(*cfg);
     const SavedLayer sl = saved_layout(d);
     const Scratch sc = scratch_layout(d);
@@ -179,6 +243,29 @@
         if (kv_cache)
             TRY(mmvid_kv_store(sv + sl.qkv, 3 * d.E, d.B, d.L, d.E, nullptr, 0, kv_lmax,
                                (char*)kv_cache + (int64_t)i * d.B * kv_lmax * 2 * d.E * 2, stream));
+        if (top.on() && i == d.layers - 1) {
+            const TopDims t = top_dims(d, top);
+            const int64_t rowb = (int64_t)d.E * 2, rowf = (int64_t)d.E * 4;
+            char* o_full = scr + sc.d_o;
+            float* xc = (float*)(scr + sc.infer);
+            if (top.fs > 0)
+                TRY(mmvid_attention_fwd(sv + sl.qkv, 3 * d.E, top.fs, d.L, d.H, d.E, scale, cfg->mask_mode, cfg->r0, cfg->c0, cfg->r1, cfg->c1,
+                                        sv + sl.o, d.E, (float*)(sv + sl.lse2), stream));
+            TRY(mmvid_attention_fwd_rows(sv + sl.qkv + t.Mf * 3 * rowb, 3 * d.E, t.nP, d.L, d.H, d.E, scale, cfg->mask_mode, cfg->r0, cfg->c0,
+                                         cfg->r1, cfg->c1, top.P, o_full + t.Mf * rowb, d.E, (float*)(sv + sl.lse2) + (int64_t)top.fs * d.H * d.L,
+                                         stream));
+            TRY(copy_rows(sv + sl.o + t.Mf * rowb, top.P * rowb, o_full + t.Mf * rowb, d.L * rowb, top.P * rowb, top.P * rowb, t.nP, stream));
+            TRY(copy_d2d(xc, x, t.Mf * rowf, stream));
+            TRY(copy_rows((char*)xc + t.Mf * rowf, top.P * rowf, (const char*)x + t.Mf * rowf, d.L * rowf, top.P * rowf, top.P * rowf, t.nP, stream));
+            TRY(linear_fwd(t.R, d.E, d.E, sv + sl.o, ly.out_w, ly.out_b, xc, nullptr, 0, xmid, nullptr, stream));
+            TRY(mmvid_layernorm_fwd(xmid, d.E, t.R, d.E, ly.ln2_w, ly.ln2_b, cfg->ln_eps, sv + sl.h2, nullptr, d.E, (float*)(sv + sl.mean2),
+                                    (float*)(sv + sl.rstd2), stream));
+            TRY(linear_fwd(t.R, d.F, d.E, sv + sl.h2, ly.fc_w, ly.fc_b, nullptr, sv + sl.pre, 1, nullptr, sv + sl.act, stream));
+            TRY(linear_fwd(t.R, d.E, d.F, sv + sl.act, ly.pj_w, ly.pj_b, xmid, nullptr, 0, x_out, nullptr, stream));
+            TRY(copy_d2d(xc, (const char*)x_out + t.Mf * rowf, t.Mp * rowf, stream));
+            TRY(copy_rows((char*)x_out + t.Mf * rowf, d.L * rowf, xc, top.P * rowf, top.P * rowf, d.L * rowf, t.nP, stream));
+            break;
+        }
         TRY(mmvid_attention_fwd(sv + sl.qkv, 3 * d.E, d.B, d.L, d.H, d.E, scale, cfg->mask_mode, cfg->r0, cfg->c0, cfg->r1,
                                 cfg->c1, sv + sl.o, d.E, (float*)(sv + sl.lse2), stream));
         TRY(linear_fwd(d.M, d.E, d.E, sv + sl.o, ly.out_w, ly.out_b, x, nullptr, 0, xmid, nullptr, stream));
@@ -202,8 +289,22 @@
     });
 }
 
+extern "C" int mmvid_tower_backward_top(const mmvid_tower_cfg_t* cfg, const mmvid_tower_layer_t* layers, float* g, void* saved,
+                                        void* scratch, int full_seqs, int prefix_rows, void* stream) {
+    TRY(check_cfg(cfg));
+    TRY(check_top(cfg, full_seqs, prefix_rows));
+    if (!top_wanted(cfg, saved, full_seqs, prefix_rows)) return mmvid_tower_backward(cfg, layers, g, saved, scratch, stream);
+    MMVID_REQUIRE(layers && g && saved && scratch, "tower_backward_top: null pointer");
+    TopRows top;
+    top.fs = full_seqs, top.P = prefix_rows;
+    const uint64_t key = mmvid_hash_bytes(&top, sizeof(top), tower_key(7, cfg, layers, g, saved, scratch, nullptr, stream));
+    return mmvid_run_cached(key, (hipStream_t)stream, [=](hipStream_t s) {
+        return tower_backward_enqueue(cfg, layers, g, saved, scratch, (void*)s, top);
+    });
+}
+
 static int tower_backward_enqueue(const mmvid_tower_cfg_t* cfg, const mmvid_tower_layer_t* layers, float* g, void* saved,
-                                  void* scratch, void* stream) {
+                                  void* scratch, void* stream, TopRows top) {
     const Dims d = dims_of(*cfg);
     const SavedLayer sl = saved_layout(d);
     const Scratch sc = scratch_layout(d);
@@ -227,31 +328,77 @@
         const char* sv = (const char*)saved + (int64_t)i * sl.total;
         char* kp = keep + (int64_t)i * kl.total;
         void* g_pj = kp + kl.g_pj;
+        const bool pruned = top.on() && i == d.layers - 1;
+        const TopDims t = top_dims(d, top);
+        const int64_t Mr = pruned ? t.R : d.M;
+        const int64_t rowb = (int64_t)d.E * 2, rowf = (int64_t)d.E * 4;
+        if (pruned) {
+            char* stage = scr + sc.infer;
+            TRY(copy_rows(stage, top.P * rowf, (const char*)g + t.Mf * rowf, d.L * rowf, top.P * rowf, top.P * rowf, t.nP, stream));
+            TRY(copy_d2d((char*)g + t.Mf * rowf, stage, t.Mp * rowf, stream));
+        }
         if (i == d.layers - 1) {
-            TRY(mmvid_cast_f32_to_bf16(g, g_pj, d.M * d.E, stream));
+            TRY(mmvid_cast_f32_to_bf16(g, g_pj, Mr * d.E, stream));
             if (ly.g_pj_b && det_ws) TRY(mmvid_colsum_bf16_det(g_pj, d.E, d.M, d.E, ly.g_pj_b, det_ws, det_bytes, stream));
-            if (ly.g_pj_b && !det_ws) TRY(mmvid_colsum_bf16(g_pj, d.E, d.M, d.E, ly.g_pj_b, stream));
-        }
-        TRY(linear_dx(d.M, d.E, d.F, g_pj, ly.pj_w, sv + sl.pre, nullptr, kp + kl.d_pre, stream, ly.g_fc_b, det_ws, det_bytes));
-        TRY(linear_dx(d.M, d.F, d.E, kp + kl.d_pre, ly.fc_w, nullptr, nullptr, d_h, stream));
+            if (ly.g_pj_b && !det_ws) TRY(mmvid_colsum_bf16(g_pj, d.E, Mr, d.E, ly.g_pj_b, stream));
+        }
+        TRY(linear_dx(Mr, d.E, d.F, g_pj, ly.pj_w, sv + sl.pre, nullptr, kp + kl.d_pre, stream, ly.g_fc_b, det_ws, det_bytes));
+        TRY(linear_dx(Mr, d.F, d.E, kp + kl.d_pre, ly.fc_w, nullptr, nullptr, d_h, stream));
         {
             mmvid_ln_reduce_t r = {(const float*)(kp + sl.k_ln2), ly.g_ln2_w, ly.g_ln2_b, ly.g_out_b};
             int nb = 0;
             TRY(mmvid_layernorm_bwd_partial(d_h, 1, d.E, (const float*)(sv + sl.x_mid), d.E, (const float*)(sv + sl.mean2),
-                                            (const float*)(sv + sl.rstd2), ly.ln2_w, d.M, d.E, g, d.E, 1, kp + kl.g_out, r.dw != nullptr,
+                                            (const float*)(sv + sl.rstd2), ly.ln2_w, Mr, d.E, g, d.E, 1, kp + kl.g_out, r.dw != nullptr,
                                             r.db != nullptr, r.dx_colsum != nullptr, (float*)(kp + sl.k_ln2), ln_ws_floats, &nb, stream));
-            if (r.dw || r.db || r.dx_colsum) ln_items.push_back(r), ln_blocks = nb;
-        }
-        TRY(linear_dx(d.M, d.E, d.E, kp + kl.g_out, ly.out_w, nullptr, nullptr, scr + sc.d_o, stream));
-        if (det_ws)
-            TRY(mmvid_attention_bwd_bias_det(sv + sl.qkv, 3 * d.E, sv + sl.o, d.E, scr + sc.d_o, d.E, (const float*)(sv + sl.lse2),
+            if (r.dw || r.db || r.dx_colsum) {
+                ln_items.push_back(r), ln_blocks = nb;
+                if (pruned) {
+                    int nb_full = (int)((d.M + 3) / 4), cap = (int)(ln_ws_floats / (3 * (int64_t)d.E));
+                    cap = cap > 2048 ? 2048 : cap;
+                    if (cap >= 64 && nb_full > cap) nb_full = cap;
+                    if (nb_full > nb && hipMemsetAsync(kp + sl.k_ln2 + (int64_t)nb * 3 * d.E * 4, 0, (size_t)(nb_full - nb) * 3 * d.E * 4,
+                                                       (hipStream_t)stream) != hipSuccess) {
+                        mmvid_set_error("tower_backward_top: memset failed");
+                        return MMVID_ERR_HIP;
+                    }
+                    ln_blocks = nb_full > nb ? nb_full : nb;
+                }
+            }
+        }
+        if (pruned) {
+            char* d_oc = (char*)d_h;
+            char* do_full = scr + sc.d_o;
+            char* o_full = scr + sc.infer;
+            TRY(linear_dx(Mr, d.E, d.E, kp + kl.g_out, ly.out_w, nullptr, nullptr, d_oc, stream));
+            TRY(copy_rows(do_full + t.Mf * rowb, d.L * rowb, d_oc + t.Mf * rowb, top.P * rowb, top.P * rowb, t.T * rowb, t.nP, stream));
+            TRY(copy_rows(o_full + t.Mf * rowb, d.L * rowb, sv + sl.o + t.Mf * rowb, top.P * rowb, top.P * rowb, t.T * rowb, t.nP, stream));
+            TRY(copy_rows(kp + kl.dqkv + t.Mf * 3 * rowb, 3 * rowb, nullptr, 0, 0, rowb, (int64_t)t.nP * d.L, stream));
+            if (top.fs > 0)
+                TRY(mmvid_attention_bwd_bias(sv + sl.qkv, 3 * d.E, sv + sl.o, d.E, d_oc, d.E, (const float*)(sv + sl.lse2), (float*)(scr + sc.delta),
+                                             top.fs, d.L, d.H, d.E, scale, cfg->mask_mode, cfg->r0, cfg->c0, cfg->r1, cfg->c1, kp + kl.dqkv, 3 * d.E,
+                                             ly.g_in_b, stream));
+            const int64_t st = (int64_t)top.fs * d.H * d.L;
+            TRY(mmvid_attention_bwd_bias_rows(sv + sl.qkv + t.Mf * 3 * rowb, 3 * d.E, o_full + t.Mf * rowb, d.E, do_full + t.Mf * rowb, d.E,
+                                              (const float*)(sv + sl.lse2) + st, (float*)(scr + sc.delta) + st, t.nP, d.L, d.H, d.E, scale,
+                                              cfg->mask_mode, cfg->r0, cfg->c0, cfg->r1, cfg->c1, top.P, kp + kl.dqkv + t.Mf * 3 * rowb, 3 * d.E,
+                                              ly.g_in_b, stream));
+        } else {
+            TRY(linear_dx(d.M, d.E, d.E, kp + kl.g_out, ly.out_w, nullptr, nullptr, scr + sc.d_o, stream));
+            if (det_ws)
+                TRY(mmvid_attention_bwd_bias_det(sv + sl.qkv, 3 * d.E, sv + sl.o, d.E, scr + sc.d_o, d.E, (const float*)(sv + sl.lse2),
+                                                 (float*)(scr + sc.delta), d.B, d.L, d.H, d.E, scale, cfg->mask_mode, cfg->r0, cfg->c0,
+                                                 cfg->r1, cfg->c1, kp + kl.dqkv, 3 * d.E, ly.g_in_b, det_ws, det_bytes, stream));
+            else
+                TRY(mmvid_attention_bwd_bias(sv + sl.qkv, 3 * d.E, sv + sl.o, d.E, scr + sc.d_o, d.E, (const float*)(sv + sl.lse2),
                                              (float*)(scr + sc.delta), d.B, d.L, d.H, d.E, scale, cfg->mask_mode, cfg->r0, cfg->c0,
-                                             cfg->r1, cfg->c1, kp + kl.dqkv, 3 * d.E, ly.g_in_b, det_ws, det_bytes, stream));
-        else
-            TRY(mmvid_attention_bwd_bias(sv + sl.qkv, 3 * d.E, sv + sl.o, d.E, scr + sc.d_o, d.E, (const float*)(sv + sl.lse2),
-                                         (float*)(scr + sc.delta), d.B, d.L, d.H, d.E, scale, cfg->mask_mode, cfg->r0, cfg->c0,
-                                         cfg->r1, cfg->c1, kp + kl.dqkv, 3 * d.E, ly.g_in_b, stream));
+                                             cfg->r1, cfg->c1, kp + kl.dqkv, 3 * d.E, ly.g_in_b, stream));
+        }
         TRY(linear_dx(d.M, 3 * d.E, d.E, kp + kl.dqkv, ly.in_w, nullptr, nullptr, d_h, stream));
+        if (pruned) {
+            char* stage = scr + sc.infer;
+            TRY(copy_d2d(stage, (const char*)g + t.Mf * rowf, t.Mp * rowf, stream));
+            TRY(copy_rows((char*)g + t.Mf * rowf, d.L * rowf, stage, top.P * rowf, top.P * rowf, d.L * rowf, t.nP, stream));
+        }
         {
             mmvid_ln_reduce_t r = {(const float*)(kp + sl.k_ln1), ly.g_ln1_w, ly.g_ln1_b, i > 0 ? layers[i - 1].g_pj_b : nullptr};
             int nb = 0;
@@ -274,6 +421,7 @@
                            {3 * d.E, d.E, kl.dqkv, sl.h1, &mmvid_tower_layer_t::g_in_w}};
     std::vector<float*> outs((size_t)d.layers * 4);
     mmvid_dw_kind_t kd[4];
+    std::vector<int32_t> rows((size_t)d.layers * 4, 0);
     int nk = 0;
     for (const Kind& k : kinds) {
         float** o = outs.data() + (size_t)nk * d.layers;
@@ -284,13 +432,17 @@
         kd[nk].dY = keep + k.dy_off, kd[nk].ldy = k.N, kd[nk].strideY = kl.total / 2;
         kd[nk].X = (const char*)saved + k.x_off, kd[nk].ldx = k.K, kd[nk].strideX = sl.total / 2;
         kd[nk].dW_list = o;
+        if (top.on() && k.dy_off != kl.dqkv) rows[(size_t)nk * d.layers + d.layers - 1] = (int32_t)top_dims(d, top).R;
         ++nk;
     }
     if (nk == 0) return MMVID_OK;
-    if (mmvid_gemm_dw_multi_fill(nk, kd, d.layers) >= 0.7) return mmvid_gemm_bf16_dw_multi(d.M, nk, kd, d.layers, 1, stream);
+    if (mmvid_gemm_dw_multi_fill(nk, kd, d.layers) >= 0.7) {
+        if (!top.on()) return mmvid_gemm_bf16_dw_multi(d.M, nk, kd, d.layers, 1, stream);
+        return mmvid_gemm_bf16_dw_multi_rows(d.M, nk, kd, d.layers, rows.data(), 1, stream);
+    }
     for (int k = 0; k < nk; ++k)
         for (int i = d.layers - 1; i >= 0; --i)
-            TRY(linear_dw(d.M, kd[k].N, kd[k].K, (const char*)kd[k].dY + (int64_t)i * kl.total, (const char*)kd[k].X + (int64_t)i * sl.total,
+            TRY(linear_dw(rows[(size_t)k * d.layers + i] > 0 ? rows[(size_t)k * d.layers + i] : d.M, kd[k].N, kd[k].K, (const char*)kd[k].dY + (int64_t)i * kl.total, (const char*)kd[k].X + (int64_t)i * sl.total,
                           kd[k].dW_list[i], nullptr, ws, stream));
     return MMVID_OK;
 }
diff --git a/mmvid_amd/dalle_bert.py b/mmvid_amd/dalle_bert.py
--- a/mmvid_amd/dalle_bert.py
+++ b/mmvid_amd/dalle_bert.py
@@ -1,3 +1,5 @@
+import os
+
 import torch
 import torch.nn.functional as F
 from torch import nn
@@ -223,8 +225,8 @@
     def get_special_token(self, tok_list, batch_size=1, device='cuda'):
         return torch.tensor(tok_list, dtype=torch.long, device=device).repeat(batch_size, 1)
 
-    def transformer_forward(self, tokens):
-        out = self.transformer(tokens)
+    def transformer_forward(self, tokens, top_rows=None):
+        out = self.transformer(tokens) if top_rows is None else self.transformer(tokens, top_rows=top_rows)
         if self.stable:
             out = self.norm_by_max(out)
         return out
@@ -456,7 +458,10 @@
             y_rel = torch.zeros(B, L, y_neg.shape[-1], device=device, dtype=y_neg.dtype).index_copy(1, keep, y_neg)
             y = torch.cat((y_main[:B], y_rel, y_main[B:])) if do_vid else torch.cat((y_main, y_rel))
         else:
-            y = self.transformer_forward(x_seq)
+            top_rows = None
+            if (rel or do_vid) and not self.stable and os.environ.get('MMVID_TOP_ROWS', '1') != '0':
+                top_rows = (B, max(([self.rel_tok_index] if rel else []) + ([self.vid_tok_index] if do_vid else [])) + 1)
+            y = self.transformer_forward(x_seq, top_rows=top_rows)
         if self._debug_keep is not None:
             self._debug_keep.update(mask1=mask1, nfm=not_fully_masked, target=target, target_warp=target_warp, ids=ids, sel=sel,
                                     tfull=tfull, cnt=cnt, x_seq=x_seq, y=y)
diff --git a/mmvid_amd/ops.py b/mmvid_amd/ops.py
--- a/mmvid_amd/ops.py
+++ b/mmvid_amd/ops.py
@@ -179,6 +179,13 @@
     call('mmvid_gemm_bf16_dw_multi', M, len(kinds), arr, G, int(accumulate), _stream())
 
 
+def gemm_dw_multi_rows(kinds, rows, accumulate=True):
+    arr, keep, M, G = _dw_kinds(kinds)
+    flat = [int(r) for per_kind in rows for r in per_kind]
+    assert len(flat) == len(kinds) * G
+    call('mmvid_gemm_bf16_dw_multi_rows', M, len(kinds), arr, G, (ctypes.c_int32 * len(flat))(*flat), int(accumulate), _stream())
+
+
 def gemm_dw_multi_fill(shapes, groups):
     arr = (_lib.DwKind * len(shapes))()
     for a, (N, K) in zip(arr, shapes):
```

After: 214,900 (median of 6 runs). No clear change (+0.8%).
